# 666DZY666/micronet

Hardware: NVIDIA H100
Metric: qat_step_images_per_sec (higher is better)
Workload: dtype f32 (bf16 tensor-core products of exact integer levels / exact bf16 pieces, fp32 accumulate)

## Files before the change

### harness/fconv_probe.py

```python
import ctypes as C
import os
import subprocess
import sys

import torch


def run():
    from micronet_b200 import _lib as L
    lib = L.load()
    B, Cc, H, W, K, R = 256, 3, 32, 32, 256, 5
    dev = torch.device("cuda")
    x = torch.randn(B, Cc, H, W, device=dev)
    w = torch.randn(K, Cc, R, R, device=dev) * 0.1
    b = torch.randn(K, device=dev)
    y = torch.empty(B, K, H, W, device=dev)
    dy = torch.randn(B, K, H, W, device=dev)
    dw = torch.empty_like(w)
    sh = L.ConvShape(B, Cc, H, W, K, R, R, 1, 1, R // 2, R // 2, 1, 1, 1)
    scratch = torch.empty(int(lib.mnb_fconv2d_wgrad_tc_scratch_bytes(C.byref(sh))), dtype=torch.uint8, device=dev)
    err = L.tc_err_flag(dev)

    def fwd():
        L.check(lib.mnb_fconv2d_fwd_tc(C.byref(sh), x.data_ptr(), w.data_ptr(), b.data_ptr(), y.data_ptr(), err.data_ptr(),
                                       L.stream()), "fwd")

    def wg():
        L.check(lib.mnb_fconv2d_wgrad_tc(C.byref(sh), dy.data_ptr(), x.data_ptr(), dw.data_ptr(), scratch.data_ptr(),
                                         err.data_ptr(), L.stream()), "wgrad")
    out = []
    for name, fn in (("fwd", fwd), ("wgrad", wg)):
        for _ in range(3):
            fn()
        torch.cuda.synchronize()
        e0, e1 = torch.cuda.Event(enable_timing=True), torch.cuda.Event(enable_timing=True)
        e0.record()
        for _ in range(10):
            fn()
        e1.record()
        torch.cuda.synchronize()
        out.append(f"{name} {e0.elapsed_time(e1) * 100:.1f}us")
    print(os.environ.get("MNB_FCONV_DEBUG", "0"), " ".join(out), flush=True)


if __name__ == "__main__":
    if len(sys.argv) > 1:
        run()
    else:
        for mask in (0, 1, 2, 4, 8, 3, 7, 9, 15):
            subprocess.run([sys.executable, __file__, "child"], env=dict(os.environ, MNB_FCONV_DEBUG=str(mask)), timeout=120)
```

### include/micronet_b200.h

```cpp
#ifndef MICRONET_B200_H
#define MICRONET_B200_H

#include <stdint.h>

#ifdef __cplusplus
extern "C" {
#endif

typedef void* mnb_stream_t;

#define MNB_E_ARG (-1)
#define MNB_E_UNSUPPORTED (-2)

int mnb_version(void);
const char* mnb_last_error(void);
int64_t mnb_launch_count(void);

typedef struct {
  int32_t batch, in_c, in_h, in_w;
  int32_t out_c, ker_h, ker_w;
  int32_t stride_h, stride_w, pad_h, pad_w, dil_h, dil_w, groups;
} mnb_conv_shape;

#define MNB_ACT_DOREFA 1
#define MNB_ACT_IAO 2
#define MNB_ACT_SIGN 3

typedef struct {
  int32_t mode;
  int32_t bits;
  int32_t qmin, qmax;
  int32_t q_type;
  const float* scale;
  const float* zero_point;
  const float* obs_min;
  const float* obs_max;
} mnb_act_qparams;

int mnb_act_quant_fwd(const float* x, int64_t n, const mnb_act_qparams* qp, uint8_t* codes,
                      uint32_t* pass_bits, float* xq, mnb_stream_t stream);
int mnb_act_quant_bwd(const float* g, const uint32_t* pass_bits, int64_t n, const mnb_act_qparams* qp,
                      float* dx, mnb_stream_t stream);

int mnb_bn_fold_fwd(const float* w, int32_t out_c, int32_t per_channel, const float* gamma, const float* beta,
                    const float* bias, const float* mean, const float* var, double eps, float* w_fused, float* b_fused,
                    mnb_stream_t stream);
int mnb_bn_fold_bwd(const float* dw_fused, const float* db_fused, const float* w, int32_t out_c, int32_t per_channel,
                    const float* gamma, const float* bias, const float* mean, const float* var, double eps, float* dw,
                    float* out6, mnb_stream_t stream);
int mnb_bn_fold_running(float* running_mean, float* running_var, const float* batch_mean, const float* batch_var, int32_t n,
                        double momentum, int32_t first, mnb_stream_t stream);

int mnb_quant_add_fwd(const float* a, const float* b, int64_t n, const mnb_act_qparams* qp, float* out,
                      uint32_t* pass_bits_a, uint32_t* pass_bits_b, int32_t relu ,
                      mnb_stream_t stream);
int mnb_quant_add_bwd(const float* g, const uint32_t* pass_bits_a, const uint32_t* pass_bits_b, int64_t n,
                      const mnb_act_qparams* qp, float* da, float* db, mnb_stream_t stream);

int64_t mnb_observe_scratch_bytes(int64_t n, int32_t rows);
int mnb_iao_observe(const float* x, int64_t n, int32_t rows, int32_t observer_kind, int32_t first,
                    double momentum, double percentile, float* min_val, float* max_val,
                    int32_t update_qparams, int32_t symmetric, int32_t qmin, int32_t qmax,
                    float* scale, float* zero_point, void* scratch, mnb_stream_t stream);
int mnb_iao_update_qparams(const float* min_val, const float* max_val, int32_t rows, int32_t symmetric,
                           int32_t qmin, int32_t qmax, float* scale, float* zero_point,
                           mnb_stream_t stream);

int mnb_dorefa_weight_fwd(const float* w, int64_t numel, int32_t out_c, int32_t w_bits, int16_t* w_int,
                          float* w_scale, float* wq, float* aux, void* scratch, mnb_stream_t stream);
int mnb_dorefa_weight_bwd(const float* g_wq, const float* aux, int64_t numel, int32_t w_bits, float* dw,
                          void* scratch, mnb_stream_t stream);
int mnb_wb_weight_fwd(float* w, int32_t out_c, int32_t in_c_per_group, int32_t ker_hw, int32_t W,
                      int16_t* w_int, float* w_scale, float* wq, float* aux, mnb_stream_t stream);
int mnb_wb_weight_bwd(const float* g_wq, const float* w, const float* aux, int32_t out_c,
                      int32_t in_c_per_group, int32_t ker_hw, int32_t W, float* dw, mnb_stream_t stream);
int mnb_iao_weight_fwd(const float* w, int64_t numel, int32_t out_c, int32_t rows, const float* scale,
                       const float* zero_point, const float* obs_min, const float* obs_max,
                       int32_t q_type, int32_t qmin, int32_t qmax, int16_t* w_int, float* w_scale,
                       float* wq, uint8_t* pass, mnb_stream_t stream);
int mnb_iao_weight_bwd(const float* g_wq, const uint8_t* pass, const float* scale, int64_t numel,
                       int32_t out_c, int32_t rows, float* dw, mnb_stream_t stream);

typedef struct {
  const uint8_t* a_codes;
  const float* a_f32;
  int32_t a_offset;
  const float* a_offset_zp;
  const float* a_scale;
  const int16_t* w_int;
  const float* w_scale;
  const float* w_f32;
  const float* bias;
} mnb_conv_operands;

int mnb_conv2d_fwd(const mnb_conv_shape* s, const mnb_conv_operands* op, float* y, mnb_stream_t stream);
int mnb_conv2d_dgrad(const mnb_conv_shape* s, const float* dy, const float* wq, const uint32_t* pass_bits,
                     const mnb_act_qparams* qp, float* dx, mnb_stream_t stream);
int64_t mnb_wgrad_scratch_bytes(const mnb_conv_shape* s);
int mnb_conv2d_wgrad(const mnb_conv_shape* s, const float* dy, const mnb_conv_operands* op, float* dwq,
                     void* scratch, mnb_stream_t stream);
int mnb_channel_stats(const float* x, int32_t batch, int32_t channels, int32_t hw, int32_t as_mean_var,
                      float* stats, void* scratch, mnb_stream_t stream);
int mnb_channel_stats_bwd(const float* x, const float* mean, const float* dmean, const float* dvar,
                          int32_t batch, int32_t channels, int32_t hw, float* dx, mnb_stream_t stream);

int mnb_fq_conv2d_fwd_tc(const mnb_conv_shape* s, const float* x, const mnb_act_qparams* qp,
                         const int16_t* w_int, const float* w_scale, const float* bias, float* y,
                         uint8_t* codes, uint32_t* pass_bits, void* wpack_scratch, int32_t* err_flag,
                         mnb_stream_t stream);

int mnb_conv2d_dgrad_tc(const mnb_conv_shape* s, const float* dy, const int16_t* w_int, const float* w_scale,
                        const uint32_t* pass_bits, const mnb_act_qparams* qp, float* dx, void* wpack_scratch,
                        int32_t* err_flag, mnb_stream_t stream);

int64_t mnb_wgrad_tc_scratch_bytes(const mnb_conv_shape* s);
int mnb_conv2d_wgrad_tc(const mnb_conv_shape* s, const float* dy, const float* x, const mnb_act_qparams* qp,
                        float* dwq, void* scratch, int32_t* inexact_flag, int32_t* err_flag, mnb_stream_t stream);
int mnb_conv2d_wgrad_cond(const mnb_conv_shape* s, const float* dy, const mnb_conv_operands* op, float* dwq,
                          void* scratch, const int32_t* run_if_nonzero, mnb_stream_t stream);

int mnb_bn_batch_stats(const float* x, int32_t batch, int32_t channels, int32_t hw, double eps, double momentum,
                       float* running_mean, float* running_var, int64_t* num_batches_tracked, float* mean_invstd,
                       void* scratch, mnb_stream_t stream);
int mnb_bn_sign_fwd(const float* x, int32_t batch, int32_t channels, int32_t hw, const float* mean, const float* invstd,
                    const float* gamma, const float* beta, int32_t out_shuffle_groups, float* y, uint32_t* pass_bits,
                    mnb_stream_t stream);
int mnb_bn_sign_bwd(const float* g, const uint32_t* pass_bits, const float* x, int32_t batch, int32_t channels, int32_t hw,
                    const float* mean, const float* invstd, const float* gamma, int32_t training,
                    int32_t out_shuffle_groups, float* dx, float* dgamma, float* dbeta, float* dx_channel_sum,
                    void* scratch, mnb_stream_t stream);

int mnb_bn_sign_pool_fwd(const float* x, int32_t batch, int32_t channels, int32_t H, int32_t W, const float* mean,
                         const float* invstd, const float* gamma, const float* beta, int32_t out_shuffle_groups, float* y,
                         uint32_t* pass_bits, uint8_t* argmax, mnb_stream_t stream);
int mnb_bn_sign_pool_bwd(const float* g, const uint32_t* pass_bits, const uint8_t* argmax, const float* x, int32_t batch,
                         int32_t channels, int32_t H, int32_t W, const float* mean, const float* invstd, const float* gamma,
                         int32_t training, int32_t out_shuffle_groups, float* dx, float* dgamma, float* dbeta,
                         float* dx_channel_sum, void* scratch, mnb_stream_t stream);

int mnb_maxpool2d_fwd(const float* x, int32_t batch, int32_t channels, int32_t H, int32_t W, int32_t kernel, int32_t stride,
                      int32_t pad, int32_t out_shuffle_groups, float* y, uint8_t* argmax, mnb_stream_t stream);
int mnb_maxpool2d_bwd(const float* g, const uint8_t* argmax, int32_t batch, int32_t channels, int32_t H, int32_t W,
                      int32_t kernel, int32_t stride, int32_t pad, int32_t out_shuffle_groups, float* dx,
                      mnb_stream_t stream);

int mnb_bn_sign_fwd_packed(const float* x, int32_t batch, int32_t channels, int32_t hw, const float* mean,
                           const float* invstd, const float* gamma, const float* beta, int32_t out_shuffle_groups, float* y,
                           uint32_t* pass_bits, void* x_packed, mnb_stream_t stream);

int mnb_fconv2d_plan(const mnb_conv_shape* s, int32_t wgrad, int32_t* out, int32_t n);
int mnb_fconv2d_fwd_tc(const mnb_conv_shape* s, const float* x, const float* w, const float* bias, float* y,
                       int32_t* err_flag, mnb_stream_t stream);
int64_t mnb_fconv2d_wgrad_tc_scratch_bytes(const mnb_conv_shape* s);
int mnb_fconv2d_wgrad_tc(const mnb_conv_shape* s, const float* dy, const float* x, float* dw, void* scratch,
                         int32_t* err_flag, mnb_stream_t stream);

int64_t mnb_pk_act_bytes(int32_t batch, int32_t channels, int32_t h, int32_t w, int32_t terms);
int mnb_pk_pack_act(const float* x, int32_t batch, int32_t channels, int32_t h, int32_t w, const mnb_act_qparams* qp,
                    int32_t terms, const float* ch_scale, int32_t phase_split, void* out_pk, uint8_t* bits8,
                    mnb_stream_t stream);
int mnb_bn_relu_quant_pack_fwd(const float* x, int32_t batch, int32_t channels, int32_t hw, const float* mean,
                               const float* invstd, const float* gamma, const float* beta, const mnb_act_qparams* qp,
                               int32_t out_shuffle_groups, void* x_packed, uint32_t* pass_bits, mnb_stream_t stream);
int mnb_bn_sign_bwd_pack(const float* g, const uint32_t* pass_bits, const float* x, int32_t batch, int32_t channels, int32_t hw,
                         const float* mean, const float* invstd, const float* gamma, const float* dgamma, const float* dbeta,
                         int32_t out_shuffle_groups, const float* ch_scale, int32_t terms, float* dx, void* dy_packed,
                         mnb_stream_t stream);
int mnb_bn_sign_pool_bwd_pack(const float* g, const uint32_t* pass_bits, const uint8_t* argmax, const float* x, int32_t batch,
                              int32_t channels, int32_t H, int32_t W, const float* mean, const float* invstd,
                              const float* gamma, const float* dgamma, const float* dbeta, int32_t out_shuffle_groups,
                              const float* ch_scale, int32_t terms, void* dy_packed, mnb_stream_t stream);
int mnb_pk_conv_codes(const mnb_conv_shape* s, const void* a_pk, int32_t terms_a, const void* w_img, int32_t terms_w,
                      const float* n_scale, const float* a_scale, float a_scale_const, const float* bias, int32_t level_bound,
                      int16_t* codes, float* dec, int32_t* err_flag, mnb_stream_t stream);
int mnb_codes_decode(const int16_t* codes, const float* dec, int32_t batch, int32_t channels, int32_t hw, float* x,
                     mnb_stream_t stream);
int mnb_bn_batch_stats_codes(const int16_t* codes, const float* dec, int32_t batch, int32_t channels, int32_t hw, double eps,
                             double momentum, float* running_mean, float* running_var, int64_t* num_batches_tracked,
                             float* mean_invstd, void* scratch, mnb_stream_t stream);
int mnb_bn_sign_fwd_packed_codes(const int16_t* codes, const float* dec, int32_t batch, int32_t channels, int32_t hw,
                                 const float* mean, const float* invstd, const float* gamma, const float* beta,
                                 int32_t out_shuffle_groups, float* y, uint32_t* pass_bits, void* x_packed, mnb_stream_t stream);
int mnb_bn_sign_bwd_codes(const float* g, const uint32_t* pass_bits, const int16_t* codes, const float* dec, int32_t batch,
                          int32_t channels, int32_t hw, const float* mean, const float* invstd, const float* gamma,
                          int32_t training, int32_t out_shuffle_groups, float* dx, float* dgamma, float* dbeta,
                          float* dx_channel_sum, void* scratch, mnb_stream_t stream);
int mnb_bn_sign_pool_fwd_codes(const int16_t* codes, const float* dec, int32_t batch, int32_t channels, int32_t H, int32_t W,
                               const float* mean, const float* invstd, const float* gamma, const float* beta,
                               int32_t out_shuffle_groups, float* y, uint32_t* pass_bits, uint8_t* argmax, mnb_stream_t stream);
int mnb_bn_sign_pool_bwd_codes(const float* g, const uint32_t* pass_bits, const uint8_t* argmax, const int16_t* codes,
                               const float* dec, int32_t batch, int32_t channels, int32_t H, int32_t W, const float* mean,
                               const float* invstd, const float* gamma, int32_t training, int32_t out_shuffle_groups, float* dx,
                               float* dgamma, float* dbeta, float* dx_channel_sum, void* scratch, mnb_stream_t stream);
int mnb_bn_sign_bwd_pack_codes(const float* g, const uint32_t* pass_bits, const int16_t* codes, const float* dec, int32_t batch,
                               int32_t channels, int32_t hw, const float* mean, const float* invstd, const float* gamma,
                               const float* dgamma, const float* dbeta, int32_t out_shuffle_groups, const float* ch_scale,
                               int32_t terms, float* dx, void* dy_packed, mnb_stream_t stream);
int mnb_bn_sign_pool_bwd_pack_codes(const float* g, const uint32_t* pass_bits, const uint8_t* argmax, const int16_t* codes,
                                    const float* dec, int32_t batch, int32_t channels, int32_t H, int32_t W, const float* mean,
                                    const float* invstd, const float* gamma, const float* dgamma, const float* dbeta,
                                    int32_t out_shuffle_groups, const float* ch_scale, int32_t terms, void* dy_packed,
                                    mnb_stream_t stream);
int mnb_pk_pack_act_relu(const float* x, int32_t batch, int32_t channels, int32_t h, int32_t w, const mnb_act_qparams* qp,
                         int32_t terms, const float* ch_scale, int32_t phase_split, int32_t relu, void* out_pk,
                         uint8_t* bits8, mnb_stream_t stream);
int64_t mnb_pk_grouped_act_bytes(int32_t batch, int32_t channels, int32_t h, int32_t w, int32_t terms, int32_t groups);
int mnb_pk_pack_act_grouped(const float* x, int32_t batch, int32_t channels, int32_t h, int32_t w, const mnb_act_qparams* qp,
                            int32_t terms, const float* ch_scale, int32_t phase_split, int32_t relu, void* out_pk,
                            uint8_t* bits8, int32_t groups, mnb_stream_t stream);
int mnb_pk_conv_plan(const mnb_conv_shape* s, int32_t mode, int32_t terms_a, int32_t terms_w, int32_t* out16);
int mnb_pk_conv_plan_ex(const mnb_conv_shape* s, int32_t mode, int32_t terms_a, int32_t terms_w, int32_t* out, int32_t n);
int mnb_pk_wgrad_plan(const mnb_conv_shape* s, int32_t terms_dy, int32_t terms_x, int32_t* out, int32_t n);
int64_t mnb_pk_wimage_bytes(const mnb_conv_shape* s, int32_t mode, int32_t terms_a, int32_t terms_w);
int mnb_pk_pack_weight(const mnb_conv_shape* s, int32_t mode, int32_t terms_a, int32_t terms_w, const int16_t* w_int,
                       const float* w_f32, const float* kzero, void* w_img, mnb_stream_t stream);
int mnb_pk_conv(const mnb_conv_shape* s, int32_t mode, const void* a_pk, int32_t terms_a, const void* w_img, int32_t terms_w,
                const float* n_scale, const float* a_scale, float a_scale_const, const float* bias, const uint8_t* bits8,
                float gain, float* out, int32_t* err_flag, mnb_stream_t stream);
typedef struct mnb_pk_post {
  const mnb_act_qparams* q;
  int32_t relu;
  int32_t phase_split;
  void* out_pk;
  const float* bn_mean;
  const float* bn_invstd;
  const float* bn_gamma;
  const float* bn_beta;
  int32_t shuffle_groups;
} mnb_pk_post;
int mnb_pk_conv_post(const mnb_conv_shape* s, const void* a_pk, int32_t terms_a, const void* w_img, int32_t terms_w,
                     const float* n_scale, const float* a_scale, float a_scale_const, const float* bias, float* out,
                     const mnb_pk_post* post, int32_t* err_flag, mnb_stream_t stream);
int mnb_quant_add_pack_fwd(const float* a, const float* b, int32_t batch, int32_t channels, int32_t h, int32_t w,
                           const mnb_act_qparams* qp, int32_t relu, float* out, const mnb_pk_post* post, mnb_stream_t stream);
int64_t mnb_pk_i8_act_bytes(int32_t batch, int32_t channels, int32_t h, int32_t w);
int mnb_pk_i8_pack_act(const float* x, int32_t batch, int32_t channels, int32_t h, int32_t w, const mnb_act_qparams* qp,
                       int32_t phase_split, int32_t relu, void* out_pk, mnb_stream_t stream);
int mnb_pk_i8_conv_plan(const mnb_conv_shape* s, int32_t* out, int32_t n);
int64_t mnb_pk_i8_wimage_bytes(const mnb_conv_shape* s);
int mnb_pk_i8_pack_weight(const mnb_conv_shape* s, const int16_t* w_int, void* w_img, mnb_stream_t stream);
int mnb_pk_i8_conv(const mnb_conv_shape* s, const void* a_pk, const void* w_img, const float* n_scale, const float* a_scale,
                   float a_scale_const, const float* bias, float* out, const mnb_pk_post* post, int32_t* err_flag,
                   mnb_stream_t stream);
int mnb_quant_add_pack_i8_fwd(const float* a, const float* b, int32_t batch, int32_t channels, int32_t h, int32_t w,
                              const mnb_act_qparams* qp, int32_t relu, float* out, const mnb_pk_post* post, mnb_stream_t stream);
int mnb_bn_relu_quant_pack_i8_fwd(const float* x, int32_t batch, int32_t channels, int32_t hw, const float* mean,
                                  const float* invstd, const float* gamma, const float* beta, const mnb_act_qparams* qp,
                                  int32_t out_shuffle_groups, void* x_packed, mnb_stream_t stream);
int mnb_pk_plane_maxpool(const void* in_pk, int32_t batch, int32_t channels, int32_t h, int32_t w, int32_t k, int32_t s, int32_t p,
                         int32_t int8, void* out_pk, mnb_stream_t stream);
int mnb_pk_plane_maxpool_requant(const void* in_pk, int32_t batch, int32_t channels, int32_t h, int32_t w, int32_t k, int32_t s,
                                 int32_t p, int32_t int8, const mnb_act_qparams* q_in, const mnb_act_qparams* q_out, void* out_pk,
                                 mnb_stream_t stream);
int64_t mnb_pk_wgrad_scratch_bytes(const mnb_conv_shape* s, int32_t terms_dy, int32_t terms_x);
int mnb_pk_wgrad(const mnb_conv_shape* s, const void* dy_pk, int32_t terms_dy, const void* x_pk, int32_t terms_x,
                 const float* a_scale, const float* kdiv, float* dw, void* scratch, int32_t* err_flag, mnb_stream_t stream);
int mnb_pk_wgrad_taps_plan(const mnb_conv_shape* s, int32_t terms_dy, int32_t terms_x, int32_t* out, int32_t n);
int mnb_pk_wgrad_taps(const mnb_conv_shape* s, const void* dy_pk, int32_t terms_dy, const void* x_pk, int32_t terms_x,
                      const float* a_scale, const float* kdiv, float* dw, void* scratch, int32_t* err_flag, mnb_stream_t stream);
int mnb_pk_gc3_plan(const mnb_conv_shape* s, int32_t mode, int32_t terms_a, int32_t terms_w, int32_t* out, int32_t n);
int mnb_pk_gc3_conv(const mnb_conv_shape* s, int32_t mode, const void* a_pk, int32_t terms_a, const void* w_img, int32_t terms_w,
                    const float* n_scale, const float* a_scale, float a_scale_const, const float* bias, const uint8_t* bits8,
                    float gain, float* out, int32_t* err_flag, mnb_stream_t stream);
int mnb_pk_gc3_conv_codes(const mnb_conv_shape* s, const void* a_pk, int32_t terms_a, const void* w_img, int32_t terms_w,
                          const float* n_scale, const float* a_scale, float a_scale_const, const float* bias, int32_t level_bound,
                          int16_t* codes, float* dec, int32_t* err_flag, mnb_stream_t stream);

int mnb_xnor_supported(const mnb_conv_shape* s);
int64_t mnb_xnor_act_bytes(int32_t batch, int32_t channels, int32_t h, int32_t w, int32_t groups);
int mnb_xnor_pack_act(const float* x, int32_t batch, int32_t channels, int32_t h, int32_t w, int32_t groups, void* out_bits,
                      mnb_stream_t stream);
int64_t mnb_xnor_wimage_bytes(const mnb_conv_shape* s);
int mnb_xnor_pack_weight(const mnb_conv_shape* s, const int16_t* w_int, void* w_img, mnb_stream_t stream);
int mnb_xnor_conv_fwd(const mnb_conv_shape* s, const void* a_bits, const void* w_img, const float* alpha, const float* bias,
                      float* y, mnb_stream_t stream);
#define MNB_XNOR_BITS 0
#define MNB_XNOR_PM1_BF16 1
typedef struct mnb_xnor_post {
  int32_t format;
  int32_t out_groups;
  int32_t shuffle_groups;
  int32_t pool2;
  const float* bn_mean;
  const float* bn_invstd;
  const float* bn_gamma;
  const float* bn_beta;
} mnb_xnor_post;
int64_t mnb_xnor_post_bytes(const mnb_conv_shape* s, const mnb_xnor_post* post);
int mnb_xnor_conv_post(const mnb_conv_shape* s, const void* a_bits, const void* w_img, const float* alpha, const float* bias,
                       const mnb_xnor_post* post, void* out, mnb_stream_t stream);
int mnb_xnor_pack_act_post(const float* x, int32_t batch, int32_t channels, int32_t h, int32_t w, const mnb_xnor_post* post,
                           void* out_bits, mnb_stream_t stream);

int mnb_adam_step(float* params, const float* grads, float* exp_avg, float* exp_avg_sq, int64_t n, float lr,
                  float beta1, float beta2, float eps, float weight_decay, int32_t step, mnb_stream_t stream);

void mnb_set_tc_profile_buffer(void* dev_int64x16);

int mnb_selftest_umma(const float* A, const float* B, float* D, int32_t N, int32_t K, int32_t int8,
                      int32_t* err_flag, mnb_stream_t stream);
int mnb_selftest_tma3d(const float* src, const int64_t* dims3_host, const int32_t* box3_host,
                       const int32_t* coord3_host, float* out, int32_t* err_flag, mnb_stream_t stream);

int mnb_selftest_mma_rate(int32_t N, int32_t n_acc, int32_t a_shift16, int32_t iters, int32_t mn_major,
                          int64_t* out2, int32_t* err_flag, mnb_stream_t stream);

#ifdef __cplusplus
}
#endif
#endif
```

### micronet_b200/_lib.py

```python
from __future__ import annotations

import ctypes as C
import os

import torch

_HERE = os.path.dirname(os.path.abspath(__file__))
LIB_PATH = os.path.join(_HERE, "lib", "libmicronet_b200.so")

ACT_DOREFA, ACT_IAO, ACT_SIGN = 1, 2, 3


class ConvShape(C.Structure):
    _fields_ = [(n, C.c_int32) for n in (
        "batch", "in_c", "in_h", "in_w", "out_c", "ker_h", "ker_w", "stride_h", "stride_w",
        "pad_h", "pad_w", "dil_h", "dil_w", "groups")]


class ActQParams(C.Structure):
    _fields_ = [("mode", C.c_int32), ("bits", C.c_int32), ("qmin", C.c_int32), ("qmax", C.c_int32),
                ("q_type", C.c_int32), ("scale", C.c_void_p), ("zero_point", C.c_void_p),
                ("obs_min", C.c_void_p), ("obs_max", C.c_void_p)]


class PkPost(C.Structure):
    _fields_ = [("q", C.POINTER(ActQParams)), ("relu", C.c_int32), ("phase_split", C.c_int32), ("out_pk", C.c_void_p),
                ("bn_mean", C.c_void_p), ("bn_invstd", C.c_void_p), ("bn_gamma", C.c_void_p), ("bn_beta", C.c_void_p),
                ("shuffle_groups", C.c_int32)]


XNOR_BITS, XNOR_PM1_BF16 = 0, 1


class XnorPost(C.Structure):
    _fields_ = [("format", C.c_int32), ("out_groups", C.c_int32), ("shuffle_groups", C.c_int32), ("pool2", C.c_int32),
                ("bn_mean", C.c_void_p), ("bn_invstd", C.c_void_p), ("bn_gamma", C.c_void_p), ("bn_beta", C.c_void_p)]


class ConvOperands(C.Structure):
    _fields_ = [("a_codes", C.c_void_p), ("a_f32", C.c_void_p), ("a_offset", C.c_int32),
                ("a_offset_zp", C.c_void_p), ("a_scale", C.c_void_p), ("w_int", C.c_void_p),
                ("w_scale", C.c_void_p), ("w_f32", C.c_void_p), ("bias", C.c_void_p)]


_P, _I, _L, _D = C.c_void_p, C.c_int32, C.c_int64, C.c_double
_SHAPE, _ACTQ, _OPS = C.POINTER(ConvShape), C.POINTER(ActQParams), C.POINTER(ConvOperands)

PROTOTYPES = {
    "mnb_version": (C.c_int, []),
    "mnb_last_error": (C.c_char_p, []),
    "mnb_launch_count": (_L, []),
    "mnb_act_quant_fwd": (C.c_int, [_P, _L, _ACTQ, _P, _P, _P, _P]),
    "mnb_act_quant_bwd": (C.c_int, [_P, _P, _L, _ACTQ, _P, _P]),
    "mnb_bn_fold_fwd": (C.c_int, [_P, _I, _I, _P, _P, _P, _P, _P, _D, _P, _P, _P]),
    "mnb_bn_fold_bwd": (C.c_int, [_P, _P, _P, _I, _I, _P, _P, _P, _P, _D, _P, _P, _P]),
    "mnb_bn_fold_running": (C.c_int, [_P, _P, _P, _P, _I, _D, _I, _P]),
    "mnb_quant_add_fwd": (C.c_int, [_P, _P, _L, _ACTQ, _P, _P, _P, _I, _P]),
    "mnb_quant_add_bwd": (C.c_int, [_P, _P, _P, _L, _ACTQ, _P, _P, _P]),
    "mnb_observe_scratch_bytes": (_L, [_L, _I]),
    "mnb_iao_observe": (C.c_int, [_P, _L, _I, _I, _I, _D, _D, _P, _P, _I, _I, _I, _I, _P, _P, _P, _P]),
    "mnb_iao_update_qparams": (C.c_int, [_P, _P, _I, _I, _I, _I, _P, _P, _P]),
    "mnb_dorefa_weight_fwd": (C.c_int, [_P, _L, _I, _I, _P, _P, _P, _P, _P, _P]),
    "mnb_dorefa_weight_bwd": (C.c_int, [_P, _P, _L, _I, _P, _P, _P]),
    "mnb_wb_weight_fwd": (C.c_int, [_P, _I, _I, _I, _I, _P, _P, _P, _P, _P]),
    "mnb_wb_weight_bwd": (C.c_int, [_P, _P, _P, _I, _I, _I, _I, _P, _P]),
    "mnb_iao_weight_fwd": (C.c_int, [_P, _L, _I, _I, _P, _P, _P, _P, _I, _I, _I, _P, _P, _P, _P, _P]),
    "mnb_iao_weight_bwd": (C.c_int, [_P, _P, _P, _L, _I, _I, _P, _P]),
    "mnb_conv2d_fwd": (C.c_int, [_SHAPE, _OPS, _P, _P]),
    "mnb_conv2d_dgrad": (C.c_int, [_SHAPE, _P, _P, _P, _ACTQ, _P, _P]),
    "mnb_wgrad_scratch_bytes": (_L, [_SHAPE]),
    "mnb_conv2d_wgrad": (C.c_int, [_SHAPE, _P, _OPS, _P, _P, _P]),
    "mnb_channel_stats": (C.c_int, [_P, _I, _I, _I, _I, _P, _P, _P]),
    "mnb_channel_stats_bwd": (C.c_int, [_P, _P, _P, _P, _I, _I, _I, _P, _P]),
    "mnb_fq_conv2d_fwd_tc": (C.c_int, [_SHAPE, _P, _ACTQ, _P, _P, _P, _P, _P, _P, _P, _P, _P]),
    "mnb_conv2d_dgrad_tc": (C.c_int, [_SHAPE, _P, _P, _P, _P, _ACTQ, _P, _P, _P, _P]),
    "mnb_wgrad_tc_scratch_bytes": (_L, [_SHAPE]),
    "mnb_conv2d_wgrad_tc": (C.c_int, [_SHAPE, _P, _P, _ACTQ, _P, _P, _P, _P, _P]),
    "mnb_conv2d_wgrad_cond": (C.c_int, [_SHAPE, _P, _OPS, _P, _P, _P, _P]),
    "mnb_bn_batch_stats": (C.c_int, [_P, _I, _I, _I, _D, _D, _P, _P, _P, _P, _P, _P]),
    "mnb_bn_sign_fwd": (C.c_int, [_P, _I, _I, _I, _P, _P, _P, _P, _I, _P, _P, _P]),
    "mnb_bn_sign_bwd": (C.c_int, [_P, _P, _P, _I, _I, _I, _P, _P, _P, _I, _I, _P, _P, _P, _P, _P, _P]),
    "mnb_bn_sign_pool_fwd": (C.c_int, [_P, _I, _I, _I, _I, _P, _P, _P, _P, _I, _P, _P, _P, _P]),
    "mnb_bn_sign_pool_bwd": (C.c_int, [_P, _P, _P, _P, _I, _I, _I, _I, _P, _P, _P, _I, _I, _P, _P, _P, _P, _P, _P]),
    "mnb_bn_sign_fwd_packed": (C.c_int, [_P, _I, _I, _I, _P, _P, _P, _P, _I, _P, _P, _P, _P]),
    "mnb_fconv2d_plan": (C.c_int, [_SHAPE, _I, _P, _I]),
    "mnb_fconv2d_fwd_tc": (C.c_int, [_SHAPE, _P, _P, _P, _P, _P, _P]),
    "mnb_fconv2d_wgrad_tc_scratch_bytes": (_L, [_SHAPE]),
    "mnb_fconv2d_wgrad_tc": (C.c_int, [_SHAPE, _P, _P, _P, _P, _P, _P]),
    "mnb_maxpool2d_fwd": (C.c_int, [_P, _I, _I, _I, _I, _I, _I, _I, _I, _P, _P, _P]),
    "mnb_maxpool2d_bwd": (C.c_int, [_P, _P, _I, _I, _I, _I, _I, _I, _I, _I, _P, _P]),
    "mnb_adam_step": (C.c_int, [_P, _P, _P, _P, _L, C.c_float, C.c_float, C.c_float, C.c_float, C.c_float, _I, _P]),
    "mnb_pk_act_bytes": (_L, [_I, _I, _I, _I, _I]),
    "mnb_pk_pack_act": (C.c_int, [_P, _I, _I, _I, _I, _ACTQ, _I, _P, _I, _P, _P, _P]),
    "mnb_bn_relu_quant_pack_fwd": (C.c_int, [_P, _I, _I, _I, _P, _P, _P, _P, _ACTQ, _I, _P, _P, _P]),
    "mnb_pk_pack_act_relu": (C.c_int, [_P, _I, _I, _I, _I, _ACTQ, _I, _P, _I, _I, _P, _P, _P]),
    "mnb_pk_grouped_act_bytes": (_L, [_I, _I, _I, _I, _I, _I]),
    "mnb_pk_pack_act_grouped": (C.c_int, [_P, _I, _I, _I, _I, _ACTQ, _I, _P, _I, _I, _P, _P, _I, _P]),
    "mnb_pk_conv_plan": (C.c_int, [_SHAPE, _I, _I, _I, _P]),
    "mnb_pk_conv_plan_ex": (C.c_int, [_SHAPE, _I, _I, _I, _P, _I]),
    "mnb_pk_wgrad_plan": (C.c_int, [_SHAPE, _I, _I, _P, _I]),
    "mnb_pk_wimage_bytes": (_L, [_SHAPE, _I, _I, _I]),
    "mnb_pk_pack_weight": (C.c_int, [_SHAPE, _I, _I, _I, _P, _P, _P, _P, _P]),
    "mnb_pk_conv": (C.c_int, [_SHAPE, _I, _P, _I, _P, _I, _P, _P, C.c_float, _P, _P, C.c_float, _P, _P, _P]),
    "mnb_bn_sign_bwd_pack": (C.c_int, [_P, _P, _P, _I, _I, _I, _P, _P, _P, _P, _P, _I, _P, _I, _P, _P, _P]),
    "mnb_bn_sign_pool_bwd_pack": (C.c_int, [_P, _P, _P, _P, _I, _I, _I, _I, _P, _P, _P, _P, _P, _I, _P, _I, _P, _P]),
    "mnb_pk_conv_post": (C.c_int, [_SHAPE, _P, _I, _P, _I, _P, _P, C.c_float, _P, _P, C.POINTER(PkPost), _P, _P]),
    "mnb_pk_conv_codes": (C.c_int, [_SHAPE, _P, _I, _P, _I, _P, _P, C.c_float, _P, _I, _P, _P, _P, _P]),
    "mnb_codes_decode": (C.c_int, [_P, _P, _I, _I, _I, _P, _P]),
    "mnb_bn_batch_stats_codes": (C.c_int, [_P, _P, _I, _I, _I, _D, _D, _P, _P, _P, _P, _P, _P]),
    "mnb_bn_sign_fwd_packed_codes": (C.c_int, [_P, _P, _I, _I, _I, _P, _P, _P, _P, _I, _P, _P, _P, _P]),
    "mnb_bn_sign_bwd_codes": (C.c_int, [_P, _P, _P, _P, _I, _I, _I, _P, _P, _P, _I, _I, _P, _P, _P, _P, _P, _P]),
    "mnb_bn_sign_pool_fwd_codes": (C.c_int, [_P, _P, _I, _I, _I, _I, _P, _P, _P, _P, _I, _P, _P, _P, _P]),
    "mnb_bn_sign_pool_bwd_codes": (C.c_int, [_P, _P, _P, _P, _P, _I, _I, _I, _I, _P, _P, _P, _I, _I, _P, _P, _P, _P, _P, _P]),
    "mnb_bn_sign_bwd_pack_codes": (C.c_int, [_P, _P, _P, _P, _I, _I, _I, _P, _P, _P, _P, _P, _I, _P, _I, _P, _P, _P]),
    "mnb_bn_sign_pool_bwd_pack_codes": (C.c_int, [_P, _P, _P, _P, _P, _I, _I, _I, _I, _P, _P, _P, _P, _P, _I, _P, _I, _P,
                                                  _P]),
    "mnb_quant_add_pack_fwd": (C.c_int, [_P, _P, _I, _I, _I, _I, _ACTQ, _I, _P, C.POINTER(PkPost), _P]),
    "mnb_pk_i8_act_bytes": (_L, [_I, _I, _I, _I]),
    "mnb_pk_i8_pack_act": (C.c_int, [_P, _I, _I, _I, _I, _ACTQ, _I, _I, _P, _P]),
    "mnb_pk_i8_conv_plan": (C.c_int, [_SHAPE, _P, _I]),
    "mnb_pk_i8_wimage_bytes": (_L, [_SHAPE]),
    "mnb_pk_i8_pack_weight": (C.c_int, [_SHAPE, _P, _P, _P]),
    "mnb_pk_i8_conv": (C.c_int, [_SHAPE, _P, _P, _P, _P, C.c_float, _P, _P, C.POINTER(PkPost), _P, _P]),
    "mnb_quant_add_pack_i8_fwd": (C.c_int, [_P, _P, _I, _I, _I, _I, _ACTQ, _I, _P, C.POINTER(PkPost), _P]),
    "mnb_bn_relu_quant_pack_i8_fwd": (C.c_int, [_P, _I, _I, _I, _P, _P, _P, _P, _ACTQ, _I, _P, _P]),
    "mnb_pk_plane_maxpool": (C.c_int, [_P, _I, _I, _I, _I, _I, _I, _I, _I, _P, _P]),
    "mnb_pk_plane_maxpool_requant": (C.c_int, [_P, _I, _I, _I, _I, _I, _I, _I, _I, _ACTQ, _ACTQ, _P, _P]),
    "mnb_pk_wgrad_scratch_bytes": (_L, [_SHAPE, _I, _I]),
    "mnb_pk_wgrad": (C.c_int, [_SHAPE, _P, _I, _P, _I, _P, _P, _P, _P, _P, _P]),
    "mnb_pk_wgrad_taps_plan": (C.c_int, [_SHAPE, _I, _I, _P, _I]),
    "mnb_pk_wgrad_taps": (C.c_int, [_SHAPE, _P, _I, _P, _I, _P, _P, _P, _P, _P, _P]),
    "mnb_pk_gc3_plan": (C.c_int, [_SHAPE, _I, _I, _I, _P, _I]),
    "mnb_pk_gc3_conv": (C.c_int, [_SHAPE, _I, _P, _I, _P, _I, _P, _P, C.c_float, _P, _P, C.c_float, _P, _P, _P]),
    "mnb_pk_gc3_conv_codes": (C.c_int, [_SHAPE, _P, _I, _P, _I, _P, _P, C.c_float, _P, _I, _P, _P, _P, _P]),
    "mnb_xnor_supported": (C.c_int, [_SHAPE]),
    "mnb_xnor_act_bytes": (_L, [_I, _I, _I, _I, _I]),
    "mnb_xnor_pack_act": (C.c_int, [_P, _I, _I, _I, _I, _I, _P, _P]),
    "mnb_xnor_wimage_bytes": (_L, [_SHAPE]),
    "mnb_xnor_pack_weight": (C.c_int, [_SHAPE, _P, _P, _P]),
    "mnb_xnor_conv_fwd": (C.c_int, [_SHAPE, _P, _P, _P, _P, _P, _P]),
    "mnb_xnor_post_bytes": (_L, [_SHAPE, C.POINTER(XnorPost)]),
    "mnb_xnor_conv_post": (C.c_int, [_SHAPE, _P, _P, _P, _P, C.POINTER(XnorPost), _P, _P]),
    "mnb_xnor_pack_act_post": (C.c_int, [_P, _I, _I, _I, _I, C.POINTER(XnorPost), _P, _P]),
    "mnb_set_tc_profile_buffer": (None, [_P]),
    "mnb_selftest_mma_rate": (C.c_int, [_I, _I, _I, _I, _I, _P, _P, _P]),
    "mnb_selftest_umma": (C.c_int, [_P, _P, _P, _I, _I, _I, _P, _P]),
    "mnb_selftest_tma3d": (C.c_int, [_P, C.POINTER(C.c_int64), C.POINTER(C.c_int32), C.POINTER(C.c_int32), _P, _P, _P]),
}

_lib = None


def load():
    global _lib
    if _lib is not None:
        return _lib
    if not os.path.exists(LIB_PATH):
        raise RuntimeError(
            f"micronet_b200: {LIB_PATH} is missing - build it with `python -m micronet_b200.build` "
            "(there is no CPU / PyTorch fallback for the fake-quant hot path)")
    lib = C.CDLL(LIB_PATH)
    for name, (res, args) in PROTOTYPES.items():
        fn = getattr(lib, name)
        fn.restype, fn.argtypes = res, args
    _lib = lib
    return lib


def check(rc: int, what: str):
    if rc != 0:
        msg = load().mnb_last_error().decode(errors="replace")
        kind = ValueError if rc < 0 else RuntimeError
        raise kind(f"micronet_b200.{what} failed (code {rc}): {msg}")


def ptr(t):
    return None if t is None else t.data_ptr()


def stream():
    return torch.cuda.current_stream().cuda_stream


def require_cuda(*tensors):
    for t in tensors:
        if t is not None and not t.is_cuda:
            raise RuntimeError(
                "micronet_b200: the fake-quant engine runs on CUDA (sm_90a) tensors only; "
                "got a CPU tensor - there is deliberately no CPU fallback")


def require_f32(*tensors):
    for t in tensors:
        if t is not None and t.dtype != torch.float32:
            raise TypeError(f"micronet_b200: fp32 tensors only (the reference's QAT modules are fp32), got {t.dtype}")


def launch_count() -> int:
    return int(load().mnb_launch_count())


_errflags = {}


def tc_err_flag(device):
    key = (device.type, device.index)
    if key not in _errflags:
        _errflags[key] = torch.zeros(1, dtype=torch.int32, device=device)
    return _errflags[key]


def tc_check(device=None):
    for key, flag in _errflags.items():
        code = int(flag.item())
        if code:
            raise RuntimeError(f"micronet_b200: tensor-core pipeline wait timed out (code {code}) on {key}")


E_UNSUPPORTED = -2
KEEP_DEBUG = False
USE_TC = os.environ.get("MNB_DISABLE_TC", "0") != "1"
PK_MODE = os.environ.get("MNB_PK", "auto")
PK_TERMS = int(os.environ.get("MNB_PK_TERMS", "3"))
PK_TERMS_BWD = int(os.environ.get("MNB_PK_TERMS_BWD", "2"))
PK_WBWTAB = os.environ.get("MNB_PK_WBWTAB", "1") == "1"
PK_WG_TAPS = os.environ.get("MNB_PK_WG_TAPS", "1") != "0"
PK_GC3 = os.environ.get("MNB_PK_GC3", "1") != "0"

XNOR_MODE = os.environ.get("MNB_XNOR", "auto")

PLANE_ONLY = os.environ.get("MNB_PLANE_ONLY", "1") == "1"

_scratch = {}


def scratch(device, rows=1):
    lib = load()
    need = int(lib.mnb_observe_scratch_bytes(0, int(rows)))
    key = (device.type, device.index)
    buf = _scratch.get(key)
    if buf is None or buf.numel() < need:
        buf = torch.zeros(max(need, 1 << 20), dtype=torch.uint8, device=device)
        _scratch[key] = buf
    return buf
```

### micronet_b200/csrc/mnb_conv_fp32_tc.cu

```cuda
#include <cuda.h>
#include <cuda_bf16.h>

#include <algorithm>
#include <cstdlib>

#include "mnb_common.cuh"
#include "mnb_tc.cuh"

namespace tcfp32 {

constexpr int NTHREADS = 512;
constexpr int kMaxDynSmem = 227 * 1024 - 2560;
constexpr int SUB = 32;

struct Params {
  int B, C, K, H, W, R, pad;
  int KR, KP;
  int NP;
  int TH, PH, PW;
  int tiles_per_img, n_tiles;
  int nbuf_a;
  int off_b, off_a, off_patch, off_tab, off_sum, off_stg, sum_bytes, a_term_bytes, a_buf_bytes, b_term_bytes, patch_bytes;
  const float* x; const float* w; const float* bias; float* y;
  const float* dy; float* partial;
  int* err;
  int dbg;
};

struct alignas(16) Shared {
  uint64_t a_full[2], a_empty[2];
  uint32_t abort;
};

__device__ __forceinline__ uint32_t pack_bf16x2(float a, float b) {
  __nv_bfloat162 v = __floats2bfloat162_rn(a, b);
  return *reinterpret_cast<uint32_t*>(&v);
}
__device__ __forceinline__ void split3_pair(float a, float b, uint32_t& hp, uint32_t& mp, uint32_t& lp) {
  hp = pack_bf16x2(a, b);
  const float ra = a - __uint_as_float(hp << 16), rb = b - __uint_as_float(hp & 0xffff0000u);
  mp = pack_bf16x2(ra, rb);
  const float la = ra - __uint_as_float(mp << 16), lb = rb - __uint_as_float(mp & 0xffff0000u);
  lp = pack_bf16x2(la, lb);
}
__device__ __forceinline__ void store_split8(const float (&v)[8], uint8_t* dst, int term_bytes) {
  uint32_t hp[4], mp[4], lp[4];
#pragma unroll
  for (int j = 0; j < 4; ++j) split3_pair(v[2 * j], v[2 * j + 1], hp[j], mp[j], lp[j]);
  *reinterpret_cast<uint4*>(dst) = make_uint4(hp[0], hp[1], hp[2], hp[3]);
  *reinterpret_cast<uint4*>(dst + term_bytes) = make_uint4(mp[0], mp[1], mp[2], mp[3]);
  *reinterpret_cast<uint4*>(dst + 2 * term_bytes) = make_uint4(lp[0], lp[1], lp[2], lp[3]);
}
__device__ __forceinline__ void conv_bar_sync(int nthreads) {
  asm volatile("bar.sync 1, %0;" ::"r"(nthreads) : "memory");
}
__device__ __forceinline__ void mma_bar_sync() {
  asm volatile("bar.sync 2, 128;" ::: "memory");
}

__device__ __constant__ int kProdA[6] = {1, 2, 0, 1, 0, 0};
__device__ __constant__ int kProdB[6] = {1, 0, 2, 0, 1, 0};

constexpr int PF = 4;
__device__ __forceinline__ float patch_element(const Params& p, int i, int b, int h0) {
  const int pc = i % p.PW, t = i / p.PW;
  const int pr = t % p.PH, c = t / p.PH;
  const int h = h0 - p.pad + pr, w = pc - p.pad;
  return (h >= 0 && h < p.H && w >= 0 && w < p.W) ? __ldg(p.x + (((int64_t)b * p.C + c) * p.H + h) * p.W + w) : 0.f;
}
__device__ __forceinline__ void patch_fetch(const Params& p, int tile, int ct, int nconv, float (&v)[PF]) {
  const int b = tile / p.tiles_per_img, h0 = (tile - b * p.tiles_per_img) * p.TH;
  const int n = p.C * p.PH * p.PW;
#pragma unroll
  for (int k = 0; k < PF; ++k) {
    const int i = ct + k * nconv;
    v[k] = i < n ? patch_element(p, i, b, h0) : 0.f;
  }
}
__device__ __forceinline__ void patch_commit(const Params& p, float* patch, int tile, int ct, int nconv, const float (&v)[PF]) {
  const int b = tile / p.tiles_per_img, h0 = (tile - b * p.tiles_per_img) * p.TH;
  const int n = p.C * p.PH * p.PW;
#pragma unroll
  for (int k = 0; k < PF; ++k) {
    const int i = ct + k * nconv;
    if (i < n) patch[i] = v[k];
  }
  for (int i = ct + PF * nconv; i < n; i += nconv) patch[i] = patch_element(p, i, b, h0);
}

constexpr int FWD_NCONV = NTHREADS - 32 - 128;

__global__ void __launch_bounds__(NTHREADS, 1) fwd_kernel(const Params p) {
  extern __shared__ __align__(1024) uint8_t smem[];
  __shared__ Shared sh;
  __shared__ __align__(16) float epi_bias[256];
  const int tid = threadIdx.x, warp = tid >> 5, lane = tid & 31;
  uint8_t* bop = smem + p.off_b;
  uint8_t* aop = smem + p.off_a;
  int* tab = reinterpret_cast<int*>(smem + p.off_tab);
  const int kchunks = p.KP / 8;

  if (tid == 0) {
    for (int i = 0; i < 2; ++i) {
      tc::mbar_init(&sh.a_full[i], FWD_NCONV / 32); tc::mbar_init(&sh.a_empty[i], 4);
    }
    sh.abort = 0;
    tc::fence_barrier_init();
  }
  for (int n = tid; n < 256; n += NTHREADS) epi_bias[n] = (p.bias && n < p.K) ? __ldg(p.bias + n) : 0.f;
  for (int i = tid; i < kchunks * p.NP; i += NTHREADS) {
    const int j = i / p.NP, n = i - j * p.NP;
    float v[8];
#pragma unroll
    for (int e = 0; e < 8; ++e) {
      const int kk = j * 8 + e;
      v[e] = (n < p.K && kk < p.KR) ? __ldg(p.w + (int64_t)n * p.KR + kk) : 0.f;
    }
    store_split8(v, bop + (size_t)i * 16, p.b_term_bytes);
  }
  for (int kk = tid; kk < p.KP; kk += NTHREADS) {
    int off = -1;
    if (kk < p.KR) {
      const int s = kk % p.R, t = kk / p.R;
      const int r = t % p.R, c = t / p.R;
      off = (c * p.PH + r) * p.PW + s;
    }
    tab[kk] = off;
  }
  tc::fence_proxy_async_smem();
  __syncthreads();

  if (warp >= 4 && warp < 8) {
    const int m = (warp - 4) * 32 + lane;
    float* stage = reinterpret_cast<float*>(smem + p.off_stg);
    const int64_t plane = (int64_t)p.H * p.W;
    const uint64_t a_desc0 = tc::smem_desc_kmajor_noswz(tc::smem_u32(aop), 128u * 16u, 128u);
    const uint64_t b_desc0 = tc::smem_desc_kmajor_noswz(tc::smem_u32(bop), (uint32_t)p.NP * 16u, 128u);
    const uint32_t a_term16 = (uint32_t)p.a_term_bytes >> 4, b_term16 = (uint32_t)p.b_term_bytes >> 4;
    const uint32_t a_buf16 = (uint32_t)p.a_buf_bytes >> 4;
    const uint32_t a_step16 = 2u * 128u, b_step16 = 2u * (uint32_t)p.NP;
    uint32_t t = 0;
    for (int tile = blockIdx.x; tile < p.n_tiles; tile += gridDim.x, ++t) {
      const uint32_t ab = p.nbuf_a == 2 ? (t & 1u) : 0u, aph = p.nbuf_a == 2 ? ((t >> 1) & 1u) : (t & 1u);
      tc::mbar_wait_soft(&sh.a_full[ab], aph, p.err, 502, &sh.abort);
      const int b = tile / p.tiles_per_img, h0 = (tile - b * p.tiles_per_img) * p.TH;
      float* dst = p.y + (int64_t)b * p.K * plane + (int64_t)h0 * p.W + m;
      for (int n0 = 0; n0 < p.NP; n0 += 32) {
        float acc0[16], acc1[16];
        tc::zero_acc(acc0); tc::zero_acc(acc1);
        tc::wg_fence();
        tc::fence_acc(acc0); tc::fence_acc(acc1);
        for (int q = (p.dbg & 2) ? 6 : 0; q < 6; ++q) {
          const uint64_t aq = a_desc0 + (uint64_t)(ab * a_buf16 + (uint32_t)kProdA[q] * a_term16);
          const uint64_t bq = b_desc0 + (uint64_t)((uint32_t)kProdB[q] * b_term16 + (uint32_t)n0);
          for (int ks = 0; ks < p.KP / 16; ++ks) {
            const uint64_t ad = aq + (uint64_t)((uint32_t)ks * a_step16), bd = bq + (uint64_t)((uint32_t)ks * b_step16);
            tc::Mma<32>::bf16<0, 0>(acc0, ad, bd, 1);
            tc::Mma<32>::bf16<0, 0>(acc1, ad + 64u, bd, 1);
          }
        }
        tc::wg_commit();
        tc::wg_wait<0>();
        tc::fence_acc(acc0); tc::fence_acc(acc1);
        if (n0 + 32 >= p.NP) {
          __syncwarp();
          if (lane == 0) tc::mbar_arrive(&sh.a_empty[ab]);
        }
        mma_bar_sync();
        tc::frag_to_smem(acc0, stage, tc::kStageLd, 0);
        tc::frag_to_smem(acc1, stage, tc::kStageLd, 64);
        mma_bar_sync();
        if (p.dbg & 4) continue;
        float bs[32];
#pragma unroll
        for (int v = 0; v < 8; ++v) {
          const float4 c4 = *reinterpret_cast<const float4*>(&epi_bias[n0 + 4 * v]);
          bs[4 * v] = c4.x; bs[4 * v + 1] = c4.y; bs[4 * v + 2] = c4.z; bs[4 * v + 3] = c4.w;
        }
        float* op = dst + (int64_t)n0 * plane;
#pragma unroll
        for (int j = 0; j < 32; ++j, op += plane)
          if (n0 + j < p.K) *op = stage[j * tc::kStageLd + m] + bs[j];
      }
    }
  } else {
    if (warp == 0) goto done;
    const int ct = warp < 4 ? tid - 32 : tid - 32 - 128;
    float* patch0 = reinterpret_cast<float*>(smem + p.off_patch);
    const int items = 128 * kchunks;
    const int patch_floats = p.patch_bytes / 4;
    float pre[PF];
    if ((int)blockIdx.x < p.n_tiles) {
      patch_fetch(p, blockIdx.x, ct, FWD_NCONV, pre);
      patch_commit(p, patch0, blockIdx.x, ct, FWD_NCONV, pre);
    }
    uint32_t t = 0;
    for (int tile = blockIdx.x; tile < p.n_tiles; tile += gridDim.x, ++t) {
      const float* patch = patch0 + (size_t)(t & 1u) * patch_floats;
      conv_bar_sync(FWD_NCONV);
      const int next = tile + (int)gridDim.x;
      if (next < p.n_tiles) patch_fetch(p, next, ct, FWD_NCONV, pre);
      const uint32_t ab = p.nbuf_a == 2 ? (t & 1u) : 0u, aph = p.nbuf_a == 2 ? ((t >> 1) & 1u) : (t & 1u);
      if (!tc::mbar_wait(&sh.a_empty[ab], aph ^ 1u, p.err, 504)) break;
      uint8_t* abuf = aop + (size_t)ab * p.a_buf_bytes;
      for (int i = (p.dbg & 1) ? items : ct; i < items; i += FWD_NCONV) {
        const int j = i >> 7, m = i & 127;
        const int base = (m / p.W) * p.PW + (m % p.W);
        int off[8];
#pragma unroll
        for (int e = 0; e < 8; ++e) off[e] = tab[j * 8 + e];
        float v[8];
#pragma unroll
        for (int e = 0; e < 8; ++e) v[e] = off[e] >= 0 ? patch[off[e] + base] : 0.f;
        store_split8(v, abuf + (size_t)i * 16, p.a_term_bytes);
      }
      tc::fence_proxy_async_smem();
      __syncwarp();
      if (lane == 0) tc::mbar_arrive(&sh.a_full[ab]);
      if (next < p.n_tiles) patch_commit(p, patch0 + (size_t)((t + 1) & 1u) * patch_floats, next, ct, FWD_NCONV, pre);
    }
  }
done:
  __syncthreads();
}

constexpr int WG_NCONV = NTHREADS - 32 - 128;

__global__ void __launch_bounds__(NTHREADS, 1) wgrad_kernel(const Params p) {
  extern __shared__ __align__(1024) uint8_t smem[];
  __shared__ Shared sh;
  const int tid = threadIdx.x, warp = tid >> 5, lane = tid & 31;
  uint8_t* bop = smem + p.off_b;
  uint8_t* aop = smem + p.off_a;
  int* tab = reinterpret_cast<int*>(smem + p.off_tab);
  const int halves = p.NP / 128;
  const int nsub = 128 / SUB;

  if (tid == 0) {
    for (int i = 0; i < 2; ++i) {
      tc::mbar_init(&sh.a_full[i], WG_NCONV / 32); tc::mbar_init(&sh.a_empty[i], 4);
    }
    sh.abort = 0;
    tc::fence_barrier_init();
  }
  for (int i = tid; i < (2 * (p.a_buf_bytes + 3 * p.b_term_bytes) + p.sum_bytes) / 16; i += NTHREADS)
    reinterpret_cast<uint4*>(smem + p.off_b)[i] = make_uint4(0, 0, 0, 0);
  for (int kk = tid; kk < p.KP; kk += NTHREADS) {
    int off = -1;
    if (kk < p.KR) {
      const int s = kk % p.R, t = kk / p.R;
      const int r = t % p.R, c = t / p.R;
      off = (c * p.PH + r) * p.PW + s;
    }
    tab[kk] = off;
  }
  tc::fence_proxy_async_smem();
  __syncthreads();
  const int b_buf_bytes = 3 * p.b_term_bytes;

  if (warp >= 4 && warp < 8) {
    const int m = (warp - 4) * 32 + lane, wq = warp - 4;
    float* sum = reinterpret_cast<float*>(smem + p.off_sum);
    const uint64_t a_desc0 = tc::smem_desc_kmajor_noswz(tc::smem_u32(aop), (uint32_t)p.NP * 16u, 128u);
    const uint64_t b_desc0 = tc::smem_desc_kmajor_noswz(tc::smem_u32(bop), (uint32_t)p.KP * 16u, 128u);
    const uint32_t a_term16 = (uint32_t)p.a_term_bytes >> 4, b_term16 = (uint32_t)p.b_term_bytes >> 4;
    const uint32_t a_buf16 = (uint32_t)p.a_buf_bytes >> 4, b_buf16 = (uint32_t)b_buf_bytes >> 4;
    const uint32_t a_step16 = 2u * (uint32_t)p.NP, b_step16 = 2u * (uint32_t)p.KP;
    const int fr = 16 * wq + (lane >> 2), fc = 2 * (lane & 3);
    uint32_t it = 0;
    for (int tile = blockIdx.x; tile < p.n_tiles; tile += gridDim.x) {
      for (int sub = 0; sub < nsub; ++sub, ++it) {
        const uint32_t ob = it & 1u, oph = (it >> 1) & 1u;
        tc::mbar_wait_soft(&sh.a_full[ob], oph, p.err, 511, &sh.abort);
        for (int hf = (p.dbg & 2) ? halves : 0; hf < halves; ++hf) {
          for (int k0 = 0; k0 < p.KP; k0 += 32) {
            float acc0[16], acc1[16];
            tc::zero_acc(acc0); tc::zero_acc(acc1);
            tc::wg_fence();
            tc::fence_acc(acc0); tc::fence_acc(acc1);
            for (int q = 0; q < 6; ++q) {
              const uint64_t aq = a_desc0 + (uint64_t)(ob * a_buf16 + (uint32_t)kProdA[q] * a_term16 + (uint32_t)hf * 128u);
              const uint64_t bq = b_desc0 + (uint64_t)(ob * b_buf16 + (uint32_t)kProdB[q] * b_term16 + (uint32_t)k0);
#pragma unroll
              for (int ks = 0; ks < SUB / 16; ++ks) {
                const uint64_t ad = aq + (uint64_t)((uint32_t)ks * a_step16), bd = bq + (uint64_t)((uint32_t)ks * b_step16);
                tc::Mma<32>::bf16<0, 0>(acc0, ad, bd, 1);
                tc::Mma<32>::bf16<0, 0>(acc1, ad + 64u, bd, 1);
              }
            }
            tc::wg_commit();
            tc::wg_wait<0>();
            tc::fence_acc(acc0); tc::fence_acc(acc1);
            if (p.dbg & 4) continue;
#pragma unroll
            for (int j = 0; j < 4; ++j)
#pragma unroll
              for (int e = 0; e < 4; ++e) {
                const int col = k0 + 8 * j + fc + (e & 1), row = fr + 8 * (e >> 1);
                if (col < p.KP) {
                  float* s0 = sum + ((hf * p.KP) + col) * 128 + row;
                  s0[0] = __fadd_rn(s0[0], acc0[4 * j + e]);
                  s0[64] = __fadd_rn(s0[64], acc1[4 * j + e]);
                }
              }
          }
        }
        __syncwarp();
        if (lane == 0) tc::mbar_arrive(&sh.a_empty[ob]);
      }
    }
    mma_bar_sync();
    float* mine = p.partial + (int64_t)blockIdx.x * p.K * p.KR;
    for (int hf = 0; hf < halves; ++hf) {
      const int n = hf * 128 + m;
      if (n < p.K)
        for (int kk = 0; kk < p.KR; ++kk) mine[(int64_t)n * p.KR + kk] = sum[((hf * p.KP) + kk) * 128 + m];
    }
  } else if (warp != 0) {
    const int ct = warp < 4 ? tid - 32 : tid - 32 - 128;
    float* patch0 = reinterpret_cast<float*>(smem + p.off_patch);
    const int64_t plane = (int64_t)p.H * p.W;
    const int d_items = p.K * (SUB / 8), x_items = p.KR * (SUB / 8);
    const int patch_floats = p.patch_bytes / 4;
    constexpr int DMAX = 3;
    float4 dpre[DMAX][2];
    auto fetch_dy = [&](int tile, int sub) {
      const int b = tile / p.tiles_per_img, h0 = (tile - b * p.tiles_per_img) * p.TH;
      const float* dy_tile = p.dy + (int64_t)b * p.K * plane + (int64_t)h0 * p.W + sub * SUB;
#pragma unroll
      for (int k = 0; k < DMAX; ++k) {
        const int i = ct + k * WG_NCONV;
        if (i < d_items) {
          const int n = i / (SUB / 8), j = i - n * (SUB / 8);
          const float4* src = reinterpret_cast<const float4*>(dy_tile + (int64_t)n * plane + j * 8);
          dpre[k][0] = __ldg(src); dpre[k][1] = __ldg(src + 1);
        }
      }
    };
    float pre[PF];
    if ((int)blockIdx.x < p.n_tiles) {
      patch_fetch(p, blockIdx.x, ct, WG_NCONV, pre);
      patch_commit(p, patch0, blockIdx.x, ct, WG_NCONV, pre);
      fetch_dy(blockIdx.x, 0);
    }
    uint32_t it = 0, t = 0;
    for (int tile = blockIdx.x; tile < p.n_tiles; tile += gridDim.x, ++t) {
      const float* patch = patch0 + (size_t)(t & 1u) * patch_floats;
      conv_bar_sync(WG_NCONV);
      const int next = tile + (int)gridDim.x;
      if (next < p.n_tiles) patch_fetch(p, next, ct, WG_NCONV, pre);
      for (int sub = 0; sub < nsub; ++sub, ++it) {
        const uint32_t ob = it & 1u, oph = (it >> 1) & 1u;
        float4 dcur[DMAX][2];
#pragma unroll
        for (int k = 0; k < DMAX; ++k) { dcur[k][0] = dpre[k][0]; dcur[k][1] = dpre[k][1]; }
        if (sub + 1 < nsub) fetch_dy(tile, sub + 1);
        else if (next < p.n_tiles) fetch_dy(next, 0);
        if (!tc::mbar_wait(&sh.a_empty[ob], oph ^ 1u, p.err, 512)) goto done;
        uint8_t* abuf = aop + (size_t)ob * p.a_buf_bytes;
        uint8_t* bbuf = bop + (size_t)ob * b_buf_bytes;
        if (!(p.dbg & 1)) {
#pragma unroll
          for (int k = 0; k < DMAX; ++k) {
            const int i = ct + k * WG_NCONV;
            if (i < d_items) {
              const int n = i / (SUB / 8), j = i - n * (SUB / 8);
              const float v[8] = {dcur[k][0].x, dcur[k][0].y, dcur[k][0].z, dcur[k][0].w,
                                  dcur[k][1].x, dcur[k][1].y, dcur[k][1].z, dcur[k][1].w};
              store_split8(v, abuf + ((size_t)j * p.NP + n) * 16, p.a_term_bytes);
            }
          }
        }
        for (int i = (p.dbg & 8) ? x_items : ct; i < x_items; i += WG_NCONV) {
          const int kk = i / (SUB / 8), j = i - kk * (SUB / 8);
          const int m = sub * SUB + j * 8;
          const float* src = patch + tab[kk] + (m / p.W) * p.PW + (m % p.W);
          float v[8];
#pragma unroll
          for (int e = 0; e < 8; ++e) v[e] = src[e];
          store_split8(v, bbuf + ((size_t)j * p.KP + kk) * 16, p.b_term_bytes);
        }
        tc::fence_proxy_async_smem();
        __syncwarp();
        if (lane == 0) tc::mbar_arrive(&sh.a_full[ob]);
      }
      if (next < p.n_tiles) patch_commit(p, patch0 + (size_t)((t + 1) & 1u) * patch_floats, next, ct, WG_NCONV, pre);
    }
  }
done:
  __syncthreads();
}

__global__ void __launch_bounds__(256) reduce_partials_kernel(const float* __restrict__ partial, int n, int ranks,
                                                              float* __restrict__ dw) {
  for (int i = blockIdx.x * blockDim.x + threadIdx.x; i < n; i += gridDim.x * blockDim.x) {
    float s = 0.f;
    for (int j = 0; j < ranks; ++j) s += partial[(int64_t)j * n + i];
    dw[i] = s;
  }
}

static int plan(const mnb_conv_shape* s, bool wgrad, Params& p, int& smem_bytes) {
  MNB_REQUIRE(s != nullptr, "conv shape is NULL");
  auto unsupported = [](const char* why) { return mnb_fail(MNB_E_UNSUPPORTED, "fp32 tc conv: %s", why); };
  p.B = s->batch; p.C = s->in_c; p.K = s->out_c; p.H = s->in_h; p.W = s->in_w; p.R = s->ker_h;
  MNB_REQUIRE(p.B > 0 && p.C > 0 && p.K > 0 && p.H > 0 && p.W > 0 && s->groups > 0, "bad conv shape");
  if (s->groups != 1 || s->stride_h != 1 || s->stride_w != 1 || s->dil_h != 1 || s->dil_w != 1)
    return unsupported("groups / stride / dilation != 1");
  if (s->ker_h != s->ker_w || (p.R & 1) == 0 || s->pad_h != p.R / 2 || s->pad_w != p.R / 2)
    return unsupported("not a 'same' odd square filter");
  p.pad = p.R / 2;
  p.KR = p.C * p.R * p.R;
  p.KP = (p.KR + 15) / 16 * 16;
  if (p.KP > 128) return unsupported("C*R*S > 128 (use the per-tap implicit GEMM)");
  if (p.K > 256) return unsupported("more than 256 output channels");
  if (p.W < 8 || p.W > 128 || 128 % p.W || (p.H * p.W) % 128) return unsupported("image rows do not tile into 128 positions");
  if ((int64_t)p.B * p.K * p.H * p.W >= (1ll << 31)) return unsupported("tensor too large");
  p.TH = 128 / p.W;
  p.PH = p.TH + 2 * p.pad; p.PW = p.W + 2 * p.pad;
  p.tiles_per_img = p.H / p.TH;
  p.n_tiles = p.B * p.tiles_per_img;
  p.patch_bytes = (p.C * p.PH * p.PW * 4 + 8 * 4 + 15) / 16 * 16;
  const int kchunks = p.KP / 8;
  if (!wgrad) {
    p.NP = (p.K + 15) / 16 * 16;
    p.b_term_bytes = kchunks * p.NP * 16;
    p.a_term_bytes = kchunks * 128 * 16;
    p.a_buf_bytes = 3 * p.a_term_bytes;
    p.off_b = 0;
    p.off_a = 3 * p.b_term_bytes;
    for (p.nbuf_a = 2; p.nbuf_a >= 1; --p.nbuf_a) {
      p.off_patch = p.off_a + p.nbuf_a * p.a_buf_bytes;
      p.off_tab = p.off_patch + 2 * p.patch_bytes;
      p.off_stg = (p.off_tab + p.KP * 4 + 15) / 16 * 16;
      smem_bytes = p.off_stg + 32 * tc::kStageLd * 4;
      if (smem_bytes <= kMaxDynSmem) break;
    }
    if (p.nbuf_a < 1) return unsupported("shared memory budget");
  } else {
    p.NP = (p.K + 127) / 128 * 128;
    p.a_term_bytes = (SUB / 8) * p.NP * 16;
    p.a_buf_bytes = 3 * p.a_term_bytes;
    p.b_term_bytes = (SUB / 8) * p.KP * 16;
    p.off_b = 0;
    p.off_a = 2 * 3 * p.b_term_bytes;
    p.off_sum = p.off_a + 2 * p.a_buf_bytes;
    p.sum_bytes = (p.NP / 128) * p.KP * 128 * 4;
    p.off_patch = p.off_sum + p.sum_bytes;
    p.off_tab = p.off_patch + 2 * p.patch_bytes;
    smem_bytes = p.off_tab + p.KP * 4;
    p.nbuf_a = 2;
    if (smem_bytes > kMaxDynSmem) return unsupported("shared memory budget");
  }
  return 0;
}

static int grid_size(const Params& p) { return std::max(1, std::min(p.n_tiles, MNB_NUM_SMS)); }
static int debug_mask() {
  static const int m = [] { const char* e = getenv("MNB_FCONV_DEBUG"); return e ? atoi(e) : 0; }();
  return m;
}

}

extern "C" int mnb_fconv2d_plan(const mnb_conv_shape* s, int32_t wgrad, int32_t* out, int32_t n) {
  tcfp32::Params p{};
  int smem_bytes = 0;
  if (int e = tcfp32::plan(s, wgrad != 0, p, smem_bytes)) return e;
  const int v[8] = {p.NP, p.KP, p.TH, p.n_tiles, tcfp32::grid_size(p), p.nbuf_a, smem_bytes, p.C * p.PH * p.PW};
  if (out)
    for (int i = 0; i < std::min(n, 8); ++i) out[i] = v[i];
  return 0;
}

extern "C" int mnb_fconv2d_fwd_tc(const mnb_conv_shape* s, const float* x, const float* w, const float* bias, float* y,
                                  int32_t* err_flag, mnb_stream_t stream) {
  using namespace tcfp32;
  MNB_REQUIRE(s && x && w && y && err_flag, "NULL pointer");
  Params p{};
  int smem_bytes = 0;
  if (int e = plan(s, false, p, smem_bytes)) return e;
  p.x = x; p.w = w; p.bias = bias; p.y = y; p.err = err_flag; p.dbg = debug_mask();
  static bool attr_set = false;
  if (!attr_set) {
    cudaError_t ce = cudaFuncSetAttribute(fwd_kernel, cudaFuncAttributeMaxDynamicSharedMemorySize, kMaxDynSmem);
    if (ce != cudaSuccess) return mnb_fail((int)ce, "cudaFuncSetAttribute: %s", cudaGetErrorString(ce));
    attr_set = true;
  }
  fwd_kernel<<<grid_size(p), NTHREADS, smem_bytes, (cudaStream_t)stream>>>(p);
  MNB_LAUNCHED(1);
  return 0;
}

extern "C" int64_t mnb_fconv2d_wgrad_tc_scratch_bytes(const mnb_conv_shape* s) {
  tcfp32::Params p{};
  int smem = 0;
  if (tcfp32::plan(s, true, p, smem)) return -1;
  return (int64_t)tcfp32::grid_size(p) * p.K * p.KR * 4;
}

extern "C" int mnb_fconv2d_wgrad_tc(const mnb_conv_shape* s, const float* dy, const float* x, float* dw, void* scratch,
                                    int32_t* err_flag, mnb_stream_t stream) {
  using namespace tcfp32;
  MNB_REQUIRE(s && dy && x && dw && scratch && err_flag, "NULL pointer");
  MNB_REQUIRE((reinterpret_cast<uintptr_t>(dy) & 15) == 0, "dy must be 16-byte aligned");
  Params p{};
  int smem_bytes = 0;
  if (int e = plan(s, true, p, smem_bytes)) return e;
  p.x = x; p.dy = dy; p.partial = reinterpret_cast<float*>(scratch); p.err = err_flag; p.dbg = debug_mask();
  static bool attr_set = false;
  if (!attr_set) {
    cudaError_t ce = cudaFuncSetAttribute(wgrad_kernel, cudaFuncAttributeMaxDynamicSharedMemorySize, kMaxDynSmem);
    if (ce != cudaSuccess) return mnb_fail((int)ce, "cudaFuncSetAttribute: %s", cudaGetErrorString(ce));
    attr_set = true;
  }
  const int grid = grid_size(p);
  cudaStream_t st = (cudaStream_t)stream;
  wgrad_kernel<<<grid, NTHREADS, smem_bytes, st>>>(p);
  const int n = p.K * p.KR;
  reduce_partials_kernel<<<std::min(mnb_ceil_div(n, 256), MNB_NUM_SMS * 4), 256, 0, st>>>(p.partial, n, grid, dw);
  MNB_LAUNCHED(2);
  return 0;
}
```

### micronet_b200/csrc/mnb_tc.cuh

```cuda
#pragma once
#include <cuda.h>
#include <cuda_runtime.h>
#include <stdint.h>

namespace tc {

__device__ __forceinline__ uint32_t smem_u32(const void* p) {
  return static_cast<uint32_t>(__cvta_generic_to_shared(p));
}

__device__ __forceinline__ void mbar_init(uint64_t* bar, uint32_t count) {
  asm volatile("mbarrier.init.shared::cta.b64 [%0], %1;" ::"r"(smem_u32(bar)), "r"(count));
}
__device__ __forceinline__ void fence_barrier_init() {
  asm volatile("fence.mbarrier_init.release.cluster;" ::: "memory");
}
__device__ __forceinline__ void mbar_arrive(uint64_t* bar) {
  asm volatile("mbarrier.arrive.shared::cta.b64 _, [%0];" ::"r"(smem_u32(bar)) : "memory");
}
__device__ __forceinline__ void mbar_arrive_expect_tx(uint64_t* bar, uint32_t bytes) {
  asm volatile("mbarrier.arrive.expect_tx.shared::cta.b64 _, [%0], %1;" ::"r"(smem_u32(bar)), "r"(bytes)
               : "memory");
}
__device__ __forceinline__ bool mbar_try_wait(uint64_t* bar, uint32_t parity) {
  uint32_t ok;
  asm volatile(
      "{\n\t.reg .pred p;\n\t"
      "mbarrier.try_wait.parity.shared::cta.b64 p, [%1], %2;\n\t"
      "selp.u32 %0, 1, 0, p;\n\t}"
      : "=r"(ok)
      : "r"(smem_u32(bar)), "r"(parity)
      : "memory");
  return ok != 0;
}
__device__ __forceinline__ bool mbar_wait(uint64_t* bar, uint32_t parity, int* err_flag, int code) {
  for (uint32_t it = 0; it < (1u << 24); ++it) {
    if (mbar_try_wait(bar, parity)) return true;
    if (it > 1024) __nanosleep(64);
    if ((it & 0xffff) == 0xffff && err_flag && *reinterpret_cast<volatile int*>(err_flag) != 0) return false;
  }
  if (err_flag) atomicCAS(err_flag, 0, code);
  return false;
}

__device__ __forceinline__ void mbar_wait_soft(uint64_t* bar, uint32_t parity, int* err_flag, int code,
                                               volatile uint32_t* abort_flag) {
  for (uint32_t it = 0;; ++it) {
    if (mbar_try_wait(bar, parity)) return;
    if ((it & 0xfffu) == 0xfffu) {
      if (*abort_flag) return;
      if (it >= (1u << 24)) {
        *abort_flag = 1u;
        if (err_flag) atomicCAS(err_flag, 0, code);
        return;
      }
      __nanosleep(64);
    }
  }
}

__device__ __forceinline__ void fence_proxy_async_smem() {
  asm volatile("fence.proxy.async.shared::cta;" ::: "memory");
}

__device__ __forceinline__ void prefetch_tmap(const CUtensorMap* m) {
  asm volatile("prefetch.tensormap [%0];" ::"l"(reinterpret_cast<uint64_t>(m)) : "memory");
}
__device__ __forceinline__ void tma_load_3d(void* smem_dst, const CUtensorMap* m, uint64_t* bar, int c0, int c1,
                                            int c2) {
  asm volatile(
      "cp.async.bulk.tensor.3d.shared::cta.global.mbarrier::complete_tx::bytes [%0], [%1, {%3, %4, %5}], [%2];"
      ::"r"(smem_u32(smem_dst)), "l"(reinterpret_cast<uint64_t>(m)), "r"(smem_u32(bar)), "r"(c0), "r"(c1), "r"(c2)
      : "memory");
}
__device__ __forceinline__ void tma_load_4d(void* smem_dst, const CUtensorMap* m, uint64_t* bar, int c0, int c1,
                                            int c2, int c3) {
  asm volatile(
      "cp.async.bulk.tensor.4d.shared::cta.global.mbarrier::complete_tx::bytes [%0], [%1, {%3, %4, %5, %6}], [%2];"
      ::"r"(smem_u32(smem_dst)), "l"(reinterpret_cast<uint64_t>(m)), "r"(smem_u32(bar)), "r"(c0), "r"(c1), "r"(c2),
      "r"(c3)
      : "memory");
}

__device__ __forceinline__ void tma_load_5d(void* smem_dst, const CUtensorMap* m, uint64_t* bar, int c0, int c1,
                                            int c2, int c3, int c4) {
  asm volatile(
      "cp.async.bulk.tensor.5d.shared::cta.global.mbarrier::complete_tx::bytes [%0], [%1, {%3, %4, %5, %6, %7}], [%2];"
      ::"r"(smem_u32(smem_dst)), "l"(reinterpret_cast<uint64_t>(m)), "r"(smem_u32(bar)), "r"(c0), "r"(c1), "r"(c2),
      "r"(c3), "r"(c4)
      : "memory");
}

__device__ __forceinline__ void bulk_load_1d(void* smem_dst, const void* gsrc, uint32_t bytes, uint64_t* bar) {
  asm volatile("cp.async.bulk.shared::cluster.global.mbarrier::complete_tx::bytes [%0], [%1], %2, [%3];"
               ::"r"(smem_u32(smem_dst)), "l"(reinterpret_cast<uint64_t>(gsrc)), "r"(bytes), "r"(smem_u32(bar))
               : "memory");
}

__device__ __forceinline__ void wg_fence() { asm volatile("wgmma.fence.sync.aligned;" ::: "memory"); }
__device__ __forceinline__ void wg_commit() { asm volatile("wgmma.commit_group.sync.aligned;" ::: "memory"); }
template <int N>
__device__ __forceinline__ void wg_wait() { asm volatile("wgmma.wait_group.sync.aligned %0;" ::"n"(N) : "memory"); }
__device__ __forceinline__ void fence_reg(float& r) { asm volatile("" : "+f"(r)::"memory"); }
__device__ __forceinline__ void fence_reg(int32_t& r) { asm volatile("" : "+r"(r)::"memory"); }
template <typename T, int NR>
__device__ __forceinline__ void fence_acc(T (&d)[NR]) {
#pragma unroll
  for (int i = 0; i < NR; ++i) fence_reg(d[i]);
}
template <typename T, int NR>
__device__ __forceinline__ void zero_acc(T (&d)[NR]) {
#pragma unroll
  for (int i = 0; i < NR; ++i) d[i] = T(0);
}

template <int N> struct Mma;
template <> struct Mma<16> {
  template <int TA, int TB>
  static __device__ __forceinline__ void bf16(float (&d)[8], uint64_t da, uint64_t db, uint32_t scale_d) {
    asm volatile(
        "{\n\t.reg .pred p;\n\tsetp.ne.b32 p, %10, 0;\n\t"
        "wgmma.mma_async.sync.aligned.m64n16k16.f32.bf16.bf16 "
        "{%0, %1, %2, %3, %4, %5, %6, %7}, %8, %9, p, 1, 1, %11, %12;\n\t}"
        : "+f"(d[0]), "+f"(d[1]), "+f"(d[2]), "+f"(d[3]), "+f"(d[4]), "+f"(d[5]), "+f"(d[6]), "+f"(d[7])
        : "l"(da), "l"(db), "r"(scale_d), "n"(TA), "n"(TB)
        : "memory");
  }
  static __device__ __forceinline__ void s8(int32_t (&d)[8], uint64_t da, uint64_t db, uint32_t scale_d) {
    asm volatile(
        "{\n\t.reg .pred p;\n\tsetp.ne.b32 p, %10, 0;\n\t"
        "wgmma.mma_async.sync.aligned.m64n16k32.s32.s8.s8 "
        "{%0, %1, %2, %3, %4, %5, %6, %7}, %8, %9, p;\n\t}"
        : "+r"(d[0]), "+r"(d[1]), "+r"(d[2]), "+r"(d[3]), "+r"(d[4]), "+r"(d[5]), "+r"(d[6]), "+r"(d[7])
        : "l"(da), "l"(db), "r"(scale_d)
        : "memory");
  }
};
template <> struct Mma<32> {
  template <int TA, int TB>
  static __device__ __forceinline__ void bf16(float (&d)[16], uint64_t da, uint64_t db, uint32_t scale_d) {
    asm volatile(
        "{\n\t.reg .pred p;\n\tsetp.ne.b32 p, %18, 0;\n\t"
        "wgmma.mma_async.sync.aligned.m64n32k16.f32.bf16.bf16 "
        "{%0, %1, %2, %3, %4, %5, %6, %7, %8, %9, %10, %11, %12, %13, %14, %15}, %16, %17, p, 1, 1, %19, %20;\n\t}"
        : "+f"(d[0]), "+f"(d[1]), "+f"(d[2]), "+f"(d[3]), "+f"(d[4]), "+f"(d[5]), "+f"(d[6]), "+f"(d[7]), "+f"(d[8]), "+f"(d[9]), "+f"(d[10]), "+f"(d[11]), "+f"(d[12]), "+f"(d[13]), "+f"(d[14]), "+f"(d[15])
        : "l"(da), "l"(db), "r"(scale_d), "n"(TA), "n"(TB)
        : "memory");
  }
  static __device__ __forceinline__ void s8(int32_t (&d)[16], uint64_t da, uint64_t db, uint32_t scale_d) {
    asm volatile(
        "{\n\t.reg .pred p;\n\tsetp.ne.b32 p, %18, 0;\n\t"
        "wgmma.mma_async.sync.aligned.m64n32k32.s32.s8.s8 "
        "{%0, %1, %2, %3, %4, %5, %6, %7, %8, %9, %10, %11, %12, %13, %14, %15}, %16, %17, p;\n\t}"
        : "+r"(d[0]), "+r"(d[1]), "+r"(d[2]), "+r"(d[3]), "+r"(d[4]), "+r"(d[5]), "+r"(d[6]), "+r"(d[7]), "+r"(d[8]), "+r"(d[9]), "+r"(d[10]), "+r"(d[11]), "+r"(d[12]), "+r"(d[13]), "+r"(d[14]), "+r"(d[15])
        : "l"(da), "l"(db), "r"(scale_d)
        : "memory");
  }
};
template <> struct Mma<48> {
  template <int TA, int TB>
  static __device__ __forceinline__ void bf16(float (&d)[24], uint64_t da, uint64_t db, uint32_t scale_d) {
    asm volatile(
        "{\n\t.reg .pred p;\n\tsetp.ne.b32 p, %26, 0;\n\t"
        "wgmma.mma_async.sync.aligned.m64n48k16.f32.bf16.bf16 "
        "{%0, %1, %2, %3, %4, %5, %6, %7, %8, %9, %10, %11, %12, %13, %14, %15, %16, %17, %18, %19, %20, %21, %22, %23}, %24, %25, p, 1, 1, %27, %28;\n\t}"
        : "+f"(d[0]), "+f"(d[1]), "+f"(d[2]), "+f"(d[3]), "+f"(d[4]), "+f"(d[5]), "+f"(d[6]), "+f"(d[7]), "+f"(d[8]), "+f"(d[9]), "+f"(d[10]), "+f"(d[11]), "+f"(d[12]), "+f"(d[13]), "+f"(d[14]), "+f"(d[15]), "+f"(d[16]), "+f"(d[17]), "+f"(d[18]), "+f"(d[19]), "+f"(d[20]), "+f"(d[21]), "+f"(d[22]), "+f"(d[23])
        : "l"(da), "l"(db), "r"(scale_d), "n"(TA), "n"(TB)
        : "memory");
  }
  static __device__ __forceinline__ void s8(int32_t (&d)[24], uint64_t da, uint64_t db, uint32_t scale_d) {
    asm volatile(
        "{\n\t.reg .pred p;\n\tsetp.ne.b32 p, %26, 0;\n\t"
        "wgmma.mma_async.sync.aligned.m64n48k32.s32.s8.s8 "
        "{%0, %1, %2, %3, %4, %5, %6, %7, %8, %9, %10, %11, %12, %13, %14, %15, %16, %17, %18, %19, %20, %21, %22, %23}, %24, %25, p;\n\t}"
        : "+r"(d[0]), "+r"(d[1]), "+r"(d[2]), "+r"(d[3]), "+r"(d[4]), "+r"(d[5]), "+r"(d[6]), "+r"(d[7]), "+r"(d[8]), "+r"(d[9]), "+r"(d[10]), "+r"(d[11]), "+r"(d[12]), "+r"(d[13]), "+r"(d[14]), "+r"(d[15]), "+r"(d[16]), "+r"(d[17]), "+r"(d[18]), "+r"(d[19]), "+r"(d[20]), "+r"(d[21]), "+r"(d[22]), "+r"(d[23])
        : "l"(da), "l"(db), "r"(scale_d)
        : "memory");
  }
};
template <> struct Mma<64> {
  template <int TA, int TB>
  static __device__ __forceinline__ void bf16(float (&d)[32], uint64_t da, uint64_t db, uint32_t scale_d) {
    asm volatile(
        "{\n\t.reg .pred p;\n\tsetp.ne.b32 p, %34, 0;\n\t"
        "wgmma.mma_async.sync.aligned.m64n64k16.f32.bf16.bf16 "
        "{%0, %1, %2, %3, %4, %5, %6, %7, %8, %9, %10, %11, %12, %13, %14, %15, %16, %17, %18, %19, %20, %21, %22, %23, %24, %25, %26, %27, %28, %29, %30, %31}, %32, %33, p, 1, 1, %35, %36;\n\t}"
        : "+f"(d[0]), "+f"(d[1]), "+f"(d[2]), "+f"(d[3]), "+f"(d[4]), "+f"(d[5]), "+f"(d[6]), "+f"(d[7]), "+f"(d[8]), "+f"(d[9]), "+f"(d[10]), "+f"(d[11]), "+f"(d[12]), "+f"(d[13]), "+f"(d[14]), "+f"(d[15]), "+f"(d[16]), "+f"(d[17]), "+f"(d[18]), "+f"(d[19]), "+f"(d[20]), "+f"(d[21]), "+f"(d[22]), "+f"(d[23]), "+f"(d[24]), "+f"(d[25]), "+f"(d[26]), "+f"(d[27]), "+f"(d[28]), "+f"(d[29]), "+f"(d[30]), "+f"(d[31])
        : "l"(da), "l"(db), "r"(scale_d), "n"(TA), "n"(TB)
        : "memory");
  }
  static __device__ __forceinline__ void s8(int32_t (&d)[32], uint64_t da, uint64_t db, uint32_t scale_d) {
    asm volatile(
        "{\n\t.reg .pred p;\n\tsetp.ne.b32 p, %34, 0;\n\t"
        "wgmma.mma_async.sync.aligned.m64n64k32.s32.s8.s8 "
        "{%0, %1, %2, %3, %4, %5, %6, %7, %8, %9, %10, %11, %12, %13, %14, %15, %16, %17, %18, %19, %20, %21, %22, %23, %24, %25, %26, %27, %28, %29, %30, %31}, %32, %33, p;\n\t}"
        : "+r"(d[0]), "+r"(d[1]), "+r"(d[2]), "+r"(d[3]), "+r"(d[4]), "+r"(d[5]), "+r"(d[6]), "+r"(d[7]), "+r"(d[8]), "+r"(d[9]), "+r"(d[10]), "+r"(d[11]), "+r"(d[12]), "+r"(d[13]), "+r"(d[14]), "+r"(d[15]), "+r"(d[16]), "+r"(d[17]), "+r"(d[18]), "+r"(d[19]), "+r"(d[20]), "+r"(d[21]), "+r"(d[22]), "+r"(d[23]), "+r"(d[24]), "+r"(d[25]), "+r"(d[26]), "+r"(d[27]), "+r"(d[28]), "+r"(d[29]), "+r"(d[30]), "+r"(d[31])
        : "l"(da), "l"(db), "r"(scale_d)
        : "memory");
  }
};
template <> struct Mma<80> {
  template <int TA, int TB>
  static __device__ __forceinline__ void bf16(float (&d)[40], uint64_t da, uint64_t db, uint32_t scale_d) {
    asm volatile(
        "{\n\t.reg .pred p;\n\tsetp.ne.b32 p, %42, 0;\n\t"
        "wgmma.mma_async.sync.aligned.m64n80k16.f32.bf16.bf16 "
        "{%0, %1, %2, %3, %4, %5, %6, %7, %8, %9, %10, %11, %12, %13, %14, %15, %16, %17, %18, %19, %20, %21, %22, %23, %24, %25, %26, %27, %28, %29, %30, %31, %32, %33, %34, %35, %36, %37, %38, %39}, %40, %41, p, 1, 1, %43, %44;\n\t}"
        : "+f"(d[0]), "+f"(d[1]), "+f"(d[2]), "+f"(d[3]), "+f"(d[4]), "+f"(d[5]), "+f"(d[6]), "+f"(d[7]), "+f"(d[8]), "+f"(d[9]), "+f"(d[10]), "+f"(d[11]), "+f"(d[12]), "+f"(d[13]), "+f"(d[14]), "+f"(d[15]), "+f"(d[16]), "+f"(d[17]), "+f"(d[18]), "+f"(d[19]), "+f"(d[20]), "+f"(d[21]), "+f"(d[22]), "+f"(d[23]), "+f"(d[24]), "+f"(d[25]), "+f"(d[26]), "+f"(d[27]), "+f"(d[28]), "+f"(d[29]), "+f"(d[30]), "+f"(d[31]), "+f"(d[32]), "+f"(d[33]), "+f"(d[34]), "+f"(d[35]), "+f"(d[36]), "+f"(d[37]), "+f"(d[38]), "+f"(d[39])
        : "l"(da), "l"(db), "r"(scale_d), "n"(TA), "n"(TB)
        : "memory");
  }
};
template <> struct Mma<96> {
  template <int TA, int TB>
  static __device__ __forceinline__ void bf16(float (&d)[48], uint64_t da, uint64_t db, uint32_t scale_d) {
    asm volatile(
        "{\n\t.reg .pred p;\n\tsetp.ne.b32 p, %50, 0;\n\t"
        "wgmma.mma_async.sync.aligned.m64n96k16.f32.bf16.bf16 "
        "{%0, %1, %2, %3, %4, %5, %6, %7, %8, %9, %10, %11, %12, %13, %14, %15, %16, %17, %18, %19, %20, %21, %22, %23, %24, %25, %26, %27, %28, %29, %30, %31, %32, %33, %34, %35, %36, %37, %38, %39, %40, %41, %42, %43, %44, %45, %46, %47}, %48, %49, p, 1, 1, %51, %52;\n\t}"
        : "+f"(d[0]), "+f"(d[1]), "+f"(d[2]), "+f"(d[3]), "+f"(d[4]), "+f"(d[5]), "+f"(d[6]), "+f"(d[7]), "+f"(d[8]), "+f"(d[9]), "+f"(d[10]), "+f"(d[11]), "+f"(d[12]), "+f"(d[13]), "+f"(d[14]), "+f"(d[15]), "+f"(d[16]), "+f"(d[17]), "+f"(d[18]), "+f"(d[19]), "+f"(d[20]), "+f"(d[21]), "+f"(d[22]), "+f"(d[23]), "+f"(d[24]), "+f"(d[25]), "+f"(d[26]), "+f"(d[27]), "+f"(d[28]), "+f"(d[29]), "+f"(d[30]), "+f"(d[31]), "+f"(d[32]), "+f"(d[33]), "+f"(d[34]), "+f"(d[35]), "+f"(d[36]), "+f"(d[37]), "+f"(d[38]), "+f"(d[39]), "+f"(d[40]), "+f"(d[41]), "+f"(d[42]), "+f"(d[43]), "+f"(d[44]), "+f"(d[45]), "+f"(d[46]), "+f"(d[47])
        : "l"(da), "l"(db), "r"(scale_d), "n"(TA), "n"(TB)
        : "memory");
  }
  static __device__ __forceinline__ void s8(int32_t (&d)[48], uint64_t da, uint64_t db, uint32_t scale_d) {
    asm volatile(
        "{\n\t.reg .pred p;\n\tsetp.ne.b32 p, %50, 0;\n\t"
        "wgmma.mma_async.sync.aligned.m64n96k32.s32.s8.s8 "
        "{%0, %1, %2, %3, %4, %5, %6, %7, %8, %9, %10, %11, %12, %13, %14, %15, %16, %17, %18, %19, %20, %21, %22, %23, %24, %25, %26, %27, %28, %29, %30, %31, %32, %33, %34, %35, %36, %37, %38, %39, %40, %41, %42, %43, %44, %45, %46, %47}, %48, %49, p;\n\t}"
        : "+r"(d[0]), "+r"(d[1]), "+r"(d[2]), "+r"(d[3]), "+r"(d[4]), "+r"(d[5]), "+r"(d[6]), "+r"(d[7]), "+r"(d[8]), "+r"(d[9]), "+r"(d[10]), "+r"(d[11]), "+r"(d[12]), "+r"(d[13]), "+r"(d[14]), "+r"(d[15]), "+r"(d[16]), "+r"(d[17]), "+r"(d[18]), "+r"(d[19]), "+r"(d[20]), "+r"(d[21]), "+r"(d[22]), "+r"(d[23]), "+r"(d[24]), "+r"(d[25]), "+r"(d[26]), "+r"(d[27]), "+r"(d[28]), "+r"(d[29]), "+r"(d[30]), "+r"(d[31]), "+r"(d[32]), "+r"(d[33]), "+r"(d[34]), "+r"(d[35]), "+r"(d[36]), "+r"(d[37]), "+r"(d[38]), "+r"(d[39]), "+r"(d[40]), "+r"(d[41]), "+r"(d[42]), "+r"(d[43]), "+r"(d[44]), "+r"(d[45]), "+r"(d[46]), "+r"(d[47])
        : "l"(da), "l"(db), "r"(scale_d)
        : "memory");
  }
};
template <> struct Mma<112> {
  template <int TA, int TB>
  static __device__ __forceinline__ void bf16(float (&d)[56], uint64_t da, uint64_t db, uint32_t scale_d) {
    asm volatile(
        "{\n\t.reg .pred p;\n\tsetp.ne.b32 p, %58, 0;\n\t"
        "wgmma.mma_async.sync.aligned.m64n112k16.f32.bf16.bf16 "
        "{%0, %1, %2, %3, %4, %5, %6, %7, %8, %9, %10, %11, %12, %13, %14, %15, %16, %17, %18, %19, %20, %21, %22, %23, %24, %25, %26, %27, %28, %29, %30, %31, %32, %33, %34, %35, %36, %37, %38, %39, %40, %41, %42, %43, %44, %45, %46, %47, %48, %49, %50, %51, %52, %53, %54, %55}, %56, %57, p, 1, 1, %59, %60;\n\t}"
        : "+f"(d[0]), "+f"(d[1]), "+f"(d[2]), "+f"(d[3]), "+f"(d[4]), "+f"(d[5]), "+f"(d[6]), "+f"(d[7]), "+f"(d[8]), "+f"(d[9]), "+f"(d[10]), "+f"(d[11]), "+f"(d[12]), "+f"(d[13]), "+f"(d[14]), "+f"(d[15]), "+f"(d[16]), "+f"(d[17]), "+f"(d[18]), "+f"(d[19]), "+f"(d[20]), "+f"(d[21]), "+f"(d[22]), "+f"(d[23]), "+f"(d[24]), "+f"(d[25]), "+f"(d[26]), "+f"(d[27]), "+f"(d[28]), "+f"(d[29]), "+f"(d[30]), "+f"(d[31]), "+f"(d[32]), "+f"(d[33]), "+f"(d[34]), "+f"(d[35]), "+f"(d[36]), "+f"(d[37]), "+f"(d[38]), "+f"(d[39]), "+f"(d[40]), "+f"(d[41]), "+f"(d[42]), "+f"(d[43]), "+f"(d[44]), "+f"(d[45]), "+f"(d[46]), "+f"(d[47]), "+f"(d[48]), "+f"(d[49]), "+f"(d[50]), "+f"(d[51]), "+f"(d[52]), "+f"(d[53]), "+f"(d[54]), "+f"(d[55])
        : "l"(da), "l"(db), "r"(scale_d), "n"(TA), "n"(TB)
        : "memory");
  }
};
template <> struct Mma<128> {
  template <int TA, int TB>
  static __device__ __forceinline__ void bf16(float (&d)[64], uint64_t da, uint64_t db, uint32_t scale_d) {
    asm volatile(
        "{\n\t.reg .pred p;\n\tsetp.ne.b32 p, %66, 0;\n\t"
        "wgmma.mma_async.sync.aligned.m64n128k16.f32.bf16.bf16 "
        "{%0, %1, %2, %3, %4, %5, %6, %7, %8, %9, %10, %11, %12, %13, %14, %15, %16, %17, %18, %19, %20, %21, %22, %23, %24, %25, %26, %27, %28, %29, %30, %31, %32, %33, %34, %35, %36, %37, %38, %39, %40, %41, %42, %43, %44, %45, %46, %47, %48, %49, %50, %51, %52, %53, %54, %55, %56, %57, %58, %59, %60, %61, %62, %63}, %64, %65, p, 1, 1, %67, %68;\n\t}"
        : "+f"(d[0]), "+f"(d[1]), "+f"(d[2]), "+f"(d[3]), "+f"(d[4]), "+f"(d[5]), "+f"(d[6]), "+f"(d[7]), "+f"(d[8]), "+f"(d[9]), "+f"(d[10]), "+f"(d[11]), "+f"(d[12]), "+f"(d[13]), "+f"(d[14]), "+f"(d[15]), "+f"(d[16]), "+f"(d[17]), "+f"(d[18]), "+f"(d[19]), "+f"(d[20]), "+f"(d[21]), "+f"(d[22]), "+f"(d[23]), "+f"(d[24]), "+f"(d[25]), "+f"(d[26]), "+f"(d[27]), "+f"(d[28]), "+f"(d[29]), "+f"(d[30]), "+f"(d[31]), "+f"(d[32]), "+f"(d[33]), "+f"(d[34]), "+f"(d[35]), "+f"(d[36]), "+f"(d[37]), "+f"(d[38]), "+f"(d[39]), "+f"(d[40]), "+f"(d[41]), "+f"(d[42]), "+f"(d[43]), "+f"(d[44]), "+f"(d[45]), "+f"(d[46]), "+f"(d[47]), "+f"(d[48]), "+f"(d[49]), "+f"(d[50]), "+f"(d[51]), "+f"(d[52]), "+f"(d[53]), "+f"(d[54]), "+f"(d[55]), "+f"(d[56]), "+f"(d[57]), "+f"(d[58]), "+f"(d[59]), "+f"(d[60]), "+f"(d[61]), "+f"(d[62]), "+f"(d[63])
        : "l"(da), "l"(db), "r"(scale_d), "n"(TA), "n"(TB)
        : "memory");
  }
  static __device__ __forceinline__ void s8(int32_t (&d)[64], uint64_t da, uint64_t db, uint32_t scale_d) {
    asm volatile(
        "{\n\t.reg .pred p;\n\tsetp.ne.b32 p, %66, 0;\n\t"
        "wgmma.mma_async.sync.aligned.m64n128k32.s32.s8.s8 "
        "{%0, %1, %2, %3, %4, %5, %6, %7, %8, %9, %10, %11, %12, %13, %14, %15, %16, %17, %18, %19, %20, %21, %22, %23, %24, %25, %26, %27, %28, %29, %30, %31, %32, %33, %34, %35, %36, %37, %38, %39, %40, %41, %42, %43, %44, %45, %46, %47, %48, %49, %50, %51, %52, %53, %54, %55, %56, %57, %58, %59, %60, %61, %62, %63}, %64, %65, p;\n\t}"
        : "+r"(d[0]), "+r"(d[1]), "+r"(d[2]), "+r"(d[3]), "+r"(d[4]), "+r"(d[5]), "+r"(d[6]), "+r"(d[7]), "+r"(d[8]), "+r"(d[9]), "+r"(d[10]), "+r"(d[11]), "+r"(d[12]), "+r"(d[13]), "+r"(d[14]), "+r"(d[15]), "+r"(d[16]), "+r"(d[17]), "+r"(d[18]), "+r"(d[19]), "+r"(d[20]), "+r"(d[21]), "+r"(d[22]), "+r"(d[23]), "+r"(d[24]), "+r"(d[25]), "+r"(d[26]), "+r"(d[27]), "+r"(d[28]), "+r"(d[29]), "+r"(d[30]), "+r"(d[31]), "+r"(d[32]), "+r"(d[33]), "+r"(d[34]), "+r"(d[35]), "+r"(d[36]), "+r"(d[37]), "+r"(d[38]), "+r"(d[39]), "+r"(d[40]), "+r"(d[41]), "+r"(d[42]), "+r"(d[43]), "+r"(d[44]), "+r"(d[45]), "+r"(d[46]), "+r"(d[47]), "+r"(d[48]), "+r"(d[49]), "+r"(d[50]), "+r"(d[51]), "+r"(d[52]), "+r"(d[53]), "+r"(d[54]), "+r"(d[55]), "+r"(d[56]), "+r"(d[57]), "+r"(d[58]), "+r"(d[59]), "+r"(d[60]), "+r"(d[61]), "+r"(d[62]), "+r"(d[63])
        : "l"(da), "l"(db), "r"(scale_d)
        : "memory");
  }
};
template <> struct Mma<144> {
  template <int TA, int TB>
  static __device__ __forceinline__ void bf16(float (&d)[72], uint64_t da, uint64_t db, uint32_t scale_d) {
    asm volatile(
        "{\n\t.reg .pred p;\n\tsetp.ne.b32 p, %74, 0;\n\t"
        "wgmma.mma_async.sync.aligned.m64n144k16.f32.bf16.bf16 "
        "{%0, %1, %2, %3, %4, %5, %6, %7, %8, %9, %10, %11, %12, %13, %14, %15, %16, %17, %18, %19, %20, %21, %22, %23, %24, %25, %26, %27, %28, %29, %30, %31, %32, %33, %34, %35, %36, %37, %38, %39, %40, %41, %42, %43, %44, %45, %46, %47, %48, %49, %50, %51, %52, %53, %54, %55, %56, %57, %58, %59, %60, %61, %62, %63, %64, %65, %66, %67, %68, %69, %70, %71}, %72, %73, p, 1, 1, %75, %76;\n\t}"
        : "+f"(d[0]), "+f"(d[1]), "+f"(d[2]), "+f"(d[3]), "+f"(d[4]), "+f"(d[5]), "+f"(d[6]), "+f"(d[7]), "+f"(d[8]), "+f"(d[9]), "+f"(d[10]), "+f"(d[11]), "+f"(d[12]), "+f"(d[13]), "+f"(d[14]), "+f"(d[15]), "+f"(d[16]), "+f"(d[17]), "+f"(d[18]), "+f"(d[19]), "+f"(d[20]), "+f"(d[21]), "+f"(d[22]), "+f"(d[23]), "+f"(d[24]), "+f"(d[25]), "+f"(d[26]), "+f"(d[27]), "+f"(d[28]), "+f"(d[29]), "+f"(d[30]), "+f"(d[31]), "+f"(d[32]), "+f"(d[33]), "+f"(d[34]), "+f"(d[35]), "+f"(d[36]), "+f"(d[37]), "+f"(d[38]), "+f"(d[39]), "+f"(d[40]), "+f"(d[41]), "+f"(d[42]), "+f"(d[43]), "+f"(d[44]), "+f"(d[45]), "+f"(d[46]), "+f"(d[47]), "+f"(d[48]), "+f"(d[49]), "+f"(d[50]), "+f"(d[51]), "+f"(d[52]), "+f"(d[53]), "+f"(d[54]), "+f"(d[55]), "+f"(d[56]), "+f"(d[57]), "+f"(d[58]), "+f"(d[59]), "+f"(d[60]), "+f"(d[61]), "+f"(d[62]), "+f"(d[63]), "+f"(d[64]), "+f"(d[65]), "+f"(d[66]), "+f"(d[67]), "+f"(d[68]), "+f"(d[69]), "+f"(d[70]), "+f"(d[71])
        : "l"(da), "l"(db), "r"(scale_d), "n"(TA), "n"(TB)
        : "memory");
  }
};
template <> struct Mma<160> {
  template <int TA, int TB>
  static __device__ __forceinline__ void bf16(float (&d)[80], uint64_t da, uint64_t db, uint32_t scale_d) {
    asm volatile(
        "{\n\t.reg .pred p;\n\tsetp.ne.b32 p, %82, 0;\n\t"
        "wgmma.mma_async.sync.aligned.m64n160k16.f32.bf16.bf16 "
        "{%0, %1, %2, %3, %4, %5, %6, %7, %8, %9, %10, %11, %12, %13, %14, %15, %16, %17, %18, %19, %20, %21, %22, %23, %24, %25, %26, %27, %28, %29, %30, %31, %32, %33, %34, %35, %36, %37, %38, %39, %40, %41, %42, %43, %44, %45, %46, %47, %48, %49, %50, %51, %52, %53, %54, %55, %56, %57, %58, %59, %60, %61, %62, %63, %64, %65, %66, %67, %68, %69, %70, %71, %72, %73, %74, %75, %76, %77, %78, %79}, %80, %81, p, 1, 1, %83, %84;\n\t}"
        : "+f"(d[0]), "+f"(d[1]), "+f"(d[2]), "+f"(d[3]), "+f"(d[4]), "+f"(d[5]), "+f"(d[6]), "+f"(d[7]), "+f"(d[8]), "+f"(d[9]), "+f"(d[10]), "+f"(d[11]), "+f"(d[12]), "+f"(d[13]), "+f"(d[14]), "+f"(d[15]), "+f"(d[16]), "+f"(d[17]), "+f"(d[18]), "+f"(d[19]), "+f"(d[20]), "+f"(d[21]), "+f"(d[22]), "+f"(d[23]), "+f"(d[24]), "+f"(d[25]), "+f"(d[26]), "+f"(d[27]), "+f"(d[28]), "+f"(d[29]), "+f"(d[30]), "+f"(d[31]), "+f"(d[32]), "+f"(d[33]), "+f"(d[34]), "+f"(d[35]), "+f"(d[36]), "+f"(d[37]), "+f"(d[38]), "+f"(d[39]), "+f"(d[40]), "+f"(d[41]), "+f"(d[42]), "+f"(d[43]), "+f"(d[44]), "+f"(d[45]), "+f"(d[46]), "+f"(d[47]), "+f"(d[48]), "+f"(d[49]), "+f"(d[50]), "+f"(d[51]), "+f"(d[52]), "+f"(d[53]), "+f"(d[54]), "+f"(d[55]), "+f"(d[56]), "+f"(d[57]), "+f"(d[58]), "+f"(d[59]), "+f"(d[60]), "+f"(d[61]), "+f"(d[62]), "+f"(d[63]), "+f"(d[64]), "+f"(d[65]), "+f"(d[66]), "+f"(d[67]), "+f"(d[68]), "+f"(d[69]), "+f"(d[70]), "+f"(d[71]), "+f"(d[72]), "+f"(d[73]), "+f"(d[74]), "+f"(d[75]), "+f"(d[76]), "+f"(d[77]), "+f"(d[78]), "+f"(d[79])
        : "l"(da), "l"(db), "r"(scale_d), "n"(TA), "n"(TB)
        : "memory");
  }
};
__device__ __forceinline__ void mma_s8_n128(int32_t (&d)[64], uint64_t da, uint64_t db, uint32_t scale_d) {
  asm volatile(
      "{\n\t.reg .pred p;\n\tsetp.ne.b32 p, %66, 0;\n\t"
      "wgmma.mma_async.sync.aligned.m64n128k32.s32.s8.s8 "
      "{%0, %1, %2, %3, %4, %5, %6, %7, %8, %9, %10, %11, %12, %13, %14, %15, %16, %17, %18, %19, %20, %21, %22, %23, %24, %25, %26, %27, %28, %29, %30, %31, %32, %33, %34, %35, %36, %37, %38, %39, %40, %41, %42, %43, %44, %45, %46, %47, %48, %49, %50, %51, %52, %53, %54, %55, %56, %57, %58, %59, %60, %61, %62, %63}, %64, %65, p;\n\t}"
      : "+r"(d[0]), "+r"(d[1]), "+r"(d[2]), "+r"(d[3]), "+r"(d[4]), "+r"(d[5]), "+r"(d[6]), "+r"(d[7]), "+r"(d[8]), "+r"(d[9]), "+r"(d[10]), "+r"(d[11]), "+r"(d[12]), "+r"(d[13]), "+r"(d[14]), "+r"(d[15]), "+r"(d[16]), "+r"(d[17]), "+r"(d[18]), "+r"(d[19]), "+r"(d[20]), "+r"(d[21]), "+r"(d[22]), "+r"(d[23]), "+r"(d[24]), "+r"(d[25]), "+r"(d[26]), "+r"(d[27]), "+r"(d[28]), "+r"(d[29]), "+r"(d[30]), "+r"(d[31]), "+r"(d[32]), "+r"(d[33]), "+r"(d[34]), "+r"(d[35]), "+r"(d[36]), "+r"(d[37]), "+r"(d[38]), "+r"(d[39]), "+r"(d[40]), "+r"(d[41]), "+r"(d[42]), "+r"(d[43]), "+r"(d[44]), "+r"(d[45]), "+r"(d[46]), "+r"(d[47]), "+r"(d[48]), "+r"(d[49]), "+r"(d[50]), "+r"(d[51]), "+r"(d[52]), "+r"(d[53]), "+r"(d[54]), "+r"(d[55]), "+r"(d[56]), "+r"(d[57]), "+r"(d[58]), "+r"(d[59]), "+r"(d[60]), "+r"(d[61]), "+r"(d[62]), "+r"(d[63])
      : "l"(da), "l"(db), "r"(scale_d)
      : "memory");
}

template <int NR>
__device__ __forceinline__ void frag_cols_to_smem(const float (&d)[NR], float* s, int ld, int row0, int c0, int nc) {
  const int lane = threadIdx.x & 31, w = (threadIdx.x >> 5) & 3;
  const int r = row0 + 16 * w + (lane >> 2), c = 2 * (lane & 3);
#pragma unroll
  for (int j = 0; j < NR / 4; ++j) {
    if (8 * j < c0 || 8 * j >= c0 + nc) continue;
    float* p = s + (8 * j - c0 + c) * ld + r;
    p[0] = d[4 * j]; p[ld] = d[4 * j + 1]; p[8] = d[4 * j + 2]; p[ld + 8] = d[4 * j + 3];
  }
}
template <int NR>
__device__ __forceinline__ void frag_to_smem(const float (&d)[NR], float* s, int ld, int row0) {
  frag_cols_to_smem(d, s, ld, row0, 0, 2 * NR);
}
constexpr int kStageLd = 132;
constexpr int kStageLd64 = 68;

__device__ __forceinline__ uint64_t smem_desc_kmajor_noswz(uint32_t saddr, uint32_t lbo_bytes, uint32_t sbo_bytes) {
  uint64_t d = 0;
  d |= (uint64_t)((saddr >> 4) & 0x3fff);
  d |= (uint64_t)((lbo_bytes >> 4) & 0x3fff) << 16;
  d |= (uint64_t)((sbo_bytes >> 4) & 0x3fff) << 32;
  return d;
}
__device__ __forceinline__ uint64_t smem_desc_mnmajor_noswz(uint32_t saddr, uint32_t lbo_bytes, uint32_t sbo_bytes) {
  return smem_desc_kmajor_noswz(saddr, lbo_bytes, sbo_bytes);
}

}

int mnb_make_tmap(CUtensorMap* out, const void* base, int elem_bytes, int rank, const uint64_t* dims,
                  const uint32_t* box);
int mnb_make_tmap_strided(CUtensorMap* out, const void* base, int elem_bytes, int rank, const uint64_t* dims,
                          const uint64_t* strides_bytes, const uint32_t* box);
```

### micronet_b200/functional.py

```python
from __future__ import annotations

import ctypes as C

import torch
from torch.autograd import Function

from . import _lib as L


class KernelTimer:

    def __init__(self):
        self.records = []

    def run(self, kind, sh, fn):
        a, b = torch.cuda.Event(enable_timing=True), torch.cuda.Event(enable_timing=True)
        a.record()
        rc = fn()
        b.record()
        self.records.append((kind, tuple(getattr(sh, f) for f, _ in sh._fields_), a, b))
        return rc

    def summary(self):
        out = {}
# ... 82 lines not shown
    @staticmethod
    def forward(ctx, a, b, spec: ActSpec, relu=False):
        L.require_cuda(a, b)
        lib = L.load()
        a, b = a.contiguous(), b.contiguous()
        assert a.shape == b.shape, "QuantAdd: operand shapes differ"
        n = a.numel()
        out = torch.empty_like(a)
        words = (n + 31) // 32
        ba = torch.empty(words, dtype=torch.int32, device=a.device) if ctx.needs_input_grad[0] else None
        bb = torch.empty(words, dtype=torch.int32, device=a.device) if ctx.needs_input_grad[1] else None
        qp = spec.struct()
        assert not (relu and (ba is not None or bb is not None)), "the folded ReLU is an inference-only fusion"
        L.check(lib.mnb_quant_add_fwd(a.data_ptr(), b.data_ptr(), n, C.byref(qp), out.data_ptr(), L.ptr(ba), L.ptr(bb),
                                      1 if relu else 0, L.stream()), "quant_add_fwd")
        ctx.spec, ctx.ba, ctx.bb = spec.frozen() if (ba is not None or bb is not None) else spec, ba, bb
        return out

    @staticmethod
    def backward(ctx, g):
        lib = L.load()
        g = g.contiguous()
        da = torch.empty_like(g) if ctx.ba is not None else None
        db = torch.empty_like(g) if ctx.bb is not None else None
        qp = ctx.spec.struct()
        L.check(lib.mnb_quant_add_bwd(g.data_ptr(), L.ptr(ctx.ba), L.ptr(ctx.bb), g.numel(), C.byref(qp), L.ptr(da),
                                      L.ptr(db), L.stream()), "quant_add_bwd")
        return da, db, None, None


class DorefaWeightFn(Function):
    @staticmethod
    def forward(ctx, w, w_bits):
        L.require_cuda(w)
        lib = L.load()
        w = w.contiguous()
        n, k = w.numel(), w.shape[0]
        wq = torch.empty_like(w)
        w_int = torch.empty(w.shape, dtype=torch.int16, device=w.device)
        w_scale = torch.empty(k, dtype=torch.float32, device=w.device)
        aux = torch.empty(n + 4, dtype=torch.float32, device=w.device)
        L.check(lib.mnb_dorefa_weight_fwd(w.data_ptr(), n, k, w_bits, w_int.data_ptr(), w_scale.data_ptr(),
                                          wq.data_ptr(), aux.data_ptr(), L.scratch(w.device).data_ptr(),
                                          L.stream()), "dorefa_weight_fwd")
        ctx.aux, ctx.w_bits = aux, w_bits
        ctx.mark_non_differentiable(w_int, w_scale)
        return wq, w_int, w_scale

    @staticmethod
    def backward(ctx, g, _gi, _gs):
        lib = L.load()
        g = g.contiguous()
        dw = torch.empty_like(g)
        L.check(lib.mnb_dorefa_weight_bwd(g.data_ptr(), ctx.aux.data_ptr(), g.numel(), ctx.w_bits,
                                          dw.data_ptr(), L.scratch(g.device).data_ptr(), L.stream()),
                "dorefa_weight_bwd")
        return dw, None


class WbWeightFn(Function):

    @staticmethod
    def forward(ctx, w, W):
        L.require_cuda(w)
        lib = L.load()
        assert w.is_contiguous() and w.dim() == 4
        k, cpg, khw = w.shape[0], w.shape[1], w.shape[2] * w.shape[3]
        wq = torch.empty_like(w)
        w_int = torch.empty(w.shape, dtype=torch.int16, device=w.device)
        w_scale = torch.empty(k, dtype=torch.float32, device=w.device)
        aux = torch.empty(3 * k, dtype=torch.float32, device=w.device)
        L.check(lib.mnb_wb_weight_fwd(w.data_ptr(), k, cpg, khw, W, w_int.data_ptr(), w_scale.data_ptr(),
                                      wq.data_ptr(), aux.data_ptr(), L.stream()), "wb_weight_fwd")
        ctx.w, ctx.aux, ctx.W = w.detach(), aux, W
        ctx.mark_non_differentiable(w_int, w_scale)
        return wq, w_int, w_scale

    @staticmethod
    def backward(ctx, g, _gi, _gs):
        lib = L.load()
        g = g.contiguous()
        w = ctx.w
        dw = torch.empty_like(g)
        L.check(lib.mnb_wb_weight_bwd(g.data_ptr(), w.data_ptr(), ctx.aux.data_ptr(), w.shape[0], w.shape[1],
                                      w.shape[2] * w.shape[3], ctx.W, dw.data_ptr(), L.stream()),
                "wb_weight_bwd")
        return dw, None


class IaoWeightFn(Function):

    @staticmethod
    def forward(ctx, w, scale, zero_point, obs_min, obs_max, q_type, qmin, qmax):
        L.require_cuda(w)
        lib = L.load()
        w = w.contiguous()
        n, k, rows = w.numel(), w.shape[0], scale.numel()
        wq = torch.empty_like(w)
        w_int = torch.empty(w.shape, dtype=torch.int16, device=w.device)
        w_scale = torch.empty(k, dtype=torch.float32, device=w.device)
        keep = torch.empty(w.shape, dtype=torch.uint8, device=w.device)
        L.check(lib.mnb_iao_weight_fwd(w.data_ptr(), n, k, rows, scale.data_ptr(), zero_point.data_ptr(),
                                       obs_min.data_ptr(), obs_max.data_ptr(), q_type, qmin, qmax,
                                       w_int.data_ptr(), w_scale.data_ptr(), wq.data_ptr(), keep.data_ptr(),
                                       L.stream()), "iao_weight_fwd")
        ctx.keep, ctx.scale, ctx.k, ctx.rows = keep, scale, k, rows
        ctx.mark_non_differentiable(w_int, w_scale)
        return wq, w_int, w_scale

    @staticmethod
    def backward(ctx, g, _gi, _gs):
        lib = L.load()
        g = g.contiguous()
        dw = torch.empty_like(g)
        L.check(lib.mnb_iao_weight_bwd(g.data_ptr(), ctx.keep.data_ptr(), ctx.scale.data_ptr(), g.numel(),
                                       ctx.k, ctx.rows, dw.data_ptr(), L.stream()), "iao_weight_bwd")
        return (dw,) + (None,) * 7


def _shape_struct(x_shape, w_shape, stride, padding, dilation, groups):
    b, c, h, w = x_shape
    k, _, r, s = w_shape
    return L.ConvShape(b, c, h, w, k, r, s, stride[0], stride[1], padding[0], padding[1],
                       dilation[0], dilation[1], groups)


def _out_hw(sh: L.ConvShape):
    p = (sh.in_h + 2 * sh.pad_h - sh.dil_h * (sh.ker_h - 1) - 1) // sh.stride_h + 1
    q = (sh.in_w + 2 * sh.pad_w - sh.dil_w * (sh.ker_w - 1) - 1) // sh.stride_w + 1
    return p, q


def channel_sums(x4):
    lib = L.load()
    b, c = x4.shape[0], x4.shape[1]
    hw = x4.numel() // (b * c)
    out = torch.empty(2 * c, dtype=torch.float32, device=x4.device)
    L.check(lib.mnb_channel_stats(x4.data_ptr(), b, c, hw, 0, out.data_ptr(),
                                  L.scratch(x4.device, c).data_ptr(), L.stream()), "channel_stats")
    return out[:c]



def materialized(t):
    xbits = getattr(t, "_mnb_xbits", None)
    if xbits is not None:
        from . import xnor as XN
        return XN.unpack(xbits[1], t.shape, xbits[3])
    codes = getattr(t, "_mnb_codes", None)
    if codes is not None:
        b, c = t.shape[0], t.shape[1]
        out = torch.empty(t.shape, dtype=torch.float32, device=t.device)
        L.check(L.load().mnb_codes_decode(codes[0].data_ptr(), codes[1].data_ptr(), b, c, t.numel() // (b * c), out.data_ptr(),
                                          L.stream()), "codes_decode")
        return out
    if not getattr(t, "_mnb_plane_only", False):
        return t
    b, c, h, w = t.shape
    plane = t._mnb_pk_pm1.view(torch.bfloat16).view(b, c // 8, h, w, 8)
    return plane.permute(0, 1, 4, 2, 3).reshape(b, c, h, w).float()


def xnor_preferred(sh, has_plane):
    return not has_plane


def _pk_terms(spec, w_int, pm1=False):
    T = L.PK_TERMS
    if spec is None:
        ta = 1 if pm1 else T
    else:
        ta = 2 if (spec.mode == L.ACT_IAO and spec.q_type == 1) else 1
    return ta, (1 if w_int is not None else T)


def _pk_forward(ctx, x, wq, bias, w_int, w_scale, spec, sh, y, prepacked=None, pre_relu=False, pm1=False, codes_out=False):
    from . import pk as PK
    need_dx, need_dw = ctx.needs_input_grad[0], ctx.needs_input_grad[1]
    ta, tw = _pk_terms(spec, w_int, pm1)
    if not PK.supported(sh, 0, ta, tw):
        return False
    Tb = min(L.PK_TERMS, L.PK_TERMS_BWD)
    if need_dx and not PK.supported(sh, 1, Tb, 1 if w_int is not None else Tb):
        return False
    if need_dw and not PK.wgrad_supported(sh, Tb, min(ta, Tb)):
        return False
    qp = spec.struct() if spec is not None else None
    if prepacked is not None:
        x_pk, bits8 = prepacked, None
    else:
        x_pk, bits8 = PK.pack_act(x, qp, ta, phase_split=sh.stride_h == 2, want_bits=need_dx, relu=pre_relu,
                                  groups=sh.groups)
    w_img = PK.weight_image(sh, ta, tw, w_int=w_int, w_f32=None if w_int is not None else wq)
    a_scale, a_const = PK.act_scale(spec, clone=need_dx or need_dw)
    rc = L.E_UNSUPPORTED
    if codes_out and w_int is not None and ta == 1 and tw == 1:
        codes = torch.empty(y.shape, dtype=torch.int16, device=y.device)
        dec = torch.empty(2 * y.shape[1], dtype=torch.float32, device=y.device)
        rc = _timed("fwd_pk", sh, lambda: PK.run_conv_codes(sh, x_pk, w_img, codes, dec, n_scale=w_scale, a_scale=a_scale,
                                                            a_scale_const=a_const, bias=bias))
        if rc == 0:
            y._mnb_codes = (codes, dec)
    if rc == L.E_UNSUPPORTED:
        rc = _timed("fwd_pk", sh, lambda: PK.run_conv(sh, 0, x_pk, ta, w_img, tw, y,
                                                      n_scale=w_scale if w_int is not None else None, a_scale=a_scale,
                                                      a_scale_const=a_const, bias=bias))
    if rc == L.E_UNSUPPORTED:
        return False
    L.check(rc, "pk_conv fwd")
    ctx.pk_x, ctx.pk_ta, ctx.pk_bits8, ctx.pk_prepacked = x_pk, ta, bits8, prepacked is not None
    ctx.pk_gain = 0.1 if (spec is not None and spec.mode == L.ACT_DOREFA) else 1.0
    ctx.pk_wg_scale = None
    if spec is not None:
        ctx.pk_wg_scale = a_scale if spec.mode == L.ACT_IAO else _dorefa_scale_tensor(spec.bits, x.device)
    if spec is None and w_int is not None and need_dw and not PK.padded(sh.out_c, sh.groups):
        y._mnb_pk_conv = (w_scale if need_dx else None, Tb)
    return True


def _pk_backward(ctx, dy):
    from . import pk as PK
    sh = ctx.sh
    T = min(L.PK_TERMS, L.PK_TERMS_BWD)
    int_w = ctx.w_int is not None
    need_dx, need_dw = ctx.needs_input_grad[0], ctx.needs_input_grad[1]
    fold = int_w and need_dx
    pre = getattr(dy, "_mnb_pk_dy", None)
    if pre is not None:
        if pre[1] != T or (pre[2] is not None) != fold or PK.padded(sh.out_c, sh.groups):
            raise RuntimeError("micronet_b200: packed gradient operand does not match this layer's backward configuration")
        dy_pk = pre[0]
    else:
        dy_pk, _ = PK.pack_act(dy, None, T, ch_scale=ctx.w_scale if fold else None, groups=sh.groups)
    dx = dwq = None
    if need_dx:
        tw = 1 if int_w else T
        w_img = PK.pack_weight(sh, 1, T, tw, w_int=ctx.w_int, w_f32=None if int_w else ctx.wq,
                               kzero=ctx.w_scale if int_w else None)
        dx = torch.empty((sh.batch, sh.in_c, sh.in_h, sh.in_w), dtype=torch.float32, device=dy.device)
        plain_gain = ctx.pk_gain if ctx.pk_prepacked else 1.0
        L.check(_timed("dgrad_pk", sh, lambda: PK.run_conv(sh, 1, dy_pk, T, w_img, tw, dx, bits8=ctx.pk_bits8, gain=ctx.pk_gain,
                                                           a_scale_const=plain_gain)), "pk_conv dgrad")
    if need_dw:
        dwq = torch.empty_like(ctx.wq)
        tx = min(ctx.pk_ta, T)
        kdiv = ctx.w_scale if fold else None
        L.check(_timed("wgrad_pk", sh, lambda: PK.run_wgrad(sh, dy_pk, T, ctx.pk_x, tx, dwq, a_scale=ctx.pk_wg_scale,
                                                            kdiv=kdiv)), "pk_wgrad")
    return dx, dwq


def _xnor_forward(x, w_int, w_scale, bias, sh, y, groups):
    from . import xnor as XN
    if not (XN.supported(sh) and (L.XNOR_MODE == "all" or xnor_preferred(sh, getattr(x, "_mnb_pk_pm1", None) is not None))):
        return False
    a_bits = XN.pack_act(materialized(x), groups)
    rc = _timed("fwd_xnor", sh, lambda: XN.conv(sh, a_bits, XN.pack_weight(sh, w_int), y, alpha=w_scale, bias=bias))
    if rc == L.E_UNSUPPORTED:
        return False
    L.check(rc, "xnor_conv_fwd")
    return True


def _save_unpacked(ctx, x, spec, codes, bits, keep_x):
    if spec is not None and (ctx.needs_input_grad[0] or ctx.needs_input_grad[1]):
        spec = spec.frozen()
    ctx.spec, ctx.codes, ctx.bits = spec, codes, bits
    ctx.x = x if keep_x else None


def _act_operands(spec, codes, x):
    ops = L.ConvOperands()
    if codes is None:
        ops.a_f32 = x.data_ptr()
        return ops
    ops.a_codes, ops.a_offset = codes.data_ptr(), spec.code_offset
    if spec.mode == L.ACT_IAO:
        ops.a_offset_zp, ops.a_scale = L.ptr(spec.zero_point), L.ptr(spec.scale)
    elif spec.mode == L.ACT_DOREFA:
        ops.a_scale = _dorefa_scale_tensor(spec.bits, codes.device).data_ptr()
    return ops


def _tc_forward(ctx, x, w_int, w_scale, bias, spec, sh, y):
    lib = L.load()
    qp = codes = bits = None
    if spec is not None:
        qp = spec.struct()
        codes = torch.empty(x.shape, dtype=torch.uint8, device=x.device)
        if ctx.needs_input_grad[0]:
            bits = torch.zeros((x.numel() + 31) // 32, dtype=torch.int32, device=x.device)
    wpack = torch.empty(w_int.numel(), dtype=torch.int16, device=x.device)
    rc = _timed("fwd_tc", sh, lambda: lib.mnb_fq_conv2d_fwd_tc(
        C.byref(sh), x.data_ptr(), None if qp is None else C.byref(qp), w_int.data_ptr(),
        w_scale.data_ptr(), L.ptr(bias), y.data_ptr(), L.ptr(codes), L.ptr(bits), wpack.data_ptr(),
        L.tc_err_flag(x.device).data_ptr(), L.stream()))
    if rc == L.E_UNSUPPORTED:
        return False
    L.check(rc, "fq_conv2d_fwd_tc")
    _save_unpacked(ctx, x, spec, codes, bits, keep_x=True)
    return True


def _fconv_forward(ctx, x, wq, bias, sh, y):
    lib = L.load()
    rc = _timed("fconv_fwd_tc", sh, lambda: lib.mnb_fconv2d_fwd_tc(
        C.byref(sh), x.data_ptr(), wq.data_ptr(), L.ptr(bias), y.data_ptr(), L.tc_err_flag(x.device).data_ptr(), L.stream()))
    if rc == L.E_UNSUPPORTED:
        return False
    L.check(rc, "fconv2d_fwd_tc")
    _save_unpacked(ctx, x, None, None, None, keep_x=True)
    return True


def _generic_forward(ctx, x, wq, bias, w_int, w_scale, spec, sh, y, keep_x):
    lib = L.load()
    codes = bits = None
    if spec is not None:
        codes, bits, _ = act_quant_raw(x, spec, True, ctx.needs_input_grad[0], False)
    ops = _act_operands(spec, codes, x)
    if codes is not None and w_int is not None:
        ops.w_int, ops.w_scale = w_int.data_ptr(), w_scale.data_ptr()
    else:
        ops.w_f32 = wq.data_ptr()
    ops.bias = L.ptr(bias)
    L.check(_timed("fwd", sh, lambda: lib.mnb_conv2d_fwd(C.byref(sh), C.byref(ops), y.data_ptr(), L.stream())), "conv2d_fwd")
    _save_unpacked(ctx, x, spec, codes, bits, keep_x=keep_x or codes is None)


def _dgrad(ctx, dy, tc):
    lib = L.load()
    sh, spec = ctx.sh, ctx.spec
    dx = torch.empty((sh.batch, sh.in_c, sh.in_h, sh.in_w), dtype=torch.float32, device=dy.device)
    qp = spec.struct() if spec is not None else None
    bits_ptr = ctx.bits.data_ptr() if spec is not None else None
    rc = L.E_UNSUPPORTED
    if tc:
        wpack = torch.empty(ctx.w_int.numel(), dtype=torch.int16, device=dy.device)
        rc = _timed("dgrad_tc", sh, lambda: lib.mnb_conv2d_dgrad_tc(
            C.byref(sh), dy.data_ptr(), ctx.w_int.data_ptr(), ctx.w_scale.data_ptr(), bits_ptr,
            None if qp is None else C.byref(qp), dx.data_ptr(), wpack.data_ptr(),
            L.tc_err_flag(dy.device).data_ptr(), L.stream()))
    if rc == L.E_UNSUPPORTED:
        rc = _timed("dgrad", sh, lambda: lib.mnb_conv2d_dgrad(
            C.byref(sh), dy.data_ptr(), ctx.wq.data_ptr(), bits_ptr, None if qp is None else C.byref(qp),
            dx.data_ptr(), L.stream()))
    L.check(rc, "conv2d_dgrad")
    return dx


def _wgrad(ctx, dy, tc):
    lib = L.load()
    sh, spec = ctx.sh, ctx.spec
    dwq = torch.empty_like(ctx.wq)
    ops = _act_operands(spec, ctx.codes, ctx.x)
    nbytes = int(lib.mnb_wgrad_scratch_bytes(C.byref(sh)))
    tbytes = int(lib.mnb_wgrad_tc_scratch_bytes(C.byref(sh))) if tc else 0
    if tbytes > 0:
        qp = spec.struct() if spec is not None else None
        ws = torch.empty(max(tbytes, nbytes, 4), dtype=torch.uint8, device=dy.device)
        inexact = torch.zeros(1, dtype=torch.int32, device=dy.device)
        rc = _timed("wgrad_tc", sh, lambda: lib.mnb_conv2d_wgrad_tc(
            C.byref(sh), dy.data_ptr(), ctx.x.data_ptr(), None if qp is None else C.byref(qp),
            dwq.data_ptr(), ws.data_ptr(), inexact.data_ptr(), L.tc_err_flag(dy.device).data_ptr(), L.stream()))
        if rc == 0:
            if spec is None:
                L.check(lib.mnb_conv2d_wgrad_cond(C.byref(sh), dy.data_ptr(), C.byref(ops), dwq.data_ptr(),
                                                  ws.data_ptr(), inexact.data_ptr(), L.stream()), "conv2d_wgrad_cond")
            return dwq
        if rc != L.E_UNSUPPORTED:
            L.check(rc, "conv2d_wgrad_tc")
    ws = torch.empty(max(nbytes, 4), dtype=torch.uint8, device=dy.device)
    L.check(_timed("wgrad", sh, lambda: lib.mnb_conv2d_wgrad(
        C.byref(sh), dy.data_ptr(), C.byref(ops), dwq.data_ptr(), ws.data_ptr(), L.stream())), "conv2d_wgrad")
    return dwq


def _fconv_wgrad(ctx, dy):
    lib = L.load()
    sh = ctx.sh
    fbytes = int(lib.mnb_fconv2d_wgrad_tc_scratch_bytes(C.byref(sh)))
    if fbytes < 0:
        return None
    dwq = torch.empty_like(ctx.wq)
    ws = torch.empty(max(fbytes, 4), dtype=torch.uint8, device=dy.device)
    L.check(_timed("fconv_wgrad_tc", sh, lambda: lib.mnb_fconv2d_wgrad_tc(
        C.byref(sh), dy.data_ptr(), ctx.x.data_ptr(), dwq.data_ptr(), ws.data_ptr(), L.tc_err_flag(dy.device).data_ptr(),
        L.stream())), "fconv2d_wgrad_tc")
    return dwq


class QuantConv2dFn(Function):

    @staticmethod
    def forward(ctx, x, wq, bias, w_int, w_scale, spec, stride, padding, dilation, groups, pre_relu=False, no_grad=False,
                codes_out=False):
        from . import pk as PK
        L.require_cuda(x, wq)
        assert not (pre_relu and any(ctx.needs_input_grad)), "the folded ReLU is an inference-only fusion"
        x = x.contiguous()
        wq = wq.contiguous()
        sh = _shape_struct(x.shape, wq.shape, stride, padding, dilation, groups)
        p, q = _out_hw(sh)
        y = torch.empty((x.shape[0], wq.shape[0], p, q), dtype=torch.float32, device=x.device)
        ctx.sh, ctx.wq, ctx.has_bias = sh, wq, bias is not None
        ctx.w_int, ctx.w_scale = (w_int, w_scale) if w_int is not None else (None, None)
        pk_on = L.PK_MODE != "off"
        pm1 = x.dtype == torch.float32 and getattr(x, "_mnb_pm1", False)
        pm1_plane = getattr(x, "_mnb_pk_pm1", None)
        padded_in = PK.padded(sh.in_c, sh.groups)
        plane = pm1_plane if (pm1_plane is not None and not padded_in and pm1_plane.numel() == x.numel() * 2) else None
        pkq = getattr(x, "_mnb_pk_q", None)
        if pkq is not None and padded_in:
            raise RuntimeError("micronet_b200: a fused producer's packed output reached a conv that reads group-padded planes")
        plane_only = getattr(x, "_mnb_plane_only", False)
        if plane_only and padded_in:
            x, plane_only = materialized(x), False
        if (L.XNOR_MODE != "off" and spec is None and w_int is not None and pm1 and not pre_relu
                and (no_grad or not any(ctx.needs_input_grad[:3])) and _xnor_forward(x, w_int, w_scale, bias, sh, y, groups)):
            family = "xnor"
        elif pkq is not None:
            if spec is None or spec.mode != L.ACT_DOREFA or spec.bits != pkq[1] or w_int is None:
                raise RuntimeError("micronet_b200: a fused producer's packed output reached a conv with another quantizer")
            if not _pk_forward(ctx, x, wq, bias, w_int, w_scale, spec, sh, y, prepacked=pkq[0]):
                raise RuntimeError("micronet_b200: fused producer output in front of a conv outside the packed-operand cover")
            family = "pk"
        elif ((pk_on and x.dtype == torch.float32 and (L.PK_MODE == "all" or spec is not None) and not plane_only
               and _pk_forward(ctx, x, wq, bias, w_int, w_scale, spec, sh, y, pre_relu=pre_relu))
              or (L.PK_WBWTAB and pk_on and spec is None and w_int is not None and pm1
                  and (pm1_plane is not None or sh.ker_h * sh.ker_w > 1 or padded_in)
                  and _pk_forward(ctx, x, wq, bias, w_int, w_scale, None, sh, y, prepacked=plane, pm1=True,
                                  codes_out=codes_out))
              or (pk_on and spec is None and w_int is None and pm1 and not pre_relu
                  and _pk_forward(ctx, x, wq, bias, None, None, None, sh, y, prepacked=plane, pm1=True))):
            family = "pk"
        else:
            if plane_only:
                x = materialized(x)
            if pre_relu:
                x = torch.relu(x)
            f32 = x.dtype == torch.float32
            if L.USE_TC and w_int is not None and f32 and _tc_forward(ctx, x, w_int, w_scale, bias, spec, sh, y):
                family = "tc"
            elif L.USE_TC and spec is None and f32 and _fconv_forward(ctx, x, wq, bias, sh, y):
                family = "fconv"
            elif pk_on and f32 and _pk_forward(ctx, x, wq, bias, w_int, w_scale, spec, sh, y):
                family = "pk"
            else:
                tc = L.USE_TC and w_int is not None
                _generic_forward(ctx, x, wq, bias, w_int, w_scale, spec, sh, y, keep_x=tc)
                family = "tc" if tc else "generic"
        ctx.family = family
        return y

    @staticmethod
    def backward(ctx, dy):
        presummed = getattr(dy, "_mnb_channel_sum", None)
        dy = dy.contiguous()
        need_dx, need_dw = ctx.needs_input_grad[0], ctx.needs_input_grad[1]
        db = None
        if ctx.has_bias and ctx.needs_input_grad[2]:
            db = presummed if presummed is not None and presummed.numel() == dy.shape[1] else channel_sums(dy)
        dx = dwq = None
        if ctx.family == "pk":
            dx, dwq = _pk_backward(ctx, dy)
        elif ctx.family == "tc":
            dx = _dgrad(ctx, dy, tc=True) if need_dx else None
            dwq = _wgrad(ctx, dy, tc=True) if need_dw else None
        elif ctx.family == "fconv":
            tc = ctx.w_int is not None
            dx = _dgrad(ctx, dy, tc) if need_dx else None
            if need_dw:
                dwq = _fconv_wgrad(ctx, dy)
                if dwq is None:
                    dwq = _wgrad(ctx, dy, tc)
        else:
            dx = _dgrad(ctx, dy, tc=False) if need_dx else None
            dwq = _wgrad(ctx, dy, tc=False) if need_dw else None
        return dx, dwq, db, None, None, None, None, None, None, None, None, None, None


def quant_conv2d(x, wq, bias, w_int, w_scale, spec, stride, padding, dilation, groups, pre_relu=False, codes_out=False):
    return QuantConv2dFn.apply(x, wq, bias, w_int, w_scale, spec, tuple(stride), tuple(padding),
                               tuple(dilation), groups, pre_relu, not torch.is_grad_enabled(), codes_out)


def _pk_plain(sh, mode, a, w, out, T):
    from . import pk as PK
    if L.PK_MODE == "off" or PK.padded_conv(sh) or not PK.supported(sh, mode, T, T):
        return False
    a_pk, _ = PK.pack_act(a, None, T, phase_split=(mode == 0 and sh.stride_h == 2))
    w_img = PK.pack_weight(sh, mode, T, T, w_f32=w)
    rc = _timed("fwd_pk" if mode == 0 else "dgrad_pk", sh, lambda: PK.conv(sh, mode, a_pk, T, w_img, T, out))
    if rc == L.E_UNSUPPORTED:
        return False
    L.check(rc, "pk_conv (plain)")
    return True


class ConvTranspose2dFn(Function):

    @staticmethod
    def forward(ctx, x, w, bias, stride, padding, output_padding, groups, dilation):
        L.require_cuda(x, w)
        L.require_f32(x, w)
        lib = L.load()
        x, w = x.contiguous(), w.contiguous()
        b, cin, h, wd = x.shape
        if w.shape[0] != cin or cin % groups:
            raise ValueError("conv_transpose2d: weight must be [C_in, C_out / groups, R, S]")
        cout = w.shape[1] * groups
        oh = (h - 1) * stride[0] - 2 * padding[0] + dilation[0] * (w.shape[2] - 1) + output_padding[0] + 1
        ow = (wd - 1) * stride[1] - 2 * padding[1] + dilation[1] * (w.shape[3] - 1) + output_padding[1] + 1
        sh = _shape_struct((b, cout, oh, ow), w.shape, stride, padding, dilation, groups)
        if _out_hw(sh) != (h, wd):
            raise ValueError("conv_transpose2d: output_padding must be smaller than the stride")
        y = torch.empty((b, cout, oh, ow), dtype=torch.float32, device=x.device)
        if not _pk_plain(sh, 1, x, w, y, L.PK_TERMS):
            L.check(_timed("dgrad", sh, lambda: lib.mnb_conv2d_dgrad(C.byref(sh), x.data_ptr(), w.data_ptr(), None, None,
                                                                      y.data_ptr(), L.stream())), "conv2d_dgrad")
        if bias is not None:
            y += bias.view(1, -1, 1, 1)
        ctx.save_for_backward(x, w)
        ctx.sh, ctx.has_bias = sh, bias is not None
        return y

    @staticmethod
    def backward(ctx, gy):
        from . import pk as PK
        lib = L.load()
        x, w = ctx.saved_tensors
        sh = ctx.sh
        gy = gy.contiguous()
        gx = gw = gb = None
        T = min(L.PK_TERMS, L.PK_TERMS_BWD)
        if ctx.needs_input_grad[0]:
            gx = torch.empty_like(x)
            if not _pk_plain(sh, 0, gy, w, gx, T):
                ops = L.ConvOperands()
                ops.a_f32, ops.w_f32 = gy.data_ptr(), w.data_ptr()
                L.check(_timed("fwd", sh, lambda: lib.mnb_conv2d_fwd(C.byref(sh), C.byref(ops), gx.data_ptr(), L.stream())),
                        "conv2d_fwd")
        if ctx.needs_input_grad[1]:
            gw = torch.empty_like(w)
            done = False
            if L.PK_MODE != "off" and not PK.padded_conv(sh) and PK.wgrad_supported(sh, T, T):
                x_pk, _ = PK.pack_act(x, None, T)
                g_pk, _ = PK.pack_act(gy, None, T, phase_split=sh.stride_h == 2)
                rc = _timed("wgrad_pk", sh, lambda: PK.wgrad(sh, x_pk, T, g_pk, T, gw))
                if rc != L.E_UNSUPPORTED:
                    L.check(rc, "pk_wgrad (transposed conv)")
                    done = True
            if not done:
                ops = L.ConvOperands()
                ops.a_f32 = gy.data_ptr()
                ws = torch.empty(max(int(lib.mnb_wgrad_scratch_bytes(C.byref(sh))), 4), dtype=torch.uint8, device=gy.device)
                L.check(_timed("wgrad", sh, lambda: lib.mnb_conv2d_wgrad(C.byref(sh), x.data_ptr(), C.byref(ops), gw.data_ptr(),
                                                                         ws.data_ptr(), L.stream())), "conv2d_wgrad")
        if ctx.has_bias and ctx.needs_input_grad[2]:
            gb = channel_sums(gy)
        return gx, gw, gb, None, None, None, None, None


def conv_transpose2d(x, w, bias, stride, padding, output_padding, groups, dilation):
    return ConvTranspose2dFn.apply(x, w, bias, tuple(stride), tuple(padding), tuple(output_padding), groups, tuple(dilation))


class Consumer:

    def __init__(self, module, spec, relu, only, w_shape, stride, padding, dilation, groups, int_weights, int8=False, bn=None,
                 shuffle_groups=1, pool=None, post_spec=None, formats=None):
        self.module, self.spec, self.relu, self.only = module, spec, bool(relu), bool(only)
        self.w_shape, self.stride, self.padding, self.dilation, self.groups = w_shape, stride, padding, dilation, groups
        self.int_weights, self.int8 = int_weights, bool(int8)
        self.bn, self.sg, self.pool = bn, int(shuffle_groups), pool
        self.target = module if pool is None else pool[0]
        self.post_spec = spec if post_spec is None else post_spec
        self.formats = formats

    def read_shape(self, out_shape):
        if self.pool is None:
            return tuple(out_shape)
        _, k, s, p = self.pool
        b, c, h, w = out_shape
        return (b, c, (h + 2 * p - k) // s + 1, (w + 2 * p - k) // s + 1)

    def format(self, out_shape):
        act_shape = self.read_shape(out_shape)
        if self.sg > 1 and (out_shape[1] % 16 or out_shape[1] % self.sg or self.split):
            return None
        fmt = None
        if self.int8 and act_shape[1] == self.w_shape[1] * self.groups:
            sh = _shape_struct(act_shape, self.w_shape, self.stride, self.padding, self.dilation, self.groups)
            if _i8_route(self.spec, self.int_weights, sh):
                fmt = "i8"
        if fmt is None and self.accepts(act_shape):
            fmt = "bf16"
        return fmt if self.formats is None or fmt in self.formats else None

    def accepts(self, act_shape):
        from . import pk as PK
        sp = self.spec
        if sp is None or not self.int_weights or not (2 <= sp.bits <= 8) or _pk_terms(sp, True)[0] != 1:
            return False
        if act_shape[1] != self.w_shape[1] * self.groups:
            return False
        if PK.padded(act_shape[1], self.groups):
            return False
        sh = _shape_struct(act_shape, self.w_shape, self.stride, self.padding, self.dilation, self.groups)
        if sh.stride_h == 2 and ((act_shape[2] | act_shape[3]) & 1):
            return False
        return L.PK_MODE != "off" and PK.supported(sh, 0, 1, 1)

    @property
    def split(self):
        return self.stride[0] == 2 and self.pool is None


def handed_plane(module, x):
    pre = getattr(x, "_mnb_pk_pre", None)
    if pre is not None and pre[0] is module and (x.device.type == "meta" or x._version == pre[2]):
        return pre[1]
    if x.device.type == "meta":
        raise RuntimeError("micronet_b200: a plane-only producer output reached a module it was not produced for")
    return None


def _tag(y, consumer, plane, fmt="bf16"):
    y._mnb_pk_pre = (consumer.target, plane, y._version, fmt)
    return y


def _i8_route(spec, w_int, sh):
    from . import pk as PK
    if spec is None or w_int is None or L.PK_MODE == "off":
        return False
    if spec.mode == L.ACT_DOREFA:
        ok = 2 <= spec.bits <= 7
    else:
        ok = spec.mode == L.ACT_IAO and spec.q_type == 0 and 2 <= spec.bits <= 8 and -128 <= spec.qmin and spec.qmax <= 127
    return ok and PK.i8_supported(sh)


def _i8_producer_writes_plane(out_channels, groups):
    return groups == 1 or (out_channels // groups) % 16 == 0


@torch.no_grad()
def frozen_conv(x, plane, wq, bias, w_int, w_scale, spec, stride, padding, dilation, groups, pre_relu=False, consumer=None,
                int8=False):
    from . import pk as PK
    stride, padding, dilation = tuple(stride), tuple(padding), tuple(dilation)
    sh = _shape_struct(x.shape, wq.shape, stride, padding, dilation, groups)
    p, q = _out_hw(sh)
    out_shape = (x.shape[0], wq.shape[0], p, q)
    fmt = "i8" if int8 and _i8_route(spec, w_int, sh) else "bf16"
    if plane is not None and x._mnb_pk_pre[3] != fmt:
        raise RuntimeError(f"micronet_b200: a {x._mnb_pk_pre[3]} operand plane reached a conv that reads {fmt}")
    cfmt = consumer.format(out_shape) if consumer is not None else None
    if fmt == "i8":
        hand = cfmt == "i8" and _i8_producer_writes_plane(wq.shape[0], groups)
        return _frozen_conv_i8(x, plane, bias, w_int, w_scale, spec, sh, out_shape, pre_relu, consumer if hand else None)
    ta, tw = _pk_terms(spec, w_int)
    fused = cfmt == "bf16" and not PK.segmented(sh, 0, ta, tw) and not PK.padded(sh.out_c, groups)
    if (plane is None and not fused) or spec is None or w_int is None or L.PK_MODE == "off" or not PK.supported(sh, 0, ta, tw):
        if plane is not None:
            raise RuntimeError("micronet_b200: handed-over plane in front of a conv outside the packed-operand cover")
        return quant_conv2d(x, wq, bias, w_int, w_scale, spec, stride, padding, dilation, groups, pre_relu=pre_relu)
    dev = wq.device
    if plane is None:
        L.require_cuda(x, wq)
        plane, _ = PK.pack_act(x.contiguous(), spec.struct(), ta, phase_split=sh.stride_h == 2, relu=pre_relu, groups=groups)
    w_img = PK.weight_image(sh, ta, tw, w_int=w_int)
    a_scale, a_const = PK.act_scale(spec)
    if not fused:
        y = torch.empty(out_shape, dtype=torch.float32, device=dev)
        L.check(_timed("fwd_pk", sh, lambda: PK.conv(sh, 0, plane, ta, w_img, tw, y, n_scale=w_scale, a_scale=a_scale,
                                                     a_scale_const=a_const, bias=bias)), "pk_conv fwd")
        return y
    y = None if consumer.only else torch.empty(out_shape, dtype=torch.float32, device=dev)
    cplane = PK.consumer_plane(*out_shape, dev)
    cqp = consumer.post_spec.struct()
    L.check(_timed("fwd_pk", sh, lambda: PK.conv_post(sh, plane, ta, w_img, tw, y, cqp, cplane, consumer.relu, consumer.split,
                                                      n_scale=w_scale, a_scale=a_scale, a_scale_const=a_const, bias=bias,
                                                      bn=consumer.bn, shuffle_groups=consumer.sg)),
            "pk_conv_post")
    if y is None:
        y = torch.empty(out_shape, dtype=torch.float32, device="meta")
    return _tag(y, consumer, cplane)


def _frozen_conv_i8(x, plane, bias, w_int, w_scale, spec, sh, out_shape, pre_relu, consumer):
# ... 121 lines not shown
```

### micronet_b200/fused.py

```python
from __future__ import annotations

import torch
import torch.nn as nn
from torch.autograd import Function

import ctypes as C

import torch.nn.functional as TF

from . import _lib as L
from . import pk as PK


def _xargs(lib, name, x, codes):
    if codes is None:
        return getattr(lib, name), (x.data_ptr(),)
    return getattr(lib, name + "_codes"), (codes[0].data_ptr(), codes[1].data_ptr())


class BNSignFn(Function):

    @staticmethod
    def forward(ctx, x, gamma, beta, mean, invstd, training, shuffle_groups, pool, plane_only=False):
        from . import functional as F_
        lib = L.load()
        x = x.contiguous()
        b, c = x.shape[0], x.shape[1]
        hw = x.numel() // (b * c)
        pk_conv = getattr(x, "_mnb_pk_conv", None)
        codes = getattr(x, "_mnb_codes", None)
        write_plane = L.PK_WBWTAB and c % 8 == 0 and hw % 32 == 0 and x.dim() == 4 and L.PK_MODE != "off"
        if codes is not None and not pool and not write_plane:
            x, codes = F_.materialized(x), None
        bits = torch.empty((x.numel() + 31) // 32, dtype=torch.int32, device=x.device)
        arg = None
        if pool:
            h, w = x.shape[2], x.shape[3]
            y = torch.empty((b, c, h // 2, w // 2), dtype=x.dtype, device=x.device)
            arg = torch.empty(y.numel(), dtype=torch.uint8, device=x.device)
            fn, xa = _xargs(lib, "mnb_bn_sign_pool_fwd", x, codes)
            L.check(fn(*xa, b, c, h, w, mean.data_ptr(), invstd.data_ptr(), gamma.data_ptr(), beta.data_ptr(), shuffle_groups,
                       y.data_ptr(), bits.data_ptr(), arg.data_ptr(), L.stream()), "bn_sign_pool_fwd")
        else:
            y = torch.empty_like(x)
            written = False
            if write_plane:
                plane = torch.empty(x.numel() * 2, dtype=torch.uint8, device=x.device)
                skip_y = bool(plane_only) and L.PLANE_ONLY
                fn, xa = _xargs(lib, "mnb_bn_sign_fwd_packed", x, codes)
                rc = fn(*xa, b, c, hw, mean.data_ptr(), invstd.data_ptr(), gamma.data_ptr(), beta.data_ptr(), shuffle_groups,
                        None if skip_y else y.data_ptr(), bits.data_ptr(), plane.data_ptr(), L.stream())
                if rc == 0:
                    y._mnb_pk_pm1 = plane
                    if skip_y:
                        y._mnb_plane_only = True
                    written = True
                elif rc != L.E_UNSUPPORTED:
                    L.check(rc, "bn_sign_fwd_packed")
                elif codes is not None:
                    x, codes = F_.materialized(x), None
            if not written:
                L.check(lib.mnb_bn_sign_fwd(x.data_ptr(), b, c, hw, mean.data_ptr(), invstd.data_ptr(), gamma.data_ptr(),
                                            beta.data_ptr(), shuffle_groups, y.data_ptr(), bits.data_ptr(), L.stream()),
                        "bn_sign_fwd")
        y._mnb_pm1 = True
        ctx.save_for_backward(x, gamma, mean, invstd)
        ctx.bits, ctx.arg, ctx.training, ctx.shuffle_groups = bits, arg, training, shuffle_groups
        ctx.pk_conv, ctx.codes = pk_conv, codes
        return y

    @staticmethod
    def backward(ctx, g):
        lib = L.load()
        x, gamma, mean, invstd = ctx.saved_tensors
        g = g.contiguous()
        b, c = x.shape[0], x.shape[1]
        hw = x.numel() // (b * c)
        dx = torch.empty_like(x)
        out = torch.empty(3 * c, dtype=torch.float32, device=x.device)
        dgamma, dbeta, dx_sum = out[:c], out[c:2 * c], out[2 * c:]
        scratch = L.scratch(x.device, c)
        if (ctx.arg is not None and ctx.pk_conv is not None and ctx.training and c % 8 == 0 and x.shape[3] % 8 == 0
                and x.shape[2] % 2 == 0):
            w_scale, T = ctx.pk_conv
            fn, xa = _xargs(lib, "mnb_bn_sign_pool_bwd", x, ctx.codes)
            L.check(fn(g.data_ptr(), ctx.bits.data_ptr(), ctx.arg.data_ptr(), *xa, b, c, x.shape[2], x.shape[3],
                       mean.data_ptr(), invstd.data_ptr(), gamma.data_ptr(), 2, ctx.shuffle_groups, dx.data_ptr(),
                       dgamma.data_ptr(), dbeta.data_ptr(), None, scratch.data_ptr(), L.stream()), "bn_sign_pool_bwd (reduce)")
            dy_pk = torch.empty(T * x.numel() * 2, dtype=torch.uint8, device=x.device)
            fn, xa = _xargs(lib, "mnb_bn_sign_pool_bwd_pack", x, ctx.codes)
            L.check(fn(g.data_ptr(), ctx.bits.data_ptr(), ctx.arg.data_ptr(), *xa, b, c, x.shape[2], x.shape[3],
                       mean.data_ptr(), invstd.data_ptr(), gamma.data_ptr(), dgamma.data_ptr(), dbeta.data_ptr(),
                       ctx.shuffle_groups, L.ptr(w_scale), T, dy_pk.data_ptr(), L.stream()), "bn_sign_pool_bwd_pack")
            dx_sum.zero_()
            dx._mnb_pk_dy = (dy_pk, T, w_scale)
        elif ctx.arg is not None:
            fn, xa = _xargs(lib, "mnb_bn_sign_pool_bwd", x, ctx.codes)
            L.check(fn(g.data_ptr(), ctx.bits.data_ptr(), ctx.arg.data_ptr(), *xa, b, c, x.shape[2], x.shape[3],
                       mean.data_ptr(), invstd.data_ptr(), gamma.data_ptr(), 1 if ctx.training else 0, ctx.shuffle_groups,
                       dx.data_ptr(), dgamma.data_ptr(), dbeta.data_ptr(), dx_sum.data_ptr(), scratch.data_ptr(), L.stream()),
                    "bn_sign_pool_bwd")
        elif ctx.pk_conv is not None and ctx.training and c % 8 == 0:
            w_scale, T = ctx.pk_conv
            fn, xa = _xargs(lib, "mnb_bn_sign_bwd", x, ctx.codes)
            L.check(fn(g.data_ptr(), ctx.bits.data_ptr(), *xa, b, c, hw, mean.data_ptr(), invstd.data_ptr(), gamma.data_ptr(),
                       2, ctx.shuffle_groups, dx.data_ptr(), dgamma.data_ptr(), dbeta.data_ptr(), None, scratch.data_ptr(),
                       L.stream()), "bn_sign_bwd (reduce)")
            dy_pk = torch.empty(T * x.numel() * 2, dtype=torch.uint8, device=x.device)
            fn, xa = _xargs(lib, "mnb_bn_sign_bwd_pack", x, ctx.codes)
            L.check(fn(g.data_ptr(), ctx.bits.data_ptr(), *xa, b, c, hw, mean.data_ptr(), invstd.data_ptr(), gamma.data_ptr(),
                       dgamma.data_ptr(), dbeta.data_ptr(), ctx.shuffle_groups, L.ptr(w_scale), T, None, dy_pk.data_ptr(),
                       L.stream()), "bn_sign_bwd_pack")
            dx_sum.zero_()
            dx._mnb_pk_dy = (dy_pk, T, w_scale)
        else:
            fn, xa = _xargs(lib, "mnb_bn_sign_bwd", x, ctx.codes)
            L.check(fn(g.data_ptr(), ctx.bits.data_ptr(), *xa, b, c, hw, mean.data_ptr(), invstd.data_ptr(), gamma.data_ptr(),
                       1 if ctx.training else 0, ctx.shuffle_groups, dx.data_ptr(), dgamma.data_ptr(), dbeta.data_ptr(),
                       dx_sum.data_ptr(), scratch.data_ptr(), L.stream()), "bn_sign_bwd")
        dx._mnb_channel_sum = dx_sum
        return dx, dgamma, dbeta, None, None, None, None, None, None


class BatchNormBinarize2d(nn.BatchNorm2d):

    out_shuffle_groups = 1
    pool2 = False
    plane_only = False

    def forward(self, input):
        frozen = self.__dict__.get("_mnb_xnor")
        if frozen is not None:
            return frozen(self, input)
        return self._forward(input)

    def _forward(self, input):
        L.require_cuda(input, self.weight)
        L.require_f32(input, self.weight)
        assert self.affine and self.track_running_stats and self.momentum is not None, \
            "BatchNormBinarize2d supports affine BN with running statistics and a float momentum"
        if self.training:
            lib = L.load()
            x = input.detach().contiguous()
            b, c = x.shape[0], x.shape[1]
            stats = torch.empty(2 * c, dtype=torch.float32, device=x.device)
            fn, xa = _xargs(lib, "mnb_bn_batch_stats", x, getattr(input, "_mnb_codes", None))
            L.check(fn(*xa, b, c, x.numel() // (b * c), float(self.eps), float(self.momentum), self.running_mean.data_ptr(),
                       self.running_var.data_ptr(), self.num_batches_tracked.data_ptr(), stats.data_ptr(),
                       L.scratch(x.device, c).data_ptr(), L.stream()), "bn_batch_stats")
            mean, invstd = stats[:c], stats[c:]
        else:
            mean = self.running_mean
            invstd = torch.rsqrt(self.running_var + self.eps)
        sg = int(self.out_shuffle_groups)
        if self.pool2 and (input.dim() != 4 or input.shape[2] % 2 or input.shape[3] % 8):
            y = BNSignFn.apply(input, self.weight, self.bias, mean, invstd, self.training, 1, False)
            return MaxPoolFn.apply(y, 2, 2, 0, sg)
        return BNSignFn.apply(input, self.weight, self.bias, mean, invstd, self.training, sg, bool(self.pool2),
                              bool(self.plane_only) and not self.pool2)

    def extra_repr(self):
        return super().extra_repr() + f", pool2={self.pool2}, out_shuffle_groups={self.out_shuffle_groups}"



class BNReluQuantFn(Function):

    @staticmethod
    def forward(ctx, x, gamma, beta, mean, invstd, training, shuffle_groups, a_bits):
        from . import functional as F_
        lib = L.load()
        x = x.contiguous()
        b, c = x.shape[0], x.shape[1]
        hw = x.numel() // (b * c)
        bits = torch.empty((x.numel() + 31) // 32, dtype=torch.int32, device=x.device)
        packed = torch.empty(x.numel() * 2, dtype=torch.uint8, device=x.device)
        qp = F_.ActSpec(L.ACT_DOREFA, bits=a_bits).struct()
        L.check(lib.mnb_bn_relu_quant_pack_fwd(x.data_ptr(), b, c, hw, mean.data_ptr(), invstd.data_ptr(), gamma.data_ptr(),
                                               beta.data_ptr(), C.byref(qp), shuffle_groups, packed.data_ptr(),
                                               bits.data_ptr(), L.stream()), "bn_relu_quant_pack_fwd")
        y = torch.empty_like(x)
        y._mnb_pk_q = (packed, a_bits)
        ctx.save_for_backward(x, gamma, mean, invstd)
        ctx.bits, ctx.training, ctx.shuffle_groups = bits, training, shuffle_groups
        return y

    @staticmethod
    def backward(ctx, g):
        lib = L.load()
        x, gamma, mean, invstd = ctx.saved_tensors
        g = g.contiguous()
        b, c = x.shape[0], x.shape[1]
        hw = x.numel() // (b * c)
        dx = torch.empty_like(x)
        out = torch.empty(3 * c, dtype=torch.float32, device=x.device)
        dgamma, dbeta, dx_sum = out[:c], out[c:2 * c], out[2 * c:]
        L.check(lib.mnb_bn_sign_bwd(g.data_ptr(), ctx.bits.data_ptr(), x.data_ptr(), b, c, hw, mean.data_ptr(),
                                    invstd.data_ptr(), gamma.data_ptr(), 1 if ctx.training else 0, ctx.shuffle_groups,
                                    dx.data_ptr(), dgamma.data_ptr(), dbeta.data_ptr(), dx_sum.data_ptr(),
                                    L.scratch(x.device, c).data_ptr(), L.stream()), "bn_sign_bwd")
        dx._mnb_channel_sum = dx_sum
        return dx, dgamma, dbeta, None, None, None, None, None


class BatchNormReluQuant2d(nn.BatchNorm2d):

    out_shuffle_groups = 1
    a_bits = 8

    def forward(self, input):
        L.require_cuda(input, self.weight)
        L.require_f32(input, self.weight)
        b, c = input.shape[0], input.shape[1]
        hw = input.numel() // max(1, b * c)
        sg = int(self.out_shuffle_groups)
        if input.dim() != 4 or c % 8 or hw % 32:
            y = TF.relu(super().forward(input))
            if sg > 1:
                y = y.view(b, sg, c // sg, *y.shape[2:]).transpose(1, 2).contiguous().view_as(y)
            return y
        if self.training:
            lib = L.load()
            x = input.detach().contiguous()
            stats = torch.empty(2 * c, dtype=torch.float32, device=x.device)
            L.check(lib.mnb_bn_batch_stats(x.data_ptr(), b, c, hw, float(self.eps), float(self.momentum),
                                           self.running_mean.data_ptr(), self.running_var.data_ptr(),
                                           self.num_batches_tracked.data_ptr(), stats.data_ptr(),
                                           L.scratch(x.device, c).data_ptr(), L.stream()), "bn_batch_stats")
            mean, invstd = stats[:c], stats[c:]
        else:
            mean = self.running_mean
            invstd = torch.rsqrt(self.running_var + self.eps)
        return BNReluQuantFn.apply(input, self.weight, self.bias, mean, invstd, self.training, sg, int(self.a_bits))

    def extra_repr(self):
        return super().extra_repr() + f", relu + dorefa a_bits={self.a_bits}, out_shuffle_groups={self.out_shuffle_groups}"


class MaxPoolFn(Function):
    @staticmethod
    def forward(ctx, x, k, s, p, shuffle_groups):
        lib = L.load()
        x = x.contiguous()
        b, c, h, w = x.shape
        oh, ow = (h + 2 * p - k) // s + 1, (w + 2 * p - k) // s + 1
        y = torch.empty((b, c, oh, ow), dtype=x.dtype, device=x.device)
        arg = torch.empty(y.numel(), dtype=torch.uint8, device=x.device)
        L.check(lib.mnb_maxpool2d_fwd(x.data_ptr(), b, c, h, w, k, s, p, shuffle_groups, y.data_ptr(), arg.data_ptr(),
                                      L.stream()), "maxpool2d_fwd")
        ctx.arg, ctx.cfg = arg, (b, c, h, w, k, s, p, shuffle_groups)
        return y

    @staticmethod
    def backward(ctx, g):
        lib = L.load()
        b, c, h, w, k, s, p, sg = ctx.cfg
        g = g.contiguous()
        dx = torch.empty((b, c, h, w), dtype=g.dtype, device=g.device)
        L.check(lib.mnb_maxpool2d_bwd(g.data_ptr(), ctx.arg.data_ptr(), b, c, h, w, k, s, p, sg, dx.data_ptr(),
                                      L.stream()), "maxpool2d_bwd")
        return dx, None, None, None, None


def _pool_cfg(m: nn.MaxPool2d):
    def one(v):
        if isinstance(v, (tuple, list)):
            return int(v[0]) if len(set(v)) == 1 else None
        return int(v)
    k, s, p, d = one(m.kernel_size), one(m.stride if m.stride is not None else m.kernel_size), one(m.padding), one(m.dilation)
    if None in (k, s, p, d) or d != 1 or m.ceil_mode or m.return_indices or k > 15 or 2 * p > k:
        return None
    return k, s, p


class EngineMaxPool2d(nn.MaxPool2d):
    out_shuffle_groups = 1

    def forward(self, input):
        L.require_cuda(input)
        L.require_f32(input)
        k, s, p = _pool_cfg(self)
        return MaxPoolFn.apply(input, k, s, p, int(self.out_shuffle_groups))

    def extra_repr(self):
        return super().extra_repr() + f", out_shuffle_groups={self.out_shuffle_groups}"


class FloatConvFn(Function):

    @staticmethod
    def forward(ctx, x, w, bias, padding):
        lib = L.load()
        x, w = x.contiguous(), w.contiguous()
        b, c, h, wd = x.shape
        k, _, r, s_ = w.shape
        sh = L.ConvShape(b, c, h, wd, k, r, s_, 1, 1, padding, padding, 1, 1, 1)
        y = torch.empty((b, k, h, wd), dtype=torch.float32, device=x.device)
        rc = lib.mnb_fconv2d_fwd_tc(C.byref(sh), x.data_ptr(), w.data_ptr(), L.ptr(bias), y.data_ptr(),
                                    L.tc_err_flag(x.device).data_ptr(), L.stream())
        ctx.engine = rc == 0
        if rc == L.E_UNSUPPORTED:
            y = TF.conv2d(x, w, bias, 1, padding)
        elif rc != 0:
            L.check(rc, "fconv2d_fwd_tc")
        ctx.save_for_backward(x, w)
        ctx.sh, ctx.padding, ctx.has_bias = sh, padding, bias is not None
        return y

    @staticmethod
    def backward(ctx, dy):
        lib = L.load()
        x, w = ctx.saved_tensors
        presummed = getattr(dy, "_mnb_channel_sum", None)
        dy = dy.contiguous()
        dx = dw = db = None
        if ctx.needs_input_grad[0]:
            dx = torch.nn.grad.conv2d_input(x.shape, w, dy, 1, ctx.padding)
        if ctx.needs_input_grad[1]:
            need = int(lib.mnb_fconv2d_wgrad_tc_scratch_bytes(C.byref(ctx.sh))) if ctx.engine else -1
            if need >= 0:
                dw = torch.empty_like(w)
                scratch = torch.empty(need, dtype=torch.uint8, device=dy.device)
                L.check(lib.mnb_fconv2d_wgrad_tc(C.byref(ctx.sh), dy.data_ptr(), x.data_ptr(), dw.data_ptr(),
                                                 scratch.data_ptr(), L.tc_err_flag(dy.device).data_ptr(), L.stream()),
                        "fconv2d_wgrad_tc")
            else:
                dw = torch.nn.grad.conv2d_weight(x, w.shape, dy, 1, ctx.padding)
        if ctx.has_bias and ctx.needs_input_grad[2]:
            if presummed is not None and presummed.numel() == dy.shape[1]:
                db = presummed
            else:
                from .functional import channel_sums
                db = channel_sums(dy)
        return dx, dw, db, None


def _float_conv_cover(m: nn.Conv2d) -> bool:
    k, p = m.kernel_size, m.padding
    return (type(m) is nn.Conv2d and m.groups == 1 and tuple(m.stride) == (1, 1) and tuple(m.dilation) == (1, 1)
            and k[0] == k[1] and k[0] % 2 == 1 and not isinstance(p, str) and tuple(p) == (k[0] // 2, k[0] // 2)
            and m.padding_mode == "zeros" and m.in_channels * k[0] * k[1] <= 128 and m.out_channels <= 256)


class EngineFloatConv2d(nn.Conv2d):

    def forward(self, input):
        L.require_cuda(input, self.weight)
        L.require_f32(input, self.weight)
        return FloatConvFn.apply(input, self.weight, self.bias, int(self.padding[0]))


class EnginePmConv2d(nn.Conv2d):

    def forward(self, input):
        from . import functional as F_, pk as PK
        if (getattr(input, "_mnb_pm1", False) and L.PK_MODE != "off" and input.is_cuda and input.dtype == torch.float32
                and input.dim() == 4 and self.padding_mode == "zeros" and not isinstance(self.padding, str)):
            sh = F_._shape_struct(input.shape, self.weight.shape, self.stride, self.padding, self.dilation, self.groups)
            T, Tb = L.PK_TERMS, min(L.PK_TERMS, L.PK_TERMS_BWD)
            if (PK.supported(sh, 0, 1, T) and PK.supported(sh, 1, Tb, Tb) and PK.wgrad_supported(sh, Tb, 1)):
                return F_.quant_conv2d(input, self.weight, self.bias, None, None, None, self.stride, self.padding,
                                       self.dilation, self.groups)
        from . import functional as F2
        return self._conv_forward(F2.materialized(input), self.weight, self.bias)


def _fuse_pairs(module: nn.Module):
    from .wbwtab import ActivationQuantizer
    prev_name, prev = None, None
    for name, child in list(module.named_children()):
        if (isinstance(child, ActivationQuantizer) and child.A == 2 and type(prev) is nn.BatchNorm2d
                and prev.affine and prev.track_running_stats and prev.momentum is not None):
            fused = BatchNormBinarize2d(prev.num_features, eps=prev.eps, momentum=prev.momentum)
            fused.weight, fused.bias = prev.weight, prev.bias
            fused.running_mean, fused.running_var = prev.running_mean, prev.running_var
            fused.num_batches_tracked = prev.num_batches_tracked
            fused.train(prev.training)
            module._modules[prev_name] = fused
            module._modules[name] = nn.Identity()
        elif type(child) is nn.Conv2d and _float_conv_cover(child):
            conv = EngineFloatConv2d(child.in_channels, child.out_channels, child.kernel_size, child.stride, child.padding,
                                     child.dilation, child.groups, child.bias is not None)
            conv.weight, conv.bias = child.weight, child.bias
            module._modules[name] = conv
        elif type(child) is nn.Conv2d and child.in_channels % 8 == 0 and child.in_channels >= 64:
            conv = EnginePmConv2d(child.in_channels, child.out_channels, child.kernel_size, child.stride, child.padding,
                                  child.dilation, child.groups, child.bias is not None, child.padding_mode)
            conv.weight, conv.bias = child.weight, child.bias
            module._modules[name] = conv
        elif type(child) is nn.MaxPool2d and _pool_cfg(child) is not None:
            pool = EngineMaxPool2d(child.kernel_size, child.stride, child.padding, child.dilation,
                                   child.return_indices, child.ceil_mode)
            module._modules[name] = pool
        else:
            _fuse_pairs(child)
        prev_name, prev = name, module._modules[name]


def _tail_producer(m: nn.Module):
    if isinstance(m, (BatchNormBinarize2d, BatchNormReluQuant2d, EngineMaxPool2d)):
        return m
    if hasattr(m, "channel_shuffle_flag"):
        kids = [k for k in m.children() if not isinstance(k, nn.Identity)]
        if kids and isinstance(kids[-1], (BatchNormBinarize2d, BatchNormReluQuant2d)):
            return kids[-1]
    return None


def _fold_pools(module: nn.Module):
    for child in module.children():
        _fold_pools(child)
    if not isinstance(module, nn.Sequential):
        return
    names = [n for n, k in module.named_children() if not isinstance(k, nn.Identity)]
    for pn, cn in zip(names, names[1:]):
        prev, cur = module._modules[pn], module._modules[cn]
        if not isinstance(cur, EngineMaxPool2d) or _pool_cfg(cur) != (2, 2, 0) or cur.out_shuffle_groups != 1:
            continue
        prod = _tail_producer(prev)
        if isinstance(prod, BatchNormBinarize2d) and not prod.pool2 and prod.out_shuffle_groups == 1:
            prod.pool2 = True
            module._modules[cn] = nn.Identity()


def _fold_shuffles(module: nn.Module):
    for child in module.children():
        _fold_shuffles(child)
    if not isinstance(module, nn.Sequential):
        return
    kids = [k for k in module.children() if not isinstance(k, nn.Identity)]
    for prev, blk in zip(kids, kids[1:]):
        groups = int(getattr(blk, "shuffle_groups", 1))
        if not getattr(blk, "channel_shuffle_flag", 0) or groups <= 1:
            continue
        prod = _tail_producer(prev)
        if prod is None or prod.out_shuffle_groups != 1:
            continue
        prod.out_shuffle_groups = groups
        blk.channel_shuffle_flag = 0


def _first_conv(m: nn.Module):
    if isinstance(m, nn.Conv2d):
        return m
    if hasattr(m, "channel_shuffle_flag"):
        kids = [k for k in m.children() if not isinstance(k, nn.Identity)]
        if kids and isinstance(kids[0], nn.Conv2d):
            return kids[0]
    return None


def _fuse_dorefa_producers(module: nn.Module):
    from .dorefa import QuantConv2d as DorefaConv
    for child in module.children():
        _fuse_dorefa_producers(child)
    if not isinstance(module, nn.Sequential) or "mnb_bn_relu_quant_pack_fwd" not in L.PROTOTYPES:
        return
    kids = [k for k in module.children() if not isinstance(k, nn.Identity)]
    for prev, nxt in zip(kids, kids[1:]):
        conv = _first_conv(nxt)
        a_bits = int(conv.activation_quantizer.a_bits) if isinstance(conv, DorefaConv) else 0
        if not (2 <= a_bits <= 8) or conv.in_channels % 8 or tuple(conv.stride) != (1, 1) or conv.quant_inference:
            continue
        if PK.padded(conv.in_channels, conv.groups):
            continue
        if not hasattr(prev, "channel_shuffle_flag"):
            continue
        names = [n for n, k in prev.named_children() if not isinstance(k, nn.Identity)]
        if len(names) < 2:
            continue
        bn, act = prev._modules[names[-2]], prev._modules[names[-1]]
        if type(bn) is not nn.BatchNorm2d or type(act) is not nn.ReLU:
            continue
        if not (bn.affine and bn.track_running_stats and bn.momentum is not None):
            continue
        fused = BatchNormReluQuant2d(bn.num_features, eps=bn.eps, momentum=bn.momentum)
        fused.weight, fused.bias = bn.weight, bn.bias
        fused.running_mean, fused.running_var = bn.running_mean, bn.running_var
        fused.num_batches_tracked = bn.num_batches_tracked
        fused.a_bits = a_bits
        fused.train(bn.training)
        prev._modules[names[-2]] = fused
        prev._modules[names[-1]] = nn.Identity()


def _mark_plane_only(module: nn.Module):
    from .wbwtab import QuantConv2d as WbConv
    for child in module.children():
        _mark_plane_only(child)
    if not isinstance(module, nn.Sequential):
        return
    kids = [k for k in module.children() if not isinstance(k, nn.Identity)]
    for prev, nxt in zip(kids, kids[1:]):
        prod, conv = _tail_producer(prev), _first_conv(nxt)
        if not isinstance(prod, BatchNormBinarize2d) or prod.pool2 or conv is None:
            continue
        if getattr(nxt, "channel_shuffle_flag", 0) or conv.in_channels % 8 or PK.padded(conv.in_channels, conv.groups):
            continue
        if isinstance(conv, WbConv):
            ok = conv.weight_quantizer.W in (2, 3) and not conv.quant_inference
        else:
            ok = isinstance(conv, EnginePmConv2d)
        if ok:
            prod.plane_only = True


def _mark_codes_out(module: nn.Module):
    from .pk import codes_fit
    from .wbwtab import QuantConv2d as WbConv
    for m in module.modules():
        if not hasattr(m, "channel_shuffle_flag"):
            continue
        kids = [k for k in m.children() if not isinstance(k, nn.Identity)]
        if len(kids) != 2 or not isinstance(kids[0], WbConv) or not isinstance(kids[1], BatchNormBinarize2d):
            continue
        conv = kids[0]
        if conv.weight_quantizer.W in (2, 3) and not conv.quant_inference and codes_fit(conv.in_channels, conv.groups,
                                                                                        conv.kernel_size):
            conv.codes_out = True


def fuse_wbwtab_blocks(model: nn.Module, fold_shuffle: bool = True) -> nn.Module:
    _fuse_pairs(model)
    _fold_pools(model)
    _fuse_dorefa_producers(model)
    if fold_shuffle:
        _fold_shuffles(model)
    _mark_plane_only(model)
    _mark_codes_out(model)
    return model


fuse_blocks = fuse_wbwtab_blocks
fuse_bn_binarize = fuse_wbwtab_blocks
```

Before: 39620.

## Add two-warpgroup warp-specialized fp32 stem conv forward and wgrad kernels

Adds new forward and weight-gradient kernels for the float stem convolution. They use warp specialization: producer warps build split-bf16 im2col tiles in shared memory while two WGMMA consumer warpgroups alternate over tiles with wide N (192/256), coordinated through mbarriers and setmaxnreg register rebalancing. The Python paths now try these kernels first and fall back to the older single-warpgroup TC kernels when the shape is unsupported. The aim is to overlap patch construction with tensor-core work and cover all output channels in one MMA pass, at the cost of extra code, larger shared-memory use, and one block per SM.

New measurement: 41670 (median of 6 runs). 5.2% higher.

```diff
diff --git a/harness/fconv_probe.py b/harness/fconv_probe.py
--- a/harness/fconv_probe.py
+++ b/harness/fconv_probe.py
@@ -1,51 +1,113 @@
+import argparse
 import ctypes as C
-import os
+import statistics
 import subprocess
-import sys
 
 import torch
 
+STEMS = {"ningc_stem": (3, 32, 32, 256, 5), "nin_stem": (3, 32, 32, 192, 5), "res_stem": (3, 32, 32, 64, 3)}
+HBM_BPS, BF16_FLOPS = 3.35e12, 989e12
+NSETS = 4
 
-def run():
+
+def card():
+    try:
+        q = subprocess.run(["nvidia-smi", "--query-gpu=name,power.limit,clocks.sm,clocks.max.sm", "--format=csv,noheader"],
+                           capture_output=True, text=True, timeout=30).stdout.strip().splitlines()
+        return q[0] if q else torch.cuda.get_device_name()
+    except (OSError, subprocess.SubprocessError):
+        return torch.cuda.get_device_name()
+
+
+def window_us(fn, launches):
+    e0, e1 = torch.cuda.Event(enable_timing=True), torch.cuda.Event(enable_timing=True)
+    e0.record()
+    for i in range(launches):
+        fn(i % NSETS)
+    e1.record()
+    torch.cuda.synchronize()
+    return e0.elapsed_time(e1) * 1e3 / launches
+
+
+def ab(fns, windows, launches):
+    for fn in fns.values():
+        for i in range(2 * NSETS):
+            fn(i % NSETS)
+    torch.cuda.synchronize()
+    times = {k: [] for k in fns}
+    for _ in range(windows):
+        for k, fn in fns.items():
+            times[k].append(window_us(fn, launches))
+    return {k: statistics.median(v) for k, v in times.items()}
+
+
+def run_stem(lib, L, name, B, windows, launches):
+    Cc, H, W, K, R = STEMS[name]
+    dev = torch.device("cuda")
+    g = torch.Generator(device=dev).manual_seed(0)
+    xs = [torch.randn(B, Cc, H, W, device=dev, generator=g) for _ in range(NSETS)]
+    ws = [torch.randn(K, Cc, R, R, device=dev, generator=g) * 0.1 for _ in range(NSETS)]
+    bs = [torch.randn(K, device=dev, generator=g) for _ in range(NSETS)]
+    dys = [torch.randn(B, K, H, W, device=dev, generator=g) for _ in range(NSETS)]
+    y_old = torch.empty(B, K, H, W, device=dev)
+    y_new = torch.empty_like(y_old)
+    dw_old = torch.empty_like(ws[0])
+    dw_new = torch.empty_like(ws[0])
+    sh = L.ConvShape(B, Cc, H, W, K, R, R, 1, 1, R // 2, R // 2, 1, 1, 1)
+    scratch = torch.empty(int(lib.mnb_fconv2d_wgrad_tc_scratch_bytes(C.byref(sh))), dtype=torch.uint8, device=dev)
+    has_fwd = lib.mnb_fconv2d_wg_plan(C.byref(sh), None, 0) == 0
+    has_wg = int(lib.mnb_fconv2d_wgrad_wg_scratch_bytes(C.byref(sh))) >= 0
+    err = L.tc_err_flag(dev)
+
+    def fwd(entry, y):
+        return lambda i: L.check(entry(C.byref(sh), xs[i].data_ptr(), ws[i].data_ptr(), bs[i].data_ptr(), y.data_ptr(),
+                                       err.data_ptr(), L.stream()), name)
+
+    def wgrad(entry, dw):
+        return lambda i: L.check(entry(C.byref(sh), dys[i].data_ptr(), xs[i].data_ptr(), dw.data_ptr(),
+                                       scratch.data_ptr(), err.data_ptr(), L.stream()), name)
+
+    fns = {"fwd_tc": fwd(lib.mnb_fconv2d_fwd_tc, y_old), "wgrad_tc": wgrad(lib.mnb_fconv2d_wgrad_tc, dw_old)}
+    if has_fwd:
+        fns["fwd_wg"] = fwd(lib.mnb_fconv2d_fwd_wg, y_new)
+    if has_wg:
+        fns["wgrad_wg"] = wgrad(lib.mnb_fconv2d_wgrad_wg, dw_new)
+    t = ab(fns, windows, launches)
+    same = True
+    for i in range(NSETS):
+        for old, new, out_old, out_new in (("fwd_tc", "fwd_wg", y_old, y_new), ("wgrad_tc", "wgrad_wg", dw_old, dw_new)):
+            if new in fns:
+                out_new.fill_(float("nan"))
+                fns[old](i)
+                fns[new](i)
+                torch.cuda.synchronize()
+                same &= torch.equal(out_old.view(torch.int32), out_new.view(torch.int32))
+    assert int(err.item()) == 0, f"error flag {int(err.item())}"
+    big = B * K * H * W * 4
+    flops = 2 * B * H * W * K * ((Cc * R * R + 15) // 16 * 16) * 6
+    hbm, tens = big / HBM_BPS * 1e6, flops / BF16_FLOPS * 1e6
+    cols = []
+    for old, new in (("fwd_tc", "fwd_wg"), ("wgrad_tc", "wgrad_wg")):
+        cols.append(f"{old} {t[old]:.1f} us" + (f" {new} {t[new]:.1f} us ({t[old] / t[new]:.2f}x)" if new in t else ""))
+    print(f"{name} B={B}: floors hbm {hbm:.0f} us, tensor {tens:.0f} us | {'  '.join(cols)} | outputs byte-equal: {same}",
+          flush=True)
+    return same
+
+
+def main():
+    ap = argparse.ArgumentParser()
+    ap.add_argument("--batch", type=int, default=256)
+    ap.add_argument("--windows", type=int, default=5)
+    ap.add_argument("--launches", type=int, default=50)
+    ap.add_argument("--stems", default=",".join(STEMS))
+    a = ap.parse_args()
     from micronet_b200 import _lib as L
     lib = L.load()
-    B, Cc, H, W, K, R = 256, 3, 32, 32, 256, 5
-    dev = torch.device("cuda")
-    x = torch.randn(B, Cc, H, W, device=dev)
-    w = torch.randn(K, Cc, R, R, device=dev) * 0.1
-    b = torch.randn(K, device=dev)
-    y = torch.empty(B, K, H, W, device=dev)
-    dy = torch.randn(B, K, H, W, device=dev)
-    dw = torch.empty_like(w)
-    sh = L.ConvShape(B, Cc, H, W, K, R, R, 1, 1, R // 2, R // 2, 1, 1, 1)
-    scratch = torch.empty(int(lib.mnb_fconv2d_wgrad_tc_scratch_bytes(C.byref(sh))), dtype=torch.uint8, device=dev)
-    err = L.tc_err_flag(dev)
-
-    def fwd():
-        L.check(lib.mnb_fconv2d_fwd_tc(C.byref(sh), x.data_ptr(), w.data_ptr(), b.data_ptr(), y.data_ptr(), err.data_ptr(),
-                                       L.stream()), "fwd")
-
-    def wg():
-        L.check(lib.mnb_fconv2d_wgrad_tc(C.byref(sh), dy.data_ptr(), x.data_ptr(), dw.data_ptr(), scratch.data_ptr(),
-                                         err.data_ptr(), L.stream()), "wgrad")
-    out = []
-    for name, fn in (("fwd", fwd), ("wgrad", wg)):
-        for _ in range(3):
-            fn()
-        torch.cuda.synchronize()
-        e0, e1 = torch.cuda.Event(enable_timing=True), torch.cuda.Event(enable_timing=True)
-        e0.record()
-        for _ in range(10):
-            fn()
-        e1.record()
-        torch.cuda.synchronize()
-        out.append(f"{name} {e0.elapsed_time(e1) * 100:.1f}us")
-    print(os.environ.get("MNB_FCONV_DEBUG", "0"), " ".join(out), flush=True)
+    print("card:", card(), flush=True)
+    ok = all([run_stem(lib, L, s, a.batch, a.windows, a.launches) for s in a.stems.split(",")])
+    print("card:", card(), flush=True)
+    raise SystemExit(0 if ok else 1)
 
 
 if __name__ == "__main__":
-    if len(sys.argv) > 1:
-        run()
-    else:
-        for mask in (0, 1, 2, 4, 8, 3, 7, 9, 15):
-            subprocess.run([sys.executable, __file__, "child"], env=dict(os.environ, MNB_FCONV_DEBUG=str(mask)), timeout=120)
+    main()
diff --git a/include/micronet_b200.h b/include/micronet_b200.h
--- a/include/micronet_b200.h
+++ b/include/micronet_b200.h
@@ -151,7 +151,13 @@
 int mnb_fconv2d_plan(const mnb_conv_shape* s, int32_t wgrad, int32_t* out, int32_t n);
 int mnb_fconv2d_fwd_tc(const mnb_conv_shape* s, const float* x, const float* w, const float* bias, float* y,
                        int32_t* err_flag, mnb_stream_t stream);
+int mnb_fconv2d_wg_plan(const mnb_conv_shape* s, int32_t* out, int32_t n);
+int mnb_fconv2d_fwd_wg(const mnb_conv_shape* s, const float* x, const float* w, const float* bias, float* y,
+                       int32_t* err_flag, mnb_stream_t stream);
 int64_t mnb_fconv2d_wgrad_tc_scratch_bytes(const mnb_conv_shape* s);
+int64_t mnb_fconv2d_wgrad_wg_scratch_bytes(const mnb_conv_shape* s);
+int mnb_fconv2d_wgrad_wg(const mnb_conv_shape* s, const float* dy, const float* x, float* dw, void* scratch,
+                         int32_t* err_flag, mnb_stream_t stream);
 int mnb_fconv2d_wgrad_tc(const mnb_conv_shape* s, const float* dy, const float* x, float* dw, void* scratch,
                          int32_t* err_flag, mnb_stream_t stream);
 
diff --git a/micronet_b200/_lib.py b/micronet_b200/_lib.py
--- a/micronet_b200/_lib.py
+++ b/micronet_b200/_lib.py
@@ -85,8 +85,12 @@
     "mnb_bn_sign_fwd_packed": (C.c_int, [_P, _I, _I, _I, _P, _P, _P, _P, _I, _P, _P, _P, _P]),
     "mnb_fconv2d_plan": (C.c_int, [_SHAPE, _I, _P, _I]),
     "mnb_fconv2d_fwd_tc": (C.c_int, [_SHAPE, _P, _P, _P, _P, _P, _P]),
+    "mnb_fconv2d_wg_plan": (C.c_int, [_SHAPE, _P, _I]),
+    "mnb_fconv2d_fwd_wg": (C.c_int, [_SHAPE, _P, _P, _P, _P, _P, _P]),
     "mnb_fconv2d_wgrad_tc_scratch_bytes": (_L, [_SHAPE]),
     "mnb_fconv2d_wgrad_tc": (C.c_int, [_SHAPE, _P, _P, _P, _P, _P, _P]),
+    "mnb_fconv2d_wgrad_wg_scratch_bytes": (_L, [_SHAPE]),
+    "mnb_fconv2d_wgrad_wg": (C.c_int, [_SHAPE, _P, _P, _P, _P, _P, _P]),
     "mnb_maxpool2d_fwd": (C.c_int, [_P, _I, _I, _I, _I, _I, _I, _I, _I, _P, _P, _P]),
     "mnb_maxpool2d_bwd": (C.c_int, [_P, _P, _I, _I, _I, _I, _I, _I, _I, _I, _P, _P]),
     "mnb_adam_step": (C.c_int, [_P, _P, _P, _P, _L, C.c_float, C.c_float, C.c_float, C.c_float, C.c_float, _I, _P]),
diff --git a/micronet_b200/csrc/mnb_conv_fp32_tc.cu b/micronet_b200/csrc/mnb_conv_fp32_tc.cu
--- a/micronet_b200/csrc/mnb_conv_fp32_tc.cu
+++ b/micronet_b200/csrc/mnb_conv_fp32_tc.cu
@@ -68,24 +68,26 @@
   const int h = h0 - p.pad + pr, w = pc - p.pad;
   return (h >= 0 && h < p.H && w >= 0 && w < p.W) ? __ldg(p.x + (((int64_t)b * p.C + c) * p.H + h) * p.W + w) : 0.f;
 }
-__device__ __forceinline__ void patch_fetch(const Params& p, int tile, int ct, int nconv, float (&v)[PF]) {
+template <int NPF = PF>
+__device__ __forceinline__ void patch_fetch(const Params& p, int tile, int ct, int nconv, float (&v)[NPF]) {
   const int b = tile / p.tiles_per_img, h0 = (tile - b * p.tiles_per_img) * p.TH;
   const int n = p.C * p.PH * p.PW;
 #pragma unroll
-  for (int k = 0; k < PF; ++k) {
+  for (int k = 0; k < NPF; ++k) {
     const int i = ct + k * nconv;
     v[k] = i < n ? patch_element(p, i, b, h0) : 0.f;
   }
 }
-__device__ __forceinline__ void patch_commit(const Params& p, float* patch, int tile, int ct, int nconv, const float (&v)[PF]) {
+template <int NPF = PF>
+__device__ __forceinline__ void patch_commit(const Params& p, float* patch, int tile, int ct, int nconv, const float (&v)[NPF]) {
   const int b = tile / p.tiles_per_img, h0 = (tile - b * p.tiles_per_img) * p.TH;
   const int n = p.C * p.PH * p.PW;
 #pragma unroll
-  for (int k = 0; k < PF; ++k) {
+  for (int k = 0; k < NPF; ++k) {
     const int i = ct + k * nconv;
     if (i < n) patch[i] = v[k];
   }
-  for (int i = ct + PF * nconv; i < n; i += nconv) patch[i] = patch_element(p, i, b, h0);
+  for (int i = ct + NPF * nconv; i < n; i += nconv) patch[i] = patch_element(p, i, b, h0);
 }
 
 constexpr int FWD_NCONV = NTHREADS - 32 - 128;
@@ -455,7 +457,356 @@
   return 0;
 }
 
+constexpr int FWG_THREADS = 384;
+constexpr int FWG_NCONV = 128;
+constexpr int FWG_PF = 6;
+constexpr int FWG_MAXBUF = 4;
+constexpr int FWG_CONV_REGS = 56, FWG_MMA_REGS = 224;
+
+struct alignas(16) FwgShared {
+  uint64_t full[FWG_MAXBUF], empty[FWG_MAXBUF];
+  uint32_t abort;
+};
+
+template <int N>
+__global__ void __launch_bounds__(FWG_THREADS, 1) fwd_wg_kernel(const Params p) {
+  extern __shared__ __align__(1024) uint8_t smem[];
+  __shared__ FwgShared sh;
+  __shared__ __align__(16) float epi_bias[N];
+  const int tid = threadIdx.x, warp = tid >> 5, lane = tid & 31;
+  uint8_t* bop = smem + p.off_b;
+  uint8_t* aop = smem + p.off_a;
+  int* tab = reinterpret_cast<int*>(smem + p.off_tab);
+  const int kchunks = p.KP / 8;
+
+  if (tid == 0) {
+    for (int i = 0; i < FWG_MAXBUF; ++i) {
+      tc::mbar_init(&sh.full[i], FWG_NCONV / 32); tc::mbar_init(&sh.empty[i], 4);
+    }
+    sh.abort = 0;
+    tc::fence_barrier_init();
+  }
+  for (int n = tid; n < N; n += FWG_THREADS) epi_bias[n] = (p.bias && n < p.K) ? __ldg(p.bias + n) : 0.f;
+  for (int i = tid; i < kchunks * N; i += FWG_THREADS) {
+    const int j = i / N, n = i - j * N;
+    float v[8];
+#pragma unroll
+    for (int e = 0; e < 8; ++e) {
+      const int kk = j * 8 + e;
+      v[e] = (n < p.K && kk < p.KR) ? __ldg(p.w + (int64_t)n * p.KR + kk) : 0.f;
+    }
+    store_split8(v, bop + (size_t)i * 16, p.b_term_bytes);
+  }
+  for (int kk = tid; kk < p.KP; kk += FWG_THREADS) {
+    int off = -1;
+    if (kk < p.KR) {
+      const int s = kk % p.R, t = kk / p.R;
+      const int r = t % p.R, c = t / p.R;
+      off = (c * p.PH + r) * p.PW + s;
+    }
+    tab[kk] = off;
+  }
+  tc::fence_proxy_async_smem();
+  __syncthreads();
+  const int n_local = (int)blockIdx.x < p.n_tiles ? (p.n_tiles - 1 - (int)blockIdx.x) / (int)gridDim.x + 1 : 0;
+
+  if (warp < FWG_NCONV / 32) {
+    asm volatile("setmaxnreg.dec.sync.aligned.u32 %0;" ::"n"(FWG_CONV_REGS));
+    const int ct = tid;
+    float* patch0 = reinterpret_cast<float*>(smem + p.off_patch);
+    const int items = 64 * kchunks;
+    const int patch_floats = p.patch_bytes / 4;
+    float pre[FWG_PF];
+    if (n_local > 0) {
+      patch_fetch(p, blockIdx.x, ct, FWG_NCONV, pre);
+      patch_commit(p, patch0, blockIdx.x, ct, FWG_NCONV, pre);
+    }
+    for (int t = 0; t < n_local; ++t) {
+      const int tile = (int)blockIdx.x + t * (int)gridDim.x;
+      const float* patch = patch0 + (size_t)(t & 1) * patch_floats;
+      conv_bar_sync(FWG_NCONV);
+      const int next = tile + (int)gridDim.x;
+      if (next < p.n_tiles) patch_fetch(p, next, ct, FWG_NCONV, pre);
+      const int ab = t % p.nbuf_a;
+      const uint32_t aph = (uint32_t)(t / p.nbuf_a) & 1u;
+      if (!tc::mbar_wait(&sh.empty[ab], aph ^ 1u, p.err, 506)) break;
+      uint8_t* abuf = aop + (size_t)ab * p.a_buf_bytes;
+      for (int i = ct; i < items; i += FWG_NCONV) {
+        const int j = i >> 6, m = i & 63;
+        const int base = (m / p.W) * p.PW + (m % p.W);
+        int off[8];
+#pragma unroll
+        for (int e = 0; e < 8; ++e) off[e] = tab[j * 8 + e];
+        float v[8];
+#pragma unroll
+        for (int e = 0; e < 8; ++e) v[e] = off[e] >= 0 ? patch[off[e] + base] : 0.f;
+        store_split8(v, abuf + (size_t)i * 16, p.a_term_bytes);
+      }
+      tc::fence_proxy_async_smem();
+      __syncwarp();
+      if (lane == 0) tc::mbar_arrive(&sh.full[ab]);
+      if (next < p.n_tiles) patch_commit(p, patch0 + (size_t)((t + 1) & 1) * patch_floats, next, ct, FWG_NCONV, pre);
+    }
+  } else {
+    asm volatile("setmaxnreg.inc.sync.aligned.u32 %0;" ::"n"(FWG_MMA_REGS));
+    const int wg = (warp - FWG_NCONV / 32) >> 2, w4 = warp & 3;
+    const int64_t plane = (int64_t)p.H * p.W;
+    const uint64_t a_desc0 = tc::smem_desc_kmajor_noswz(tc::smem_u32(aop), 64u * 16u, 128u);
+    const uint64_t b_desc0 = tc::smem_desc_kmajor_noswz(tc::smem_u32(bop), (uint32_t)N * 16u, 128u);
+    const uint32_t a_term16 = (uint32_t)p.a_term_bytes >> 4, b_term16 = (uint32_t)p.b_term_bytes >> 4;
+    const uint32_t a_buf16 = (uint32_t)p.a_buf_bytes >> 4;
+    const uint32_t a_step16 = 2u * 64u, b_step16 = 2u * (uint32_t)N;
+    const int ksteps = p.KP / 16;
+    const int fr = 16 * w4 + (lane >> 2), fc = 2 * (lane & 3);
+    for (int t = wg; t < n_local; t += 2) {
+      const int tile = (int)blockIdx.x + t * (int)gridDim.x;
+      const int ab = t % p.nbuf_a;
+      tc::mbar_wait_soft(&sh.full[ab], (uint32_t)(t / p.nbuf_a) & 1u, p.err, 505, &sh.abort);
+      float acc[N / 2];
+      tc::zero_acc(acc);
+      tc::wg_fence();
+      tc::fence_acc(acc);
+#pragma unroll
+      for (int q = 0; q < 6; ++q) {
+        const uint64_t aq = a_desc0 + (uint64_t)((uint32_t)ab * a_buf16 + (uint32_t)kProdA[q] * a_term16);
+        const uint64_t bq = b_desc0 + (uint64_t)((uint32_t)kProdB[q] * b_term16);
+        for (int ks = 0; ks < ksteps; ++ks)
+          tc::Mma<N>::template bf16<0, 0>(acc, aq + (uint64_t)((uint32_t)ks * a_step16), bq + (uint64_t)((uint32_t)ks * b_step16), 1);
+      }
+      tc::wg_commit();
+      tc::wg_wait<0>();
+      tc::fence_acc(acc);
+      __syncwarp();
+      if (lane == 0) tc::mbar_arrive(&sh.empty[ab]);
+      const int b = tile / p.tiles_per_img, h0 = (tile - b * p.tiles_per_img) * p.TH;
+      float* dst = p.y + (int64_t)b * p.K * plane + (int64_t)h0 * p.W + fr;
+#pragma unroll
+      for (int j = 0; j < N / 8; ++j) {
+        const int n = 8 * j + fc;
+        const float2 bs = *reinterpret_cast<const float2*>(&epi_bias[n]);
+        float* o = dst + (int64_t)n * plane;
+        if (n < p.K) { o[0] = __fadd_rn(acc[4 * j], bs.x); o[8] = __fadd_rn(acc[4 * j + 2], bs.x); }
+        if (n + 1 < p.K) { o[plane] = __fadd_rn(acc[4 * j + 1], bs.y); o[plane + 8] = __fadd_rn(acc[4 * j + 3], bs.y); }
+      }
+    }
+  }
+  __syncthreads();
+}
+
 static int grid_size(const Params& p) { return std::max(1, std::min(p.n_tiles, MNB_NUM_SMS)); }
+
+static int plan_wg(const mnb_conv_shape* s, Params& p, int& smem_bytes) {
+  if (int e = plan(s, false, p, smem_bytes)) return e;
+  auto unsupported = [](const char* why) { return mnb_fail(MNB_E_UNSUPPORTED, "fp32 tc conv (two warpgroups): %s", why); };
+  if (64 % p.W) return unsupported("image rows do not tile into 64 positions");
+  if (p.K <= 128) return unsupported("128 output channels or fewer");
+  p.TH = 64 / p.W;
+  p.PH = p.TH + 2 * p.pad;
+  p.tiles_per_img = p.H / p.TH;
+  p.n_tiles = p.B * p.tiles_per_img;
+  p.patch_bytes = (p.C * p.PH * p.PW * 4 + 8 * 4 + 15) / 16 * 16;
+  p.NP = p.K <= 192 ? 192 : 256;
+  const int kchunks = p.KP / 8;
+  p.b_term_bytes = kchunks * p.NP * 16;
+  p.a_term_bytes = kchunks * 64 * 16;
+  p.a_buf_bytes = 3 * p.a_term_bytes;
+  p.off_b = 0;
+  p.off_a = 3 * p.b_term_bytes;
+  for (p.nbuf_a = FWG_MAXBUF; p.nbuf_a >= 3; --p.nbuf_a) {
+    p.off_patch = p.off_a + p.nbuf_a * p.a_buf_bytes;
+    p.off_tab = p.off_patch + 2 * p.patch_bytes;
+    smem_bytes = p.off_tab + p.KP * 4;
+    if (smem_bytes <= kMaxDynSmem) break;
+  }
+  if (p.nbuf_a < 3) return unsupported("shared memory budget (3 im2col buffers)");
+  return 0;
+}
+
+template <int N>
+static int launch_fwd_wg(const Params& p, int smem_bytes, mnb_stream_t stream) {
+  static bool attr_set = false;
+  if (!attr_set) {
+    cudaError_t ce = cudaFuncSetAttribute(fwd_wg_kernel<N>, cudaFuncAttributeMaxDynamicSharedMemorySize, kMaxDynSmem);
+    if (ce != cudaSuccess) return mnb_fail((int)ce, "cudaFuncSetAttribute: %s", cudaGetErrorString(ce));
+    attr_set = true;
+  }
+  fwd_wg_kernel<N><<<grid_size(p), FWG_THREADS, smem_bytes, (cudaStream_t)stream>>>(p);
+  MNB_LAUNCHED(1);
+  return 0;
+}
+
+constexpr int WWG_THREADS = 384;
+constexpr int WWG_NCONV = 128;
+constexpr int WWG_DMAX = 8;
+constexpr int WWG_NBUF = 3;
+constexpr int WWG_KP = 80;
+
+template <int KP>
+__global__ void __launch_bounds__(WWG_THREADS, 1) wgrad_wg_kernel(const Params p) {
+  extern __shared__ __align__(1024) uint8_t smem[];
+  __shared__ FwgShared sh;
+  const int tid = threadIdx.x, warp = tid >> 5, lane = tid & 31;
+  uint8_t* bop = smem + p.off_b;
+  uint8_t* aop = smem + p.off_a;
+  int* tab = reinterpret_cast<int*>(smem + p.off_tab);
+  const int nsub = 128 / SUB;
+  const int b_buf_bytes = 3 * p.b_term_bytes;
+
+  if (tid == 0) {
+    for (int i = 0; i < WWG_NBUF; ++i) {
+      tc::mbar_init(&sh.full[i], WWG_NCONV / 32); tc::mbar_init(&sh.empty[i], 8);
+    }
+    sh.abort = 0;
+    tc::fence_barrier_init();
+  }
+  for (int i = tid; i < WWG_NBUF * (p.a_buf_bytes + b_buf_bytes) / 16; i += WWG_THREADS)
+    reinterpret_cast<uint4*>(smem + p.off_b)[i] = make_uint4(0, 0, 0, 0);
+  for (int kk = tid; kk < p.KP; kk += WWG_THREADS) {
+    int off = -1;
+    if (kk < p.KR) {
+      const int s = kk % p.R, t = kk / p.R;
+      const int r = t % p.R, c = t / p.R;
+      off = (c * p.PH + r) * p.PW + s;
+    }
+    tab[kk] = off;
+  }
+  tc::fence_proxy_async_smem();
+  __syncthreads();
+
+  if (warp >= 4) {
+    const int wg = (warp - 4) >> 2, w4 = warp & 3;
+    const uint64_t a_desc0 = tc::smem_desc_kmajor_noswz(tc::smem_u32(aop), (uint32_t)p.NP * 16u, 128u);
+    const uint64_t b_desc0 = tc::smem_desc_kmajor_noswz(tc::smem_u32(bop), (uint32_t)KP * 16u, 128u);
+    const uint32_t a_term16 = (uint32_t)p.a_term_bytes >> 4, b_term16 = (uint32_t)p.b_term_bytes >> 4;
+    const uint32_t a_buf16 = (uint32_t)p.a_buf_bytes >> 4, b_buf16 = (uint32_t)b_buf_bytes >> 4;
+    const uint32_t a_step16 = 2u * (uint32_t)p.NP, b_step16 = 2u * (uint32_t)KP;
+    float sum0[KP / 2], sum1[KP / 2];
+    tc::zero_acc(sum0); tc::zero_acc(sum1);
+    uint32_t it = 0;
+    for (int tile = blockIdx.x; tile < p.n_tiles; tile += gridDim.x) {
+      for (int sub = 0; sub < nsub; ++sub, ++it) {
+        const uint32_t ob = it % WWG_NBUF, oph = (it / WWG_NBUF) & 1u;
+        tc::mbar_wait_soft(&sh.full[ob], oph, p.err, 515, &sh.abort);
+#pragma unroll 1
+        for (int mb = 0; mb < 2; ++mb) {
+          float acc[KP / 2];
+          tc::zero_acc(acc);
+          tc::wg_fence();
+          tc::fence_acc(acc);
+#pragma unroll
+          for (int q = 0; q < 6; ++q) {
+            const uint64_t aq = a_desc0 + (uint64_t)(ob * a_buf16 + (uint32_t)kProdA[q] * a_term16 + (uint32_t)(wg + 2 * mb) * 64u);
+            const uint64_t bq = b_desc0 + (uint64_t)(ob * b_buf16 + (uint32_t)kProdB[q] * b_term16);
+#pragma unroll
+            for (int ks = 0; ks < SUB / 16; ++ks)
+              tc::Mma<KP>::template bf16<0, 0>(acc, aq + (uint64_t)((uint32_t)ks * a_step16), bq + (uint64_t)((uint32_t)ks * b_step16), 1);
+          }
+          tc::wg_commit();
+          tc::wg_wait<0>();
+          tc::fence_acc(acc);
+#pragma unroll
+          for (int i = 0; i < KP / 2; ++i) {
+            if (mb == 0) sum0[i] = __fadd_rn(sum0[i], acc[i]);
+            else sum1[i] = __fadd_rn(sum1[i], acc[i]);
+          }
+        }
+        __syncwarp();
+        if (lane == 0) tc::mbar_arrive(&sh.empty[ob]);
+      }
+    }
+    float* mine = p.partial + (int64_t)blockIdx.x * p.K * p.KR;
+#pragma unroll
+    for (int mb = 0; mb < 2; ++mb) {
+#pragma unroll
+      for (int e = 0; e < KP / 2; ++e) {
+        const int n = 64 * (wg + 2 * mb) + 16 * w4 + (lane >> 2) + 8 * ((e >> 1) & 1);
+        const int kk = 8 * (e >> 2) + 2 * (lane & 3) + (e & 1);
+        if (n < p.K && kk < p.KR) mine[(int64_t)n * p.KR + kk] = mb == 0 ? sum0[e] : sum1[e];
+      }
+    }
+  } else {
+    const int ct = tid;
+    float* patch0 = reinterpret_cast<float*>(smem + p.off_patch);
+    const int64_t plane = (int64_t)p.H * p.W;
+    const int d_items = p.K * (SUB / 8), x_items = p.KR * (SUB / 8);
+    const int patch_floats = p.patch_bytes / 4;
+    float4 dpre[WWG_DMAX][2];
+    auto fetch_dy = [&](int tile, int sub) {
+      const int b = tile / p.tiles_per_img, h0 = (tile - b * p.tiles_per_img) * p.TH;
+      const float* dy_tile = p.dy + (int64_t)b * p.K * plane + (int64_t)h0 * p.W + sub * SUB;
+#pragma unroll
+      for (int k = 0; k < WWG_DMAX; ++k) {
+        const int i = ct + k * WWG_NCONV;
+        if (i < d_items) {
+          const int n = i / (SUB / 8), j = i - n * (SUB / 8);
+          const float4* src = reinterpret_cast<const float4*>(dy_tile + (int64_t)n * plane + j * 8);
+          dpre[k][0] = __ldg(src); dpre[k][1] = __ldg(src + 1);
+        }
+      }
+    };
+    float pre[PF];
+    if ((int)blockIdx.x < p.n_tiles) {
+      patch_fetch(p, blockIdx.x, ct, WWG_NCONV, pre);
+      patch_commit(p, patch0, blockIdx.x, ct, WWG_NCONV, pre);
+    }
+    uint32_t it = 0, t = 0;
+    for (int tile = blockIdx.x; tile < p.n_tiles; tile += gridDim.x, ++t) {
+      const float* patch = patch0 + (size_t)(t & 1u) * patch_floats;
+      conv_bar_sync(WWG_NCONV);
+      const int next = tile + (int)gridDim.x;
+      if (next < p.n_tiles) patch_fetch(p, next, ct, WWG_NCONV, pre);
+      for (int sub = 0; sub < nsub; ++sub, ++it) {
+        const uint32_t ob = it % WWG_NBUF, oph = (it / WWG_NBUF) & 1u;
+        fetch_dy(tile, sub);
+        const auto& dcur = dpre;
+        if (!tc::mbar_wait(&sh.empty[ob], oph ^ 1u, p.err, 516)) goto done;
+        uint8_t* abuf = aop + (size_t)ob * p.a_buf_bytes;
+        uint8_t* bbuf = bop + (size_t)ob * b_buf_bytes;
+#pragma unroll
+        for (int k = 0; k < WWG_DMAX; ++k) {
+          const int i = ct + k * WWG_NCONV;
+          if (i < d_items) {
+            const int n = i / (SUB / 8), j = i - n * (SUB / 8);
+            const float v[8] = {dcur[k][0].x, dcur[k][0].y, dcur[k][0].z, dcur[k][0].w,
+                                dcur[k][1].x, dcur[k][1].y, dcur[k][1].z, dcur[k][1].w};
+            store_split8(v, abuf + ((size_t)j * p.NP + n) * 16, p.a_term_bytes);
+          }
+        }
+        for (int i = ct; i < x_items; i += WWG_NCONV) {
+          const int kk = i / (SUB / 8), j = i - kk * (SUB / 8);
+          const int m = sub * SUB + j * 8;
+          const float* src = patch + tab[kk] + (m / p.W) * p.PW + (m % p.W);
+          float v[8];
+#pragma unroll
+          for (int e = 0; e < 8; ++e) v[e] = src[e];
+          store_split8(v, bbuf + ((size_t)j * KP + kk) * 16, p.b_term_bytes);
+        }
+        tc::fence_proxy_async_smem();
+        __syncwarp();
+        if (lane == 0) tc::mbar_arrive(&sh.full[ob]);
+      }
+      if (next < p.n_tiles) patch_commit(p, patch0 + (size_t)((t + 1) & 1u) * patch_floats, next, ct, WWG_NCONV, pre);
+    }
+  }
+done:
+  __syncthreads();
+}
+
+static int plan_wgrad_wg(const mnb_conv_shape* s, Params& p, int& smem_bytes) {
+  if (int e = plan(s, true, p, smem_bytes)) return e;
+  if (p.KP != WWG_KP) return mnb_fail(MNB_E_UNSUPPORTED, "fp32 tc wgrad (two warpgroups): C*R*S not in 65..80");
+  if (p.NP != 256) return mnb_fail(MNB_E_UNSUPPORTED, "fp32 tc wgrad (two warpgroups): 128 output channels or fewer");
+  p.off_b = 0;
+  p.off_a = WWG_NBUF * 3 * p.b_term_bytes;
+  p.off_patch = p.off_a + WWG_NBUF * p.a_buf_bytes;
+  p.off_tab = p.off_patch + 2 * p.patch_bytes;
+  p.sum_bytes = 0;
+  p.nbuf_a = WWG_NBUF;
+  smem_bytes = p.off_tab + p.KP * 4;
+  if (smem_bytes > kMaxDynSmem) return mnb_fail(MNB_E_UNSUPPORTED, "fp32 tc wgrad (two warpgroups): shared memory budget");
+  return 0;
+}
+
 static int debug_mask() {
   static const int m = [] { const char* e = getenv("MNB_FCONV_DEBUG"); return e ? atoi(e) : 0; }();
   return m;
@@ -490,6 +841,27 @@
   fwd_kernel<<<grid_size(p), NTHREADS, smem_bytes, (cudaStream_t)stream>>>(p);
   MNB_LAUNCHED(1);
   return 0;
+}
+
+extern "C" int mnb_fconv2d_wg_plan(const mnb_conv_shape* s, int32_t* out, int32_t n) {
+  tcfp32::Params p{};
+  int smem_bytes = 0;
+  if (int e = tcfp32::plan_wg(s, p, smem_bytes)) return e;
+  const int v[8] = {p.NP, p.KP, p.TH, p.n_tiles, tcfp32::grid_size(p), p.nbuf_a, smem_bytes, p.C * p.PH * p.PW};
+  if (out)
+    for (int i = 0; i < std::min(n, 8); ++i) out[i] = v[i];
+  return 0;
+}
+
+extern "C" int mnb_fconv2d_fwd_wg(const mnb_conv_shape* s, const float* x, const float* w, const float* bias, float* y,
+                                  int32_t* err_flag, mnb_stream_t stream) {
+  using namespace tcfp32;
+  MNB_REQUIRE(s && x && w && y && err_flag, "NULL pointer");
+  Params p{};
+  int smem_bytes = 0;
+  if (int e = plan_wg(s, p, smem_bytes)) return e;
+  p.x = x; p.w = w; p.bias = bias; p.y = y; p.err = err_flag;
+  return p.NP == 192 ? launch_fwd_wg<192>(p, smem_bytes, stream) : launch_fwd_wg<256>(p, smem_bytes, stream);
 }
 
 extern "C" int64_t mnb_fconv2d_wgrad_tc_scratch_bytes(const mnb_conv_shape* s) {
@@ -522,3 +894,34 @@
   MNB_LAUNCHED(2);
   return 0;
 }
+
+extern "C" int64_t mnb_fconv2d_wgrad_wg_scratch_bytes(const mnb_conv_shape* s) {
+  tcfp32::Params p{};
+  int smem = 0;
+  if (tcfp32::plan_wgrad_wg(s, p, smem)) return -1;
+  return (int64_t)tcfp32::grid_size(p) * p.K * p.KR * 4;
+}
+
+extern "C" int mnb_fconv2d_wgrad_wg(const mnb_conv_shape* s, const float* dy, const float* x, float* dw, void* scratch,
+                                    int32_t* err_flag, mnb_stream_t stream) {
+  using namespace tcfp32;
+  MNB_REQUIRE(s && dy && x && dw && scratch && err_flag, "NULL pointer");
+  MNB_REQUIRE((reinterpret_cast<uintptr_t>(dy) & 15) == 0, "dy must be 16-byte aligned");
+  Params p{};
+  int smem_bytes = 0;
+  if (int e = plan_wgrad_wg(s, p, smem_bytes)) return e;
+  p.x = x; p.dy = dy; p.partial = reinterpret_cast<float*>(scratch); p.err = err_flag;
+  static bool attr_set = false;
+  if (!attr_set) {
+    cudaError_t ce = cudaFuncSetAttribute(wgrad_wg_kernel<WWG_KP>, cudaFuncAttributeMaxDynamicSharedMemorySize, kMaxDynSmem);
+    if (ce != cudaSuccess) return mnb_fail((int)ce, "cudaFuncSetAttribute: %s", cudaGetErrorString(ce));
+    attr_set = true;
+  }
+  const int grid = grid_size(p);
+  cudaStream_t st = (cudaStream_t)stream;
+  wgrad_wg_kernel<WWG_KP><<<grid, WWG_THREADS, smem_bytes, st>>>(p);
+  const int n = p.K * p.KR;
+  reduce_partials_kernel<<<std::min(mnb_ceil_div(n, 256), MNB_NUM_SMS * 4), 256, 0, st>>>(p.partial, n, grid, dw);
+  MNB_LAUNCHED(2);
+  return 0;
+}
diff --git a/micronet_b200/csrc/mnb_tc.cuh b/micronet_b200/csrc/mnb_tc.cuh
--- a/micronet_b200/csrc/mnb_tc.cuh
+++ b/micronet_b200/csrc/mnb_tc.cuh
@@ -289,6 +289,30 @@
         : "memory");
   }
 };
+template <> struct Mma<192> {
+  template <int TA, int TB>
+  static __device__ __forceinline__ void bf16(float (&d)[96], uint64_t da, uint64_t db, uint32_t scale_d) {
+    asm volatile(
+        "{\n\t.reg .pred p;\n\tsetp.ne.b32 p, %98, 0;\n\t"
+        "wgmma.mma_async.sync.aligned.m64n192k16.f32.bf16.bf16 "
+        "{%0, %1, %2, %3, %4, %5, %6, %7, %8, %9, %10, %11, %12, %13, %14, %15, %16, %17, %18, %19, %20, %21, %22, %23, %24, %25, %26, %27, %28, %29, %30, %31, %32, %33, %34, %35, %36, %37, %38, %39, %40, %41, %42, %43, %44, %45, %46, %47, %48, %49, %50, %51, %52, %53, %54, %55, %56, %57, %58, %59, %60, %61, %62, %63, %64, %65, %66, %67, %68, %69, %70, %71, %72, %73, %74, %75, %76, %77, %78, %79, %80, %81, %82, %83, %84, %85, %86, %87, %88, %89, %90, %91, %92, %93, %94, %95}, %96, %97, p, 1, 1, %99, %100;\n\t}"
+        : "+f"(d[0]), "+f"(d[1]), "+f"(d[2]), "+f"(d[3]), "+f"(d[4]), "+f"(d[5]), "+f"(d[6]), "+f"(d[7]), "+f"(d[8]), "+f"(d[9]), "+f"(d[10]), "+f"(d[11]), "+f"(d[12]), "+f"(d[13]), "+f"(d[14]), "+f"(d[15]), "+f"(d[16]), "+f"(d[17]), "+f"(d[18]), "+f"(d[19]), "+f"(d[20]), "+f"(d[21]), "+f"(d[22]), "+f"(d[23]), "+f"(d[24]), "+f"(d[25]), "+f"(d[26]), "+f"(d[27]), "+f"(d[28]), "+f"(d[29]), "+f"(d[30]), "+f"(d[31]), "+f"(d[32]), "+f"(d[33]), "+f"(d[34]), "+f"(d[35]), "+f"(d[36]), "+f"(d[37]), "+f"(d[38]), "+f"(d[39]), "+f"(d[40]), "+f"(d[41]), "+f"(d[42]), "+f"(d[43]), "+f"(d[44]), "+f"(d[45]), "+f"(d[46]), "+f"(d[47]), "+f"(d[48]), "+f"(d[49]), "+f"(d[50]), "+f"(d[51]), "+f"(d[52]), "+f"(d[53]), "+f"(d[54]), "+f"(d[55]), "+f"(d[56]), "+f"(d[57]), "+f"(d[58]), "+f"(d[59]), "+f"(d[60]), "+f"(d[61]), "+f"(d[62]), "+f"(d[63]), "+f"(d[64]), "+f"(d[65]), "+f"(d[66]), "+f"(d[67]), "+f"(d[68]), "+f"(d[69]), "+f"(d[70]), "+f"(d[71]), "+f"(d[72]), "+f"(d[73]), "+f"(d[74]), "+f"(d[75]), "+f"(d[76]), "+f"(d[77]), "+f"(d[78]), "+f"(d[79]), "+f"(d[80]), "+f"(d[81]), "+f"(d[82]), "+f"(d[83]), "+f"(d[84]), "+f"(d[85]), "+f"(d[86]), "+f"(d[87]), "+f"(d[88]), "+f"(d[89]), "+f"(d[90]), "+f"(d[91]), "+f"(d[92]), "+f"(d[93]), "+f"(d[94]), "+f"(d[95])
+        : "l"(da), "l"(db), "r"(scale_d), "n"(TA), "n"(TB)
+        : "memory");
+  }
+};
+template <> struct Mma<256> {
+  template <int TA, int TB>
+  static __device__ __forceinline__ void bf16(float (&d)[128], uint64_t da, uint64_t db, uint32_t scale_d) {
+    asm volatile(
+        "{\n\t.reg .pred p;\n\tsetp.ne.b32 p, %130, 0;\n\t"
+        "wgmma.mma_async.sync.aligned.m64n256k16.f32.bf16.bf16 "
+        "{%0, %1, %2, %3, %4, %5, %6, %7, %8, %9, %10, %11, %12, %13, %14, %15, %16, %17, %18, %19, %20, %21, %22, %23, %24, %25, %26, %27, %28, %29, %30, %31, %32, %33, %34, %35, %36, %37, %38, %39, %40, %41, %42, %43, %44, %45, %46, %47, %48, %49, %50, %51, %52, %53, %54, %55, %56, %57, %58, %59, %60, %61, %62, %63, %64, %65, %66, %67, %68, %69, %70, %71, %72, %73, %74, %75, %76, %77, %78, %79, %80, %81, %82, %83, %84, %85, %86, %87, %88, %89, %90, %91, %92, %93, %94, %95, %96, %97, %98, %99, %100, %101, %102, %103, %104, %105, %106, %107, %108, %109, %110, %111, %112, %113, %114, %115, %116, %117, %118, %119, %120, %121, %122, %123, %124, %125, %126, %127}, %128, %129, p, 1, 1, %131, %132;\n\t}"
+        : "+f"(d[0]), "+f"(d[1]), "+f"(d[2]), "+f"(d[3]), "+f"(d[4]), "+f"(d[5]), "+f"(d[6]), "+f"(d[7]), "+f"(d[8]), "+f"(d[9]), "+f"(d[10]), "+f"(d[11]), "+f"(d[12]), "+f"(d[13]), "+f"(d[14]), "+f"(d[15]), "+f"(d[16]), "+f"(d[17]), "+f"(d[18]), "+f"(d[19]), "+f"(d[20]), "+f"(d[21]), "+f"(d[22]), "+f"(d[23]), "+f"(d[24]), "+f"(d[25]), "+f"(d[26]), "+f"(d[27]), "+f"(d[28]), "+f"(d[29]), "+f"(d[30]), "+f"(d[31]), "+f"(d[32]), "+f"(d[33]), "+f"(d[34]), "+f"(d[35]), "+f"(d[36]), "+f"(d[37]), "+f"(d[38]), "+f"(d[39]), "+f"(d[40]), "+f"(d[41]), "+f"(d[42]), "+f"(d[43]), "+f"(d[44]), "+f"(d[45]), "+f"(d[46]), "+f"(d[47]), "+f"(d[48]), "+f"(d[49]), "+f"(d[50]), "+f"(d[51]), "+f"(d[52]), "+f"(d[53]), "+f"(d[54]), "+f"(d[55]), "+f"(d[56]), "+f"(d[57]), "+f"(d[58]), "+f"(d[59]), "+f"(d[60]), "+f"(d[61]), "+f"(d[62]), "+f"(d[63]), "+f"(d[64]), "+f"(d[65]), "+f"(d[66]), "+f"(d[67]), "+f"(d[68]), "+f"(d[69]), "+f"(d[70]), "+f"(d[71]), "+f"(d[72]), "+f"(d[73]), "+f"(d[74]), "+f"(d[75]), "+f"(d[76]), "+f"(d[77]), "+f"(d[78]), "+f"(d[79]), "+f"(d[80]), "+f"(d[81]), "+f"(d[82]), "+f"(d[83]), "+f"(d[84]), "+f"(d[85]), "+f"(d[86]), "+f"(d[87]), "+f"(d[88]), "+f"(d[89]), "+f"(d[90]), "+f"(d[91]), "+f"(d[92]), "+f"(d[93]), "+f"(d[94]), "+f"(d[95]), "+f"(d[96]), "+f"(d[97]), "+f"(d[98]), "+f"(d[99]), "+f"(d[100]), "+f"(d[101]), "+f"(d[102]), "+f"(d[103]), "+f"(d[104]), "+f"(d[105]), "+f"(d[106]), "+f"(d[107]), "+f"(d[108]), "+f"(d[109]), "+f"(d[110]), "+f"(d[111]), "+f"(d[112]), "+f"(d[113]), "+f"(d[114]), "+f"(d[115]), "+f"(d[116]), "+f"(d[117]), "+f"(d[118]), "+f"(d[119]), "+f"(d[120]), "+f"(d[121]), "+f"(d[122]), "+f"(d[123]), "+f"(d[124]), "+f"(d[125]), "+f"(d[126]), "+f"(d[127])
+        : "l"(da), "l"(db), "r"(scale_d), "n"(TA), "n"(TB)
+        : "memory");
+  }
+};
 __device__ __forceinline__ void mma_s8_n128(int32_t (&d)[64], uint64_t da, uint64_t db, uint32_t scale_d) {
   asm volatile(
       "{\n\t.reg .pred p;\n\tsetp.ne.b32 p, %66, 0;\n\t"
diff --git a/micronet_b200/functional.py b/micronet_b200/functional.py
--- a/micronet_b200/functional.py
+++ b/micronet_b200/functional.py
@@ -408,10 +408,37 @@
     return True
 
 
+def fconv_fwd(sh, x, w, bias, y, kind=None):
+    lib = L.load()
+    args = (C.byref(sh), x.data_ptr(), w.data_ptr(), L.ptr(bias), y.data_ptr(), L.tc_err_flag(x.device).data_ptr(),
+            L.stream())
+
+    def run():
+        rc = lib.mnb_fconv2d_fwd_wg(*args)
+        return lib.mnb_fconv2d_fwd_tc(*args) if rc == L.E_UNSUPPORTED else rc
+    return run() if kind is None else _timed(kind, sh, run)
+
+
+def fconv_wgrad(sh, dy, x, dw, kind=None):
+    lib = L.load()
+    entry = lib.mnb_fconv2d_wgrad_wg
+    fbytes = int(lib.mnb_fconv2d_wgrad_wg_scratch_bytes(C.byref(sh)))
+    if fbytes < 0:
+        entry = lib.mnb_fconv2d_wgrad_tc
+        fbytes = int(lib.mnb_fconv2d_wgrad_tc_scratch_bytes(C.byref(sh)))
+    if fbytes < 0:
+        return False
+    ws = torch.empty(max(fbytes, 4), dtype=torch.uint8, device=dy.device)
+
+    def run():
+        return entry(C.byref(sh), dy.data_ptr(), x.data_ptr(), dw.data_ptr(), ws.data_ptr(),
+                     L.tc_err_flag(dy.device).data_ptr(), L.stream())
+    L.check(run() if kind is None else _timed(kind, sh, run), "fconv2d_wgrad")
+    return True
+
+
 def _fconv_forward(ctx, x, wq, bias, sh, y):
-    lib = L.load()
-    rc = _timed("fconv_fwd_tc", sh, lambda: lib.mnb_fconv2d_fwd_tc(
-        C.byref(sh), x.data_ptr(), wq.data_ptr(), L.ptr(bias), y.data_ptr(), L.tc_err_flag(x.device).data_ptr(), L.stream()))
+    rc = fconv_fwd(sh, x, wq, bias, y, "fconv_fwd_tc")
     if rc == L.E_UNSUPPORTED:
         return False
     L.check(rc, "fconv2d_fwd_tc")
@@ -483,17 +510,8 @@
 
 
 def _fconv_wgrad(ctx, dy):
-    lib = L.load()
-    sh = ctx.sh
-    fbytes = int(lib.mnb_fconv2d_wgrad_tc_scratch_bytes(C.byref(sh)))
-    if fbytes < 0:
-        return None
     dwq = torch.empty_like(ctx.wq)
-    ws = torch.empty(max(fbytes, 4), dtype=torch.uint8, device=dy.device)
-    L.check(_timed("fconv_wgrad_tc", sh, lambda: lib.mnb_fconv2d_wgrad_tc(
-        C.byref(sh), dy.data_ptr(), ctx.x.data_ptr(), dwq.data_ptr(), ws.data_ptr(), L.tc_err_flag(dy.device).data_ptr(),
-        L.stream())), "fconv2d_wgrad_tc")
-    return dwq
+    return dwq if fconv_wgrad(ctx.sh, dy, ctx.x, dwq, "fconv_wgrad_tc") else None
 
 
 class QuantConv2dFn(Function):
diff --git a/micronet_b200/fused.py b/micronet_b200/fused.py
--- a/micronet_b200/fused.py
+++ b/micronet_b200/fused.py
@@ -290,14 +290,13 @@
 
     @staticmethod
     def forward(ctx, x, w, bias, padding):
-        lib = L.load()
+        from .functional import fconv_fwd
         x, w = x.contiguous(), w.contiguous()
         b, c, h, wd = x.shape
         k, _, r, s_ = w.shape
         sh = L.ConvShape(b, c, h, wd, k, r, s_, 1, 1, padding, padding, 1, 1, 1)
         y = torch.empty((b, k, h, wd), dtype=torch.float32, device=x.device)
-        rc = lib.mnb_fconv2d_fwd_tc(C.byref(sh), x.data_ptr(), w.data_ptr(), L.ptr(bias), y.data_ptr(),
-                                    L.tc_err_flag(x.device).data_ptr(), L.stream())
+        rc = fconv_fwd(sh, x, w, bias, y)
         ctx.engine = rc == 0
         if rc == L.E_UNSUPPORTED:
             y = TF.conv2d(x, w, bias, 1, padding)
@@ -309,7 +308,7 @@
 
     @staticmethod
     def backward(ctx, dy):
-        lib = L.load()
+        from .functional import fconv_wgrad
         x, w = ctx.saved_tensors
         presummed = getattr(dy, "_mnb_channel_sum", None)
         dy = dy.contiguous()
@@ -317,14 +316,8 @@
         if ctx.needs_input_grad[0]:
             dx = torch.nn.grad.conv2d_input(x.shape, w, dy, 1, ctx.padding)
         if ctx.needs_input_grad[1]:
-            need = int(lib.mnb_fconv2d_wgrad_tc_scratch_bytes(C.byref(ctx.sh))) if ctx.engine else -1
-            if need >= 0:
-                dw = torch.empty_like(w)
-                scratch = torch.empty(need, dtype=torch.uint8, device=dy.device)
-                L.check(lib.mnb_fconv2d_wgrad_tc(C.byref(ctx.sh), dy.data_ptr(), x.data_ptr(), dw.data_ptr(),
-                                                 scratch.data_ptr(), L.tc_err_flag(dy.device).data_ptr(), L.stream()),
-                        "fconv2d_wgrad_tc")
-            else:
+            dw = torch.empty_like(w)
+            if not (ctx.engine and fconv_wgrad(ctx.sh, dy, x, dw)):
                 dw = torch.nn.grad.conv2d_weight(x, w.shape, dy, 1, ctx.padding)
         if ctx.has_bias and ctx.needs_input_grad[2]:
             if presummed is not None and presummed.numel() == dy.shape[1]:
```
